# sthagen/foundationdb

Hardware: AMD Instinct MI355X
Metric: resolved txns/sec (conflict ranges checked/sec) per batch; HBM GB/s vs peak (higher is better)
Workload: dtype u8/int64 (byte keys, int64 versions)

## Files before the change

foundationdb_amd/build.py:

```python
from __future__ import annotations

import os
import shutil
import subprocess
import sys

HERE = os.path.dirname(os.path.abspath(__file__))
CSRC = os.path.join(HERE, "csrc")
ROOT = os.path.dirname(HERE)
LIB = os.path.join(HERE, "libfdbcs.so")
SOURCES = ["engine.cpp", "kernels.hip"]
HEADERS = ["dkey.h", "engine.h", "scan.h", "launch.h", "lane_xor.h"]
ARCH = os.environ.get("FDBCS_OFFLOAD_ARCH", "gfx950")


def _hipcc() -> str:
    for c in (os.environ.get("HIPCC"), "/opt/rocm/bin/hipcc", shutil.which("hipcc")):
        if c and os.path.exists(c):
            return c
    raise RuntimeError("hipcc not found")


def _stale() -> bool:
    if not os.path.exists(LIB):
        return True
    t = os.path.getmtime(LIB)
    deps = [os.path.join(CSRC, f) for f in SOURCES + HEADERS] + [os.path.join(ROOT, "include", "fdb_conflict_set.h")]
    return any(os.path.getmtime(d) > t for d in deps)


def build(force: bool = False, verbose: bool = False) -> str:
    if not force and not _stale():
        return LIB
    objs = []
    hipcc = _hipcc()
    common = ["-O3", "-std=c++17", "-fPIC", f"--offload-arch={ARCH}", "-Wall", "-Wno-unused-function",
              "-mllvm", "-disable-promote-alloca-to-lds"]
    for src in SOURCES:
        obj = os.path.join(CSRC, src.rsplit(".", 1)[0] + ".o")
        cmd = [hipcc, *common, "-c", os.path.join(CSRC, src), "-o", obj]
        if src.endswith(".cpp"):
            cmd = [hipcc, "-O3", "-std=c++17", "-fPIC", "-Wall", "-c", os.path.join(CSRC, src), "-o", obj]
        if verbose:
            print(" ".join(cmd), file=sys.stderr)
        subprocess.check_call(cmd)
        objs.append(obj)
    tmp = LIB + ".tmp"
    cmd = [hipcc, f"--offload-arch={ARCH}", "-shared", "-fPIC", "-o", tmp, *objs]
    if verbose:
        print(" ".join(cmd), file=sys.stderr)
    subprocess.check_call(cmd)
    os.replace(tmp, LIB)
    return LIB


if __name__ == "__main__":
    build(force="--force" in sys.argv, verbose=True)
    print(LIB)
```

foundationdb_amd/csrc/engine.cpp:

```cpp
#include <hip/hip_runtime.h>
#include <stdio.h>
#include <stdlib.h>
#include <string.h>
#include <unistd.h>

#include <cxxabi.h>

#include <algorithm>
#include <array>
#include <atomic>
#include <chrono>
#include <condition_variable>
#include <functional>
#include <mutex>
#include <new>
#include <string>
#include <thread>
#include <unordered_set>
#include <vector>

#include "../../include/fdb_conflict_set.h"
#include "engine.h"

using namespace fdbcs;
// ... 107 lines not shown
            shutdown();
            throw;
        }
    }
    ~AddPool() { shutdown(); }
    void shutdown() {
        {
            std::lock_guard<std::mutex> lk(m);
            stop = true;
            gen.fetch_add(1);
        }
        cv.notify_all();
        for (auto& t : th)
            if (t.joinable()) t.join();
    }
    void run(uint32_t g, int nn, const std::function<void(int)>* fn) {
        uint64_t cur = ticket.load(std::memory_order_acquire);
        for (;;) {
            if ((uint32_t)(cur >> 32) != g || (int)(cur & 0xffffffffu) >= nn) return;
            if (ticket.compare_exchange_weak(cur, cur + 1, std::memory_order_acq_rel)) {
                (*fn)((int)(cur & 0xffffffffu));
                done.fetch_add(1, std::memory_order_acq_rel);
                cur = ticket.load(std::memory_order_acquire);
            }
        }
    }
    void worker() {
        uint32_t seen = 0;
        for (;;) {
            uint32_t g;
            int nn;
            const std::function<void(int)>* fn;
            {
                std::unique_lock<std::mutex> lk(m);
                if (gen.load(std::memory_order_relaxed) == seen && !stop) {
                    sleepers.fetch_add(1);
                    cv.wait(lk, [&] { return stop || gen.load(std::memory_order_relaxed) != seen; });
                    sleepers.fetch_sub(1);
                }
                if (stop) return;
                seen = g = gen.load(std::memory_order_relaxed);
                nn = n;
                fn = job;
            }
            run(g, nn, fn);
        }
    }
    void parallel_for(int tickets, const std::function<void(int)>& fn) {
        uint32_t g;
        {
            std::lock_guard<std::mutex> lk(m);
            g = gen.load(std::memory_order_relaxed) + 1;
            n = tickets;
            job = &fn;
            done.store(0, std::memory_order_relaxed);
            ticket.store((uint64_t)g << 32, std::memory_order_release);
            gen.store(g, std::memory_order_release);
        }
        if (sleepers.load(std::memory_order_acquire) > 0) cv.notify_all();
        run(g, tickets, &fn);
        while (done.load(std::memory_order_acquire) < tickets) __builtin_ia32_pause();
    }
};

struct fdbcs_conflict_set {
    int device = 0;
    hipStream_t stream = nullptr;
    hipStream_t astream = nullptr;
    hipStream_t cstream = nullptr;
    hipEvent_t ev_c[kNumWork] = {};
    hipEvent_t ev_cmp = nullptr;
    bool cmp_recorded = false;
    int split_check = 2;
    hipStream_t ustream = nullptr;
    hipEvent_t ev_a[kNumWork] = {};
    hipEvent_t ev_b[kNumWork] = {};
    hipStream_t ystream = nullptr;
    hipEvent_t ev_res[kNumWork] = {};
    hipEvent_t xfree_ev[kNumWork] = {};
    bool prev_segs = false;
    int prev_wp = 0;
    int64_t prev_now = 0;
    int last_wp = -1, prev2_wp = -1;
    bool xfree_rec[kNumWork] = {};
    fdbcs_batch* ws_user[kNumWork] = {};
    fdbcs_batch* xfree_user[kNumWork] = {};
    bool y_async[kNumWork] = {};
    bool wused[kNumWork] = {};
    int wpar = 0;
    int timing = 0;
    uint32_t seq = 0;
    int64_t oldest = 0;
    int64_t header_version = 0;
    int64_t max_written = 0;
    int gc_interval = 0;
    int batches_since_compact = 0;
    int compactions_since_gc = 0;
    int64_t gc_applied = 0;
    int64_t delta_limit = 0;

    DBuf hkey[2], hlt[2], hver[2];
    DBuf lvl[kMaxLevels];
    DBuf dir;
    DBuf edir[2];
    uint32_t ddir_epoch[2] = {0, 0};
    uint32_t ddir_counter = 0;
    int cur = 0;
    int64_t hist_cap = 0;
    int64_t n_ub = 0;
    int64_t lvl3_n = 0;
    int64_t lvl2_n = 0;
    DBuf dkey[2], dlt[2], dver[2];
    DBuf dlvl[2][kMaxLevels];
    int dcur = 0;
    int64_t delta_cap = 0;
    int64_t nd_ub = 0;
    int64_t dlvl3_n = 0;
    int64_t dlvl2_n = 0;
    DBuf cws[6];
    DBuf htail[2];
    int tcur = 0;
    int64_t tail_ub = 0;
    int64_t tail_cap = 0;
    DBuf scal;
    int64_t route_timeout_ms = 60000;
    DBuf route_btail;
    std::vector<uint8_t> route_bounds;
    DBuf ws[kNumWork][56];
    DBuf wbtail[kNumWork];
    int64_t ws_T = -1, ws_R = -1, ws_W = -1;
    Work work[kNumWork]{};
    int64_t edge_cap = 0;

    int inflight = 0;
    bool validate = false;
    int bucket_target = 0;
    bool sort_cold = false;
    DBuf quant;
    int qcur = 0;
    bool quant_valid = false;
    hipStream_t quant_sa = nullptr;
    hipEvent_t ev_quant = nullptr;
    int64_t sort_big_buckets = 0;
    bool trace = false;
    bool serial = false;
    bool no_prepass = false;
    int64_t tail_reclaim = kTailReclaimDefault;
    bool write_groups = true;
    bool directory = true;
    uint32_t dir_p = 0;
    uint64_t dir_phi = 0, dir_plo = 0;
    uint32_t dir_e = 0, dir_top = 0;
    uint32_t dir_pos[kDirPos] = {}, dir_w[kDirPos] = {};
    int dir_bits = 0;
    DBuf trace_buf;
    struct KProf {
        const void* func;
        int64_t launches;
        double ms;
    };
    std::vector<KProf> kprof;
    const void* timed_func = nullptr;
    HBuf hold;
    HBuf hedge;
    bool skip_edges = true;
    fdbcs_stats stats{};
    std::vector<BatchSlot*> pool;
    bool submit_thread = true;
    int add_threads = 5;
    AddPool* add_pool = nullptr;
    int wait_query_ms = 2;
    bool htrace = false;
    std::vector<HSpan> htr[2];
    uint32_t work_a_seq = 0, work_y_seq = 0;
    double add_prof[4] = {0, 0, 0, 0};
    int64_t add_prof_n = 0;
    std::thread worker;
    std::mutex wmu;
    std::condition_variable wcv;
    std::atomic<int> wjob{0};
    std::atomic<uint32_t> b_issued{0};
    uint32_t b_recorded = 0;
    std::atomic<int> werr{0};
    LaunchList work_a, work_c;
    hipStream_t work_sa = nullptr;
    uint32_t work_need_b = 0;
    LaunchList work_y;
    hipStream_t work_ys = nullptr;
    uint32_t work_need_x = 0;
    std::atomic<uint32_t> x_issued{0};
    fdbcs_batch* work_y_batch = nullptr;
    LaunchList rec_a, rec_b, rec_c, rec_y, pending_b, pending_y;
    hipStream_t pending_ys = nullptr;
    fdbcs_batch* pending_batch = nullptr;
    std::unordered_set<fdbcs_batch*> live;
    DBuf x_pos, x_val, x_btail, x_state, x_ver, x_off, x_bytes;
    bool x_valid = false;
    int64_t x_n = 0, x_nbytes = 0;
    hipEvent_t x_ev0 = nullptr, x_ev1 = nullptr;
    double x_ms_kernels = 0, x_ms_d2h = 0;
    int64_t x_hdr = 0;
    DBuf i_bytes, i_off, i_ver, i_bnd, i_okey, i_olt, i_over, i_otail, i_mval, i_mkey, i_mlt, i_dblt, i_vblt, i_state;
    hipEvent_t i_ev[6] = {};
    double i_ms_kernels = 0, i_ms_host = 0;
};

struct BatchSlot {
    DBuf dev;
    HBuf pin_in;
    HBuf pin_out;
    DBuf dverdict;
    hipEvent_t ev[kPhCount] = {};
    bool events_made = false;
    hipEvent_t ev_up = nullptr;
    HBuf pin_inv;
    DBuf rt_scan, rt_inv, rt_rids, rt_dres, rt_info, rt_txpre;
    HBuf rt_res;
    hipEvent_t ev_rt0 = nullptr, ev_rt1 = nullptr;
    bool rt_timed = false;
    std::vector<hipEvent_t> prof_pool;
    size_t prof_next = 0;
    std::vector<std::pair<const void*, std::pair<hipEvent_t, hipEvent_t>>> prof_spans;
    LaunchList::Profile prof{&prof_pool, &prof_next, &prof_spans};
};

struct fdbcs_batch {
    fdbcs_conflict_set* cs = nullptr;
    BatchSlot* slot = nullptr;
    int report_enabled = 0;
    int state = 0;
    std::vector<int64_t> snap;
    std::vector<uint8_t> flags;
    std::vector<int32_t> roff{0}, woff{0};
    std::vector<int32_t> rowner, wowner;
    std::vector<DKey> rkeys, wkeys;
    std::vector<uint8_t> tail;
    bool direct = false;
    size_t d_keys = 0, d_rown = 0, d_wown = 0, d_tail = 0, d_small = 0;
    size_t d_tail_bytes = 0;
    BatchDev bd{};
    size_t tail_bytes = 0;
    uint8_t* h_verdict = nullptr;
    Scalars* h_scal = nullptr;
    uint8_t* h_rconf = nullptr;
    uint8_t* h_hist = nullptr;
    int32_t* h_first = nullptr;
    bool gc_ran = false;
    bool compacted = false;
    uint32_t seq = 0;
    volatile uint32_t* h_flag = nullptr;
    int64_t n_report = 0;
    uint32_t recorded = 0;
    bool any_report = false;
    int64_t check_hist = 0;
    std::vector<int32_t> out_ids;
    int64_t out_n = 0;
    uint8_t* out_dev = nullptr;
    int wp = 0;
    int32_t max_len = 0;
    int64_t wtail = 0;
    std::vector<int32_t> conf_off, conf_idx;
    int32_t n_committed = 0, n_too_old = 0;

    bool routed = false, route_pending = false;
    int32_t rT = 0, rR = 0, rW = 0;
    size_t r_tail = 0;

    int32_t T() const { return routed ? rT : (int32_t)snap.size(); }
    int32_t R() const { return routed ? rR : roff.back(); }
    int32_t W() const { return routed ? rW : woff.back(); }
    size_t tail_size() const { return routed ? r_tail : direct ? d_tail_bytes : tail.size(); }
};

namespace {

void add_key(fdbcs_batch* b, std::vector<DKey>& out, const uint8_t* p, int32_t len) {
    DKey k;
    dkey_prefix(p, (uint32_t)len, &k.hi, &k.lo);
    k.len = (uint32_t)len;
    k.tail = 0;
    if (len > b->max_len) b->max_len = len;
    if (len > 16) {
        k.tail = (uint32_t)b->tail.size();
        b->tail.insert(b->tail.end(), p + 16, p + len);
    }
    out.push_back(k);
}

int cmp_bytes(const uint8_t* a, int32_t al, const uint8_t* b, int32_t bl) {
    int c = memcmp(a, b, (size_t)std::min(al, bl));
    if (c) return c;
    return (al > bl) - (al < bl);
}

int ensure_scan_arena(fdbcs_conflict_set* cs) {
    if (cs->ws_T < 0 || cs->hist_cap <= 0) return FDBCS_OK;
    if (cs->delta_cap <= 0) return FDBCS_OK;
    const int64_t words = scan_arena_words(cs->ws_T, cs->ws_R, cs->ws_W, cs->hist_cap, cs->delta_cap);
    for (int k = 0; k < kNumWork; k++) {
        Work& w = cs->work[k];
        int rc = cs->ws[k][kWsArenaSlot].ensure(8 * words + 64);
        if (rc) return rc;
        w.scan_arena = (uint64_t*)cs->ws[k][kWsArenaSlot].p;
        if ((rc = cs->ws[k][kWsTileSlot].ensure(4 * (std::max(cs->hist_cap, cs->delta_cap) / 256 + 8)))) return rc;
        w.tile_first = (int32_t*)cs->ws[k][kWsTileSlot].p;
        carve_scans(w, cs->ws_T, cs->ws_R, cs->ws_W, cs->hist_cap, cs->delta_cap);
        HIPOK(hipMemsetAsync(w.scan_arena, 0, 8 * w.scan_words, cs->stream));
        for (int q = 0; q < kNumScans; q++) w.scan[q].error = &w.bsc->debug_error;
    }
    HIPOK(hipStreamSynchronize(cs->stream));
    return FDBCS_OK;
}

int flush_pending(fdbcs_conflict_set* cs);

int sync_all(fdbcs_conflict_set* cs) {
    if (int rc = flush_pending(cs)) return rc;
    HIPOK(hipStreamSynchronize(cs->ustream));
    HIPOK(hipStreamSynchronize(cs->cstream));
    HIPOK(hipStreamSynchronize(cs->astream));
    HIPOK(hipStreamSynchronize(cs->stream));
    HIPOK(hipStreamSynchronize(cs->ystream));
    cs->prev_segs = false;
    return FDBCS_OK;
}

int ensure_btail(fdbcs_conflict_set* cs, int64_t bytes) {
    const size_t need = (size_t)bytes + 64;
    if (cs->wbtail[0].p && need <= cs->wbtail[0].cap) return FDBCS_OK;
    if (int rc = sync_all(cs)) return rc;
    for (int k = 0; k < kNumWork; k++) {
        if (int rc = cs->wbtail[k].ensure(std::max<size_t>(need, 1 << 16))) return rc;
        cs->work[k].btail = (uint8_t*)cs->wbtail[k].p;
    }
    return FDBCS_OK;
}

int ensure_workspace(fdbcs_conflict_set* cs, int64_t T, int64_t R, int64_t W) {
    if (T <= cs->ws_T && R <= cs->ws_R && W <= cs->ws_W) return FDBCS_OK;
    T = std::max<int64_t>(T, std::max<int64_t>(cs->ws_T, 1024));
    R = std::max<int64_t>(R, std::max<int64_t>(cs->ws_R, 4096));
    W = std::max<int64_t>(W, std::max<int64_t>(cs->ws_W, 4096));
    if (int rc = sync_all(cs)) return rc;
    const int64_t E = 2 * (R + W);
    int64_t edge_cap = std::max<int64_t>(16 * R, 1 << 22);
    if (const char* env = getenv("FDBCS_EDGE_CAP")) edge_cap = std::max<int64_t>(1, atoll(env));
    for (int k = 0; k < kNumWork; k++) {
    Work& w = cs->work[k];
    size_t off = 0;
    char* arena = nullptr;
    auto take = [&](size_t bytes, void** ptr) -> int {
        off = align_up(off, 256);
        if (arena) *ptr = arena + off;
        off += bytes + 64;
        return FDBCS_OK;
    };
    for (int pass = 0; pass < 2; pass++) {
    if (pass == 1) {
        if (int rc = cs->ws[k][0].ensure(align_up(off, (size_t)2 << 20))) return rc;
        arena = (char*)cs->ws[k][0].p;
        off = 0;
    }
#define TAKE(field, bytes) \
    if (int rc = take((bytes), (void**)&w.field)) return rc
    TAKE(hist_conf, T);
    TAKE(rconf, R);
    TAKE(status, T);
    TAKE(first_conf, 4 * T);
    const int64_t slab_buckets = std::min<int64_t>(kSortMaxBuckets, (E + kSortTarget - 1) / kSortTarget + 1);
    TAKE(items, sizeof(SortItem) * E);
    TAKE(scnt, 8 * kCntStride * (size_t)kSortMaxBuckets);
    TAKE(slab, sizeof(SortItem) * kSlab * slab_buckets);
    TAKE(ovf, sizeof(SortItem) * E);
    TAKE(ovf_b, 4 * E);
    TAKE(big, sizeof(SortItem) * E);
    TAKE(big_p, 4 * E);
    TAKE(samples, sizeof(SortItem) * kMaxSample);
    TAKE(srank, 4 * (kMaxSample + 64));
    w.slab_buckets = (int32_t)slab_buckets;
    TAKE(pos, 4 * E);
    TAKE(pmeta, 4 * E);
    TAKE(cwb, 4 * (E + 1));
    TAKE(crb, 4 * (E + 1));
    TAKE(cwe, 4 * (E + 1));
    TAKE(wends, 8 * (2 * W + 1));
    TAKE(wkeys, sizeof(DKey) * (2 * W + 1));
    TAKE(segk, sizeof(DKey) * (2 * W + 2));
    TAKE(cflag, 2 * W + 2);
    TAKE(wbrange, 4 * W);
    TAKE(wlead, 4 * (W + 1));
    TAKE(wtxn, 4 * (W + 1));
    TAKE(gminc, 4 * (W + 1));
    TAKE(rbrange, 4 * R);
    TAKE(eoff, 4 * (R + 1));
    TAKE(poff, 4 * (R + W + 1));
    TAKE(pcg, 4 * (R + W + 1));
    TAKE(pcoff, 4 * (R + W + 1));
    TAKE(pcbase, 4 * (R + W + 1));
    TAKE(pca, 4 * (R + W + 1));
    TAKE(ecur, 4 * R);
    TAKE(edges, 4 * edge_cap);
    TAKE(eptr, 4 * T);
    TAKE(pre_st, T);
    TAKE(pre_ep, 4 * T);
    TAKE(pre_end, 4 * T);
    TAKE(ulist, 32 * T);
    TAKE(wpk, 4 * (W + 1));
    TAKE(tedges, 4 * edge_cap);
    TAKE(mcs_bits, 8 * (E / 64 + 2));
    TAKE(seg_b, 4 * (W + 1));
    TAKE(seg_e, 4 * (W + 1));
    TAKE(seg_lo, 8 * (W + 1));
    TAKE(seg_hi, 8 * (W + 1));
    TAKE(seg_rem, 8 * (W + 1));
    TAKE(seg_ins, 8 * (W + 1));
    TAKE(seg_tlen, 8 * (W + 1));
    TAKE(seg_endins, W + 1);
    TAKE(seg_vend, 8 * (W + 1));
    TAKE(verdict, T);
    TAKE(bsc, sizeof(BatchScalars));
    }
#undef TAKE
    w.edge_cap = edge_cap;
    w.cap_T = T;
    w.cap_R = R;
    HIPOK(hipMemsetAsync(w.hist_conf, 0, T, cs->stream));
    HIPOK(hipMemsetAsync(w.rconf, 0, R, cs->stream));
    HIPOK(hipMemsetAsync(w.ecur, 0, 4 * R, cs->stream));
    HIPOK(hipMemsetAsync(w.scnt, 0, 8 * kCntStride * (size_t)kSortMaxBuckets, cs->stream));
    HIPOK(hipMemsetAsync(w.srank, 0, 4 * (kMaxSample + 64), cs->stream));
    HIPOK(hipMemsetAsync(w.bsc, 0, sizeof(BatchScalars), cs->stream));
    if (k >= 1) {
        Work& w0 = cs->work[0];
        w.c_lo = w0.c_lo, w.c_hi = w0.c_hi, w.c_rem = w0.c_rem, w.c_ins = w0.c_ins, w.c_val = w0.c_val;
        w.c_exact = w0.c_exact;
    }
    }
    cs->edge_cap = edge_cap;
    cs->prev_segs = false;
    cs->ws_T = T;
    cs->ws_R = R;
    cs->ws_W = W;
    return ensure_scan_arena(cs);
}

constexpr int64_t kDeltaFloor = 1250000;
constexpr int kTimingEvery = 4;
int64_t delta_limit_for(const fdbcs_conflict_set* cs, int64_t n_base) {
    if (cs->delta_limit > 0) return cs->delta_limit;
    return std::max<int64_t>({(int64_t)1 << 16, n_base / 16, std::min<int64_t>(n_base / 4, kDeltaFloor)});
}


Hist hist_of(fdbcs_conflict_set* cs, int k) {
    Hist h;
    h.key = (ulonglong2*)cs->hkey[k].p;
    h.lt = (uint2*)cs->hlt[k].p;
    h.ver = (int64_t*)cs->hver[k].p;
    return h;
}

void carve_index(MaxLevels& m, ulonglong2* base, int64_t cap) {
    for (int L = 0; L < kIdxLevels; L++) {
        m.skey[L] = base;
        base += idx_level_cap(cap, L);
    }
    m.skey8 = base;
    m.idx_cap = cap;
}

int64_t index_bytes(int64_t cap) {
    int64_t n = 0;
    for (int L = 0; L < kIdxLevels; L++) n += idx_level_cap(cap, L);
    return 16 * (n + cap / 8 + 2);
}

static void set_dir_fields(const fdbcs_conflict_set* cs, MaxLevels& m) {
    m.dir_p = cs->dir_p;
    m.dir_phi = cs->dir_phi;
    m.dir_plo = cs->dir_plo;
    m.dir_e = cs->dir_e;
    m.dir_top = cs->dir_top;
    for (int i = 0; i < kDirPos; i++) m.dir_pos[i] = cs->dir_pos[i], m.dir_w[i] = cs->dir_w[i];
}

static int set_dir_map(fdbcs_conflict_set* cs, const ulonglong2* k, int64_t n) {
    auto byte_at = [](const ulonglong2& x, int i) -> uint32_t {
        return i < 8 ? (uint32_t)(x.x >> (56 - 8 * i)) & 255u : (uint32_t)(x.y >> (56 - 8 * (i - 8))) & 255u;
    };
    const bool rank = n >= 2;
    uint32_t p = 0;
    if (rank) {
        const uint64_t xh = k[0].x ^ k[n - 1].x, xl = k[0].y ^ k[n - 1].y;
        const uint32_t lcp = xh ? (uint32_t)__builtin_clzll(xh) / 8 : (xl ? 8 + (uint32_t)__builtin_clzll(xl) / 8 : 16);
        p = std::min<uint32_t>(lcp, 15);
    }
    const uint64_t mh = p >= 8 ? ~0ull : (p ? ~0ull << (64 - 8 * p) : 0ull);
    const uint64_t ml = p <= 8 ? 0ull : ~0ull << (128 - 8 * p);
    cs->dir_p = p;
    cs->dir_phi = n ? k[0].x & mh : 0;
    cs->dir_plo = n ? k[0].y & ml : 0;
    const int npos = std::min<int>(kDirPos, 16 - (int)p);
    uint32_t lo[kDirPos], hi[kDirPos];
    for (int i = 0; i < kDirPos; i++) lo[i] = rank ? 255 : 0, hi[i] = 255;
    if (rank) {
        for (int i = 0; i < kDirPos; i++) hi[i] = 0;
        const int64_t stride = std::max<int64_t>(1, n / (1 << 21));
        auto mark = [&](const ulonglong2& x) {
            for (int i = 0; i < npos; i++) {
                const uint32_t b = byte_at(x, (int)p + i);
                lo[i] = std::min(lo[i], b);
                hi[i] = std::max(hi[i], b);
            }
        };
        for (int64_t j = 0; j < n; j += stride) mark(k[j]);
        mark(k[n - 1]);
    }
    const int64_t samples = (n + kFan - 1) / kFan;
    uint64_t budget = 1ull << 16;
    if (cs->dir_bits)
        budget = 1ull << cs->dir_bits;
    else
        while (budget < (1ull << kDirMaxBits) && 8 * budget < (uint64_t)samples) budget <<= 1;
    uint32_t radix[kDirPos], shift[kDirPos];
    uint64_t prod = 1;
    int e = 0;
    for (int i = 0; i < npos; i++) {
        const uint32_t d = hi[i] - lo[i] + 1;
        shift[i] = 0;
        if (prod * d <= budget) {
            radix[i] = d;
            prod *= d;
            if (d > 1) e = i + 1;
            continue;
        }
        uint32_t s = 0;
        while (prod * (((d - 1) >> s) + 1) > budget) s++;
        if (((d - 1) >> s) + 1 > 1) {
            radix[i] = ((d - 1) >> s) + 1;
            shift[i] = s;
            e = i + 1;
        }
        break;
    }
    prod = 1;
    for (int i = 0; i < e; i++) prod *= radix[i];
    uint64_t w = 1;
    for (int i = kDirPos - 1; i >= 0; i--) {
        if (i >= e) {
            cs->dir_pos[i] = cs->dir_w[i] = 0;
            continue;
        }
        cs->dir_pos[i] = lo[i] | (hi[i] - lo[i] + 1) << 8 | shift[i] << 17;
        cs->dir_w[i] = (uint32_t)w;
        w *= radix[i];
    }
    cs->dir_e = (uint32_t)e;
    cs->dir_top = (uint32_t)prod + 2;
    return FDBCS_OK;
}

MaxLevels levels_of(fdbcs_conflict_set* cs, int k) {
    MaxLevels m;
    m.lvl[0] = (int64_t*)cs->hver[k].p;
    for (int L = 1; L < kMaxLevels; L++) m.lvl[L] = (int64_t*)cs->lvl[L].p;
    m.keys = (const ulonglong2*)cs->hkey[k].p;
    carve_index(m, (ulonglong2*)cs->lvl[0].p, cs->hist_cap);
    m.dir = cs->directory ? (const int32_t*)cs->dir.p : nullptr;
    set_dir_fields(cs, m);
    return m;
}

Hist delta_of(fdbcs_conflict_set* cs, int k) {
    Hist h;
    h.key = (ulonglong2*)cs->dkey[k].p;
    h.lt = (uint2*)cs->dlt[k].p;
    h.ver = (int64_t*)cs->dver[k].p;
    return h;
}

MaxLevels dlevels_of(fdbcs_conflict_set* cs, int k) {
    MaxLevels m;
    m.lvl[0] = (int64_t*)cs->dver[k].p;
    for (int L = 1; L < kMaxLevels; L++) m.lvl[L] = (int64_t*)cs->dlvl[k][L].p;
    m.keys = (const ulonglong2*)cs->dkey[k].p;
    carve_index(m, (ulonglong2*)cs->dlvl[k][0].p, cs->delta_cap);
    m.edir = (uint64_t*)cs->edir[k].p;
    m.edir_epoch = cs->edir[k].p ? cs->ddir_epoch[k] : 0;
    set_dir_fields(cs, m);
    return m;
}

int sync_sizes(fdbcs_conflict_set* cs) {
    if (int rc = sync_all(cs)) return rc;
    Scalars s;
    HIPOK(hipMemcpyAsync(&s, cs->scal.p, sizeof(s), hipMemcpyDeviceToHost, cs->stream));
    HIPOK(hipStreamSynchronize(cs->stream));
    cs->n_ub = s.n;
    cs->nd_ub = s.nd;
    cs->tail_ub = s.tail_used;
    return FDBCS_OK;
}

int alloc_levels(DBuf* lv, int64_t cap, int64_t* top_n, int64_t* l2_n) {
    lv[0].release();
    if (int rc = lv[0].ensure(index_bytes(cap))) return rc;
    int64_t m = cap;
    for (int L = 1; L < kMaxLevels; L++) {
// ... 1598 lines not shown
    b->bd.rowner = a.rown;
    b->bd.wowner = a.wown;
    b->bd.snap = a.snap;
    b->bd.roff = a.roff;
    b->bd.woff = a.woff;
    b->bd.flags = a.flags;
    b->bd.tail = a.tail;
    b->routed = true;
    b->route_pending = true;
    b->rT = b->rR = b->rW = 0;
    b->out_dev = conflict_out;
    b->out_n = n_global;
    b->out_ids.clear();
    b->state = 1;
    return FDBCS_OK;
}

static int finish_route(fdbcs_batch* b) {
    if (!b->route_pending) return FDBCS_OK;
    BatchSlot* sl = b->slot;
    HIPOK(hipEventSynchronize(sl->ev_up));
    std::atomic_thread_fence(std::memory_order_acquire);
    RouteResult r;
    memcpy(&r, (const void*)sl->rt_res.p, sizeof(r));
    if (r.error != 0) {
        if (r.error == 2) fprintf(stderr, "fdbcs: routed batch: the shares' ready flag was never set\n");
        b->routed = b->route_pending = false;
        b->out_dev = nullptr;
        b->out_n = 0;
        b->state = 0;
        return r.error == 2 ? FDBCS_E_TIMEOUT
                            : r.error == 1 ? FDBCS_E_NOMEM : r.error == 3 ? FDBCS_E_INVALID : FDBCS_E_DEVICE;
    }
    b->rT = r.T;
    b->rR = r.R;
    b->rW = r.W;
    b->r_tail = (size_t)r.tail_bytes;
    b->tail_bytes = b->r_tail;
    b->bd.tail_n = r.tail_bytes;
    b->bd.T = r.T;
    b->bd.R = r.R;
    b->bd.W = r.W;
    b->wtail = r.tail_bytes + 14 * (int64_t)r.W;
    b->max_len = r.n_gt24 ? 25 : (r.n_gt19 ? 20 : 16);
    b->any_report = r.reports > 0;
    b->route_pending = false;
    return FDBCS_OK;
}

int fdbcs_batch_routed_info(fdbcs_batch* b, int32_t* T, int32_t* R, int32_t* W, void** inv_dev, void** read_ids_dev) {
    if (!b) return FDBCS_E_INVALID;
    if (!b->routed) return FDBCS_E_STATE;
    if (int rc = finish_route(b)) return rc;
    if (T) *T = b->rT;
    if (R) *R = b->rR;
    if (W) *W = b->rW;
    if (inv_dev) *inv_dev = b->slot->rt_inv.p;
    if (read_ids_dev) *read_ids_dev = b->slot->rt_rids.p;
    return FDBCS_OK;
}

int fdbcs_sync(fdbcs_conflict_set* cs) {
    if (!cs) return FDBCS_E_INVALID;
    HIPOK(hipSetDevice(cs->device));
    return sync_all(cs);
}

int fdbcs_batch_upload(fdbcs_batch* b) {
    if (!b) return FDBCS_E_INVALID;
    if (!b->cs) return FDBCS_E_STATE;
    if (b->state != 0) return b->state == 1 ? FDBCS_OK : FDBCS_E_STATE;
    HIPOK(hipSetDevice(b->cs->device));
    return do_upload(b, b->cs->ustream);
}


int fdbcs_batch_detect_async(fdbcs_batch* b, int64_t now, int64_t new_oldest_version) {
    if (!b) return FDBCS_E_INVALID;
    if (!b->cs) return FDBCS_E_STATE;
    if (b->state > 1) return FDBCS_E_STATE;
    fdbcs_conflict_set* cs = b->cs;
    const auto t_begin = std::chrono::steady_clock::now();
    HIPOK(hipSetDevice(cs->device));
    if (now < cs->max_written) return FDBCS_E_VERSION;
    if (int rc0 = finish_route(b)) return rc0;
    if (b->T() > kMaxTxnLds) return FDBCS_E_INVALID;
    const int64_t tail_add = b->wtail;
    if (cs->tail_ub + tail_add + 1 >= kTailLimit) return FDBCS_E_NOMEM;
    const int64_t T = b->T(), R = b->R(), W = b->W();
    int rc;
    if ((rc = ensure_workspace(cs, T, R, W))) return rc;
    if ((rc = ensure_btail(cs, (int64_t)b->tail_size()))) return rc;
    if ((rc = ensure_delta(cs, cs->nd_ub + 2 * W + 1))) return rc;
    if ((rc = ensure_history(cs, cs->n_ub + cs->nd_ub + 2 * W + 1, cs->tail_ub + tail_add + 1)))
        return rc;
    if ((rc = ensure_events(b))) return rc;
    if (cs->ddir_counter == UINT32_MAX && cs->edir[0].p) {
        if ((rc = sync_all(cs))) return rc;
        for (int k = 0; k < 2; k++) HIPOK(hipMemsetAsync(cs->edir[k].p, 0, 8 * (size_t)kDirAlloc, cs->stream));
        HIPOK(hipStreamSynchronize(cs->stream));
        cs->ddir_counter = 0;
    }
    const ResultLayout RL = result_layout(T, R);
    const size_t o_sc = RL.sc, o_fl = RL.fl, o_rc = RL.rc, o_hc = RL.hc, o_fc = RL.fc, out_bytes = RL.total;
    BatchSlot* sl = b->slot;
    if ((rc = sl->pin_out.ensure(out_bytes, true))) return rc;
    char* ho = (char*)sl->pin_out.p;
    b->h_verdict = (uint8_t*)ho;
    b->h_scal = (Scalars*)(ho + o_sc);
    b->h_flag = (volatile uint32_t*)(ho + o_fl);
    b->h_rconf = (uint8_t*)(ho + o_rc);
    b->h_hist = (uint8_t*)(ho + o_hc);
    b->h_first = (int32_t*)(ho + o_fc);
    if ((rc = sl->dverdict.ensure(T + 64))) return rc;
    if (b->out_dev && b->out_n > 0 && !b->routed) {
        if ((int64_t)b->out_ids.size() != T) return FDBCS_E_STATE;
        if ((rc = sl->pin_inv.ensure(4 * (size_t)b->out_n + 64, true))) return rc;
        int32_t* inv = (int32_t*)sl->pin_inv.p;
        std::fill(inv, inv + b->out_n, -1);
        for (int32_t t = 0; t < (int32_t)T; t++) inv[b->out_ids[t]] = t;
    }
    if (!b->routed) {
        b->any_report = b->n_report > 0;
    }
    b->seq = ++cs->seq;
    if (b->seq == 0) b->seq = ++cs->seq;
    *b->h_flag = 0;
    b->recorded = 0;

    hipStream_t s = cs->stream;
    const int timing = cs->timing;
    hipStream_t sa = (timing == 2 || cs->serial) ? s : cs->astream;
    const int wp = cs->wpar;
    cs->wpar = (wp + 1) % kNumWork;
    b->wp = wp;
    Work& w = cs->work[wp];
    w.groups = cs->write_groups && W > 0 && W <= kMaxGroupWrites && T <= kMaxTxnLds ? 1 : 0;
    const bool sampled = timing >= 2 || b->seq % (uint32_t)kTimingEvery == 0;
    auto rec = [&](int ph, int level) -> hipEvent_t {
        if (timing == 3 || timing < level || (level == 1 && (!sampled || cs->timed_func))) return nullptr;
        b->recorded |= 1u << ph;
        return sl->ev[ph];
    };
    auto mark = [&](int ph) -> int {
        if (hipEvent_t e = rec(ph, 2)) fdb_event(LaunchList::kTimingRecord, e, s);
        return FDBCS_OK;
    };
    const bool was_uploaded = b->state == 1;
    LaunchList& la = cs->rec_a;
    LaunchList& lb = cs->rec_b;
    LaunchList& lc = cs->rec_c;
    LaunchList& ly = cs->rec_y;
    la.clear();
    lb.clear();
    lc.clear();
    ly.clear();
    sl->prof_next = 0;
    sl->prof_spans.clear();
    const bool kprof = timing == 3 || (timing == 1 && sampled && cs->timed_func);
    for (LaunchList* L : {&la, &lb, &lc, &ly}) {
        L->prof = kprof ? &sl->prof : nullptr;
        L->timed_func = timing == 3 ? nullptr : cs->timed_func;
    }
    const bool split = (cs->split_check == 1 || (cs->split_check == 2 && cs->n_ub >= kSplitCheckMinBase)) &&
                       !cs->serial && timing != 2;
    const bool threaded = cs->submit_thread && timing < 2 && !cs->trace && sa != s;
    cs->stats.host_ms_prepare += host_ms_since(t_begin);
    const auto t_rec = std::chrono::steady_clock::now();
    const bool own_upload = timing != 2 && !cs->serial;
    if (hipEvent_t e = rec(kPhStart, 2)) HIPOK(hipEventRecord(e, sa));
    if (b->state == 0 && (rc = do_upload(b, own_upload ? cs->ustream : sa))) return rc;
    if (hipEvent_t e = rec(kPhUpload, 2)) HIPOK(hipEventRecord(e, sa));
    t_record = &la;
    const bool ws_busy = cs->wused[wp] && (threaded || !stage_b_done(cs, wp));
    if (ws_busy && (sa != s || cs->y_async[wp])) fdb_event(LaunchList::kSyncWait, cs->ev_b[wp], sa);
    if (cs->xfree_rec[wp] && sa != s && (threaded || !batch_done(cs->xfree_user[wp])))
        fdb_event(LaunchList::kSyncWait, cs->xfree_ev[wp], sa);
    cs->xfree_rec[wp] = false;
    cs->wused[wp] = true;
    cs->ws_user[wp] = b;
    if (own_upload || (was_uploaded && hipEventQuery(sl->ev_up) != hipSuccess))
        fdb_event(LaunchList::kSyncWait, sl->ev_up, sa);
    const BatchDev& bd = b->bd;
    if (b->routed) launch_route_too_old(sa, bd, cs->oldest);
    const bool long_keys = b->max_len > 24;
    Scalars* sc = (Scalars*)cs->scal.p;
    const int bsrc = cs->cur, dsrc = cs->dcur;
    const bool pipe = !(timing == 2 || cs->serial);
    hipStream_t ys = pipe ? cs->ystream : s;
    const bool use_prev = pipe && cs->prev_segs;
    const int dchk = use_prev ? dsrc ^ 1 : dsrc;
    const Tier base{hist_of(cs, bsrc), levels_of(cs, bsrc), &sc->n, cs->header_version};
    const Tier delta{delta_of(cs, dsrc), dlevels_of(cs, dsrc), &sc->ndb[dsrc], kHole};
    const Tier cdelta{delta_of(cs, dchk), dlevels_of(cs, dchk), &sc->ndb[dchk], kHole};
    PrevSegs ps{};
    if (use_prev) {
        const Work& pw = cs->work[cs->prev_wp];
        ps = PrevSegs{pw.segk, pw.btail, &pw.bsc->n_segments, cs->prev_now};
    }
    uint8_t* htail = (uint8_t*)cs->htail[cs->tcur].p;

    w.trace = cs->trace ? (unsigned long long*)cs->trace_buf.p : nullptr;
    w.no_prepass = cs->no_prepass ? 1 : 0;
    if (w.trace) {
        HIPOK(hipStreamSynchronize(cs->astream));
        HIPOK(hipStreamSynchronize(s));
        unsigned long long init[kTrSlots];
        for (int i = 0; i < kTrSlots; i++)
            init[i] = (i == kTrSampleBegin || i == kTrCheckBegin || i == kTrEpiBegin || i == kTrResBegin || i == kTrResW0min ||
                       i == kTrPartBegin || i == kTrBktBegin)
                          ? ~0ull
                          : 0ull;
        HIPOK(hipMemcpy(w.trace, init, sizeof(init), hipMemcpyHostToDevice));
    }
    int sort_nb = 0, sort_samples = 0;
    {
        const int64_t E = 2 * (R + W);
        const int nbk = sort_bucket_count(E, cs->bucket_target, w.slab_buckets);
        const bool cold = nbk > 1 && (cs->sort_cold || !cs->quant_valid);
        sort_nb = E > 0 ? nbk : 0;
        sort_samples = E > 0 && cold ? sort_cold_samples(E, nbk) : 0;
        const bool write_quant = E >= kQuantMinE;
        SplitKey* qt = (SplitKey*)cs->quant.p;
        if (cs->quant_sa && cs->quant_sa != sa) {
            if ((rc = flush_pending(cs))) return rc;
            HIPOK(hipEventRecord(cs->ev_quant, cs->quant_sa));
            fdb_event(LaunchList::kSyncWait, cs->ev_quant, sa);
        }
        cs->quant_sa = sa;
        launch_sort(sa, bd, w, qt + cs->qcur * kQuant, write_quant ? qt + (cs->qcur ^ 1) * kQuant : nullptr, cold,
                    cs->bucket_target, b->max_len > (int32_t)kSortNxLen, cs->validate, rec(kPhSortBegin, 1),
                    rec(kPhSortEnd, 1));
        if (write_quant) {
            cs->qcur ^= 1;
            cs->quant_valid = true;
        }
    }
    mark(kPhSort);
    if (cs->validate) launch_validate_sort(sa, bd, w);
    w.hseq = b->seq;
    launch_edges(sa, bd, w);
    if (sa != s) fdb_event(LaunchList::kSyncRecord, cs->ev_a[wp], sa);
    mark(kPhEdges);
    if (split) {
        t_record = &lc;
        hipStream_t sc_ = cs->cstream;
        fdb_event(LaunchList::kSyncWait, sl->ev_up, sc_);
        if (ws_busy) fdb_event(LaunchList::kSyncWait, cs->ev_b[wp], sc_);
        if (cs->cmp_recorded && (threaded || hipEventQuery(cs->ev_cmp) != hipSuccess))
            fdb_event(LaunchList::kSyncWait, cs->ev_cmp, sc_);
        fdb_event(LaunchList::kTimingRecord, rec(kPhCheckBegin, 1), sc_);
        launch_check_tier(sc_, bd, w, base, true, htail, long_keys, PrevSegs{});
        fdb_event(LaunchList::kTimingRecord, rec(kPhCheckEnd, 1), sc_);
        fdb_event(LaunchList::kSyncRecord, cs->ev_c[wp], sc_);
    }
    t_record = &lb;
    if (sa == s || !was_uploaded || hipEventQuery(sl->ev_up) != hipSuccess) fdb_event(LaunchList::kSyncWait, sl->ev_up, s);
    {
        const int wy = use_prev ? cs->prev2_wp : cs->last_wp;
        if (wy >= 0 && cs->y_async[wy] && (threaded || !stage_b_done(cs, wy)))
            fdb_event(LaunchList::kSyncWait, cs->ev_b[wy], s);
    }
    if (split) {
        b->check_hist = cs->n_ub;
        launch_check_tier(s, bd, w, cdelta, false, htail, long_keys, ps);
    } else {
        b->check_hist = cs->n_ub + cs->nd_ub;
        fdb_event(LaunchList::kTimingRecord, rec(kPhCheckBegin, 1), s);
        launch_check(s, bd, w, base, cdelta, htail, long_keys, ps);
        fdb_event(LaunchList::kTimingRecord, rec(kPhCheckEnd, 1), s);
    }
    if (use_prev) {
        cs->xfree_ev[cs->prev_wp] = cs->ev_res[wp];
        cs->xfree_user[cs->prev_wp] = b;
        cs->xfree_rec[cs->prev_wp] = true;
    }
    mark(kPhCheck);
    if (sa != s) fdb_event(LaunchList::kSyncWait, cs->ev_a[wp], s);
    if (split) fdb_event(LaunchList::kSyncWait, cs->ev_c[wp], s);
    w.vdev = (uint8_t*)sl->dverdict.p;
    launch_resolve(s, bd, w, b->any_report, (uint8_t*)sl->pin_out.dp, sc);
    w.vdev = nullptr;
    if (b->out_dev && b->out_n > 0)
        launch_conflict_output(s, bd, w, b->routed ? (const int32_t*)sl->rt_inv.p : (const int32_t*)sl->pin_inv.dp,
                               b->out_n, b->out_dev);
    if (b->any_report) {
        char* hdv = (char*)sl->pin_out.dp;
        if (R) launch_copy_bytes(s, hdv + o_rc, w.rconf, R);
        launch_copy_bytes(s, hdv + o_hc, w.hist_conf, T);
        launch_copy_bytes(s, hdv + o_fc, w.first_conf, 4 * T);
    }
    mark(kPhIntra);
    mark(kPhCombine);
    fdb_event(LaunchList::kSyncRecord, cs->ev_res[wp], s);
    t_record = &ly;
    if (ys != s) fdb_event(LaunchList::kSyncWait, cs->ev_res[wp], ys);
    const int dnew = dsrc ^ 1;
    const int64_t nd_after = cs->nd_ub + 2 * W;
    const int64_t new_oldest = std::max(cs->oldest, new_oldest_version);
    bool compact = nd_after > delta_limit_for(cs, cs->n_ub);
    if (cs->gc_interval > 0 && ++cs->batches_since_compact >= cs->gc_interval) compact = true;
    if (cs->tail_ub > cs->tail_reclaim) compact = true;
    char* hd = (char*)sl->pin_out.dp;
    launch_merge(ys, bd, w, delta.h, delta.m, delta_of(cs, dnew), dlevels_of(cs, dnew), &sc->ndb[dsrc], htail, sc, now,
                 cs->dlvl3_n, cs->dlvl2_n, cs->nd_ub + 1, rec(kPhCopyBegin, 1), rec(kPhCopyEnd, 1), long_keys);
    mark(kPhMerge);
    bool gc = false;
    int final_base = bsrc;
    const int64_t base_hint = cs->n_ub + nd_after + 1;
    if (compact) {
        launch_compact(ys, w, base.h, base.m, delta_of(cs, dnew), hist_of(cs, bsrc ^ 1), htail, sc,
                       cs->header_version, cs->lvl3_n, cs->lvl2_n, nd_after + 1, cs->n_ub + 1, rec(kPhCompBegin, 1),
                       rec(kPhCompEnd, 1), long_keys ? 2 : 1, cs->n_ub <= (16 << 20) ? 1024 : 4096,
                       cs->n_ub > (16 << 20));
        final_base = bsrc ^ 1;
        cs->batches_since_compact = 0;
        const bool gc_turn = cs->gc_interval > 0 || ++cs->compactions_since_gc >= kGcEveryCompactions;
        gc = (new_oldest > cs->gc_applied && gc_turn) || cs->tail_ub > cs->tail_reclaim;
        if (gc) cs->compactions_since_gc = 0;
    }
    mark(kPhCompact);
    if (gc) {
        launch_gc(ys, w, hist_of(cs, final_base), hist_of(cs, final_base ^ 1), htail,
                  (uint8_t*)cs->htail[cs->tcur ^ 1].p, sc, std::max(new_oldest, cs->gc_applied), cs->header_version,
                  base_hint);
        cs->tcur ^= 1;
        final_base ^= 1;
        cs->gc_applied = new_oldest;
    }
    mark(kPhGc);
    b->gc_ran = gc;
    b->compacted = compact;
    if (compact || !cs->edir[dnew].p) {
        cs->ddir_epoch[dnew] = 0;
    } else {
        cs->ddir_epoch[dnew] = ++cs->ddir_counter;
    }
    launch_epilogue(ys, bd, w, compact ? levels_of(cs, final_base) : dlevels_of(cs, dnew), sc, compact ? 1 : 0,
                    gc ? 1 : 0, (uint8_t*)hd, (uint32_t*)(hd + o_fl), b->seq,
                    compact ? base_hint : nd_after + 1, &sc->ndb[dnew], sort_nb, sort_samples);
    fdb_event(LaunchList::kSyncRecord, cs->ev_b[wp], ys);
    if (compact || gc) {
        fdb_event(LaunchList::kSyncRecord, cs->ev_cmp, ys);
        cs->cmp_recorded = true;
    }
    mark(kPhEpilogue);
    mark(kPhEnd);
    t_record = nullptr;
    cs->stats.host_ms_record += host_ms_since(t_rec);
    const auto t_sub = std::chrono::steady_clock::now();
    if (threaded) {
        if ((rc = worker_wait(cs))) return rc;
        std::swap(cs->work_a, la);
        std::swap(cs->work_c, lc);
        cs->work_sa = sa;
        cs->work_a_seq = b->seq;
        const bool prev = cs->pending_batch != nullptr;
        if (prev) {
            cs->work_y_seq = cs->pending_batch->seq;
            std::swap(cs->work_y, cs->pending_y);
            cs->work_ys = cs->pending_ys;
            cs->work_need_x = cs->x_issued.load(std::memory_order_relaxed) + 1;
            cs->work_y_batch = cs->pending_batch;
        }
        cs->work_need_b = cs->b_recorded;
        worker_start_job(cs);
        if (prev) {
            fdbcs_batch* pb_ = cs->pending_batch;
            cs->pending_batch = nullptr;
            const int64_t tx = cs->htrace ? mono_ns() : 0;
            const uint32_t pseq = pb_->seq;
            hipError_t e = cs->pending_b.replay(s, x_skip(cs, pb_), &cs->stats.x_launches_skipped);
            if (cs->htrace) cs->htr[0].push_back({pseq, 'X', tx, mono_ns()});
            cs->x_issued.fetch_add(1, std::memory_order_release);
            if (e != hipSuccess) return FDBCS_E_DEVICE;
        }
        std::swap(cs->pending_b, lb);
        std::swap(cs->pending_y, ly);
        cs->pending_ys = ys;
        cs->b_recorded++;
        cs->pending_batch = b;
    } else if (flush_pending(cs)) {
        return FDBCS_E_DEVICE;
    } else {
        HIPOK(la.replay(sa));
        if (split) HIPOK(lc.replay(cs->cstream));
        HIPOK(lb.replay(s));
        HIPOK(ly.replay(ys));
    }
    HIPOK(take_launch_error());
    cs->stats.host_ms_submit += host_ms_since(t_sub);
    cs->cur = final_base;
    cs->dcur = dnew;
    cs->prev_segs = pipe && !compact;
    cs->prev2_wp = cs->last_wp;
    cs->last_wp = wp;
    cs->y_async[wp] = ys != s;
    cs->prev_wp = wp;
    cs->prev_now = now;
    cs->oldest = new_oldest;
    if (W) cs->max_written = std::max(cs->max_written, now);
    if (compact) {
        cs->n_ub += nd_after;
        cs->nd_ub = 0;
    } else {
        cs->nd_ub = nd_after;
    }
    cs->tail_ub += tail_add;
    cs->inflight++;
    cs->x_valid = false;
    b->state = 2;
    if (cs->htrace)
        cs->htr[0].push_back({b->seq, 'D',
                              (int64_t)std::chrono::duration_cast<std::chrono::nanoseconds>(t_begin.time_since_epoch()).count(),
                              mono_ns()});
    return FDBCS_OK;
}

int fdbcs_batch_wait(fdbcs_batch* b, uint8_t* verdicts, int32_t* n_committed, int32_t* n_too_old) {
    if (!b) return FDBCS_E_INVALID;
    if (b->state == 2 && !b->cs) return FDBCS_E_STATE;
    fdbcs_conflict_set* cs = b->cs;
    if (b->state == 2) {
        const int64_t tw0 = cs->htrace ? mono_ns() : 0;
        HIPOK(hipSetDevice(cs->device));
        if (cs->pending_batch == b)
            if (int rc = flush_pending(cs)) return rc;
        if (cs->work_y_batch == b)
            if (int rc = worker_wait(cs)) return rc;
        auto t_q = std::chrono::steady_clock::now();
        for (uint64_t spin = 0; *b->h_flag != b->seq; spin++) {
            __builtin_ia32_pause();
            if ((spin & 4095) != 4095) continue;
            if (std::chrono::steady_clock::now() - t_q < std::chrono::milliseconds(cs->wait_query_ms)) continue;
            t_q = std::chrono::steady_clock::now();
            {
                hipError_t e = hipStreamQuery(cs->astream);
                if (e == hipSuccess || e == hipErrorNotReady) e = hipStreamQuery(cs->stream);
                if (e == hipSuccess) e = hipStreamQuery(cs->ystream);
                if (e != hipSuccess && e != hipErrorNotReady) {
                    fprintf(stderr, "fdbcs: stream error while waiting: %s\n", hipGetErrorString(e));
                    return FDBCS_E_DEVICE;
                }
                if (e == hipSuccess && *b->h_flag != b->seq) {
                    fprintf(stderr, "fdbcs: stream idle but batch %u not completed\n", b->seq);
                    return FDBCS_E_DEVICE;
                }
            }
        }
        std::atomic_thread_fence(std::memory_order_acquire);
        if (cs->htrace) cs->htr[0].push_back({b->seq, 'W', tw0, mono_ns()});
        if (cs->trace && cs->inflight == 1) {
            if (int rc = sync_all(cs)) return rc;
            unsigned long long tr[kTrSlots];
            HIPOK(hipMemcpy(tr, cs->trace_buf.p, sizeof(tr), hipMemcpyDeviceToHost));
            auto us = [&](int a, int z) { return (double)((long long)(tr[z] - tr[a])) / 100.0; };
            fprintf(stderr,
                    "fdbcs trace: sample %.2f us, check %.2f us (check starts %+.2f us after sample); epilogue "
                    "levels %.2f, zero %.2f, host %.2f, fence %.2f us\n",
                    us(kTrSampleBegin, kTrSampleEnd), us(kTrCheckBegin, kTrCheckEnd), us(kTrSampleBegin, kTrCheckBegin),
                    us(kTrEpiBegin, kTrEpiLevels), us(kTrEpiLevels, kTrEpiZero), us(kTrEpiZero, kTrEpiHost),
                    us(kTrEpiHost, kTrEpiFence));
            fprintf(stderr,
                    "fdbcs trace: sort partition fill %.2f, search %.2f, end %.2f us; bucket prologue %.2f, "
                    "sorted %.2f, ties %.2f, end %.2f us (partition start to bucket start %.2f us)\n",
                    us(kTrPartBegin, kTrPartFill), us(kTrPartBegin, kTrPartSearch), us(kTrPartBegin, kTrPartEnd),
                    us(kTrBktBegin, kTrBktPrologue), us(kTrBktBegin, kTrBktSorted), us(kTrBktBegin, kTrBktTies),
                    us(kTrBktBegin, kTrBktEnd),
                    us(kTrPartBegin, kTrBktBegin));
            {
                const double nw = tr[kTrBktWaves] ? (double)tr[kTrBktWaves] : 1.0;
                fprintf(stderr, "fdbcs trace: bucket tie runs: %llu lanes in runs, %llu ranked in registers, %llu serially, "
                        "longest run %llu\n", tr[kTrBktRuns], tr[kTrBktSimple], tr[kTrBktSlow], tr[kTrBktMaxRun]);
                fprintf(stderr,
                        "fdbcs trace: bucket per wave (%llu waves): load %.2f, sort %.2f, ties %.2f, put %.2f us\n",
                        tr[kTrBktWaves], tr[kTrBktSumLoad] / nw / 100.0, tr[kTrBktSumSort] / nw / 100.0,
                        tr[kTrBktSumTies] / nw / 100.0, tr[kTrBktSumPut] / nw / 100.0);
                const double np = tr[kTrPartWaves] ? (double)tr[kTrPartWaves] : 1.0;
                fprintf(stderr,
                        "fdbcs trace: partition per wave (%llu waves): fill %.2f, tail copy %.2f, search %.2f, "
                        "place %.2f us\n",
                        tr[kTrPartWaves], tr[kTrPartSumFill] / np / 100.0, tr[kTrPartSumCopy] / np / 100.0,
                        tr[kTrPartSumSearch] / np / 100.0, tr[kTrPartSumPlace] / np / 100.0);
            }
            fprintf(stderr, "fdbcs trace: resolve pre-pass %.2f us, wait %.2f us, rounds %.2f us (setup %.2f, first round "
                    "%.2f of which minima %.2f, %d rounds), finish %.2f us; waves start %.2f..%.2f us before the first kernarg use\n",
                    us(kTrResBegin, kTrResPre), us(kTrResPre, kTrResWait), us(kTrResWait, kTrResRounds),
                    us(kTrResWait, kTrResSetup), us(kTrResSetup, kTrResRound1), us(kTrResSetup, kTrResMin1),
                    (int)b->h_scal->intra_rounds,
                    us(kTrResRounds, kTrResEnd), us(kTrResW0min, kTrResWait), us(kTrResW0max, kTrResWait));
            fprintf(stderr, "fdbcs trace: combine chunk 0: loads %.2f, scan1 %.2f, scan2 %.2f, stores %.2f us\n",
                    us(kTrResRounds, kTrCmbLoad), us(kTrCmbLoad, kTrCmbScan1), us(kTrCmbScan1, kTrCmbScan2),
                    us(kTrCmbScan2, kTrCmbStore));


        }
        if (b->h_scal->debug_error) {
            fprintf(stderr, "fdbcs: device invariant check failed (debug_error=%d)\n", b->h_scal->debug_error);
            cs->inflight--;
            b->state = 3;
            return FDBCS_E_DEVICE;
        }
        const int32_t T = b->T();
        int32_t nc = 0, nt = 0;
        for (int32_t t = 0; t < T; t++) {
            nc += b->h_verdict[t] == FDBCS_TRANSACTION_COMMITTED;
            nt += b->h_verdict[t] == FDBCS_TRANSACTION_TOO_OLD;
        }
        b->n_committed = nc;
        b->n_too_old = nt;
        b->conf_off.assign(T + 1, 0);
        b->conf_idx.clear();
        if (b->any_report) {
            for (int32_t t = 0; t < T; t++) {
                if ((b->flags[t] & kFlagReport) && b->h_verdict[t] == FDBCS_TRANSACTION_CONFLICT) {
                    if (b->h_hist[t]) {
                        for (int32_t r = b->roff[t]; r < b->roff[t + 1]; r++)
                            if (b->h_rconf[r]) b->conf_idx.push_back(r - b->roff[t]);
                    } else if (b->h_first[t] != INT_MAX) {
                        b->conf_idx.push_back(b->h_first[t]);
                    }
                }
                b->conf_off[t + 1] = (int32_t)b->conf_idx.size();
            }
        }
        fdbcs_stats& st = cs->stats;
        st.batches++;
        st.transactions += T;
        st.read_ranges += b->R();
        st.write_ranges += b->W();
        for (int e : {(int)kPhEnd, (int)kPhCompEnd, (int)kPhCopyEnd, (int)kPhCheckEnd})
            if ((b->recorded >> e) & 1u) {
                HIPOK(hipEventSynchronize(b->slot->ev[e]));
                break;
            }
        for (const auto& sp : b->slot->prof_spans) {
            HIPOK(hipEventSynchronize(sp.second.second));
            const double ms = ev_ms(sp.second.first, sp.second.second);
            auto it = std::find_if(cs->kprof.begin(), cs->kprof.end(), [&](const auto& k) { return k.func == sp.first; });
            if (it == cs->kprof.end()) {
                cs->kprof.push_back({sp.first, 0, 0.0});
                it = cs->kprof.end() - 1;
            }
            it->launches += 1;
            it->ms += ms;
        }
        b->slot->prof_spans.clear();
        auto ph = [&](int a, int z) {
            return ((b->recorded >> a) & (b->recorded >> z) & 1u) ? ev_ms(b->slot->ev[a], b->slot->ev[z]) : 0.0;
        };
        st.ms_upload += ph(kPhStart, kPhUpload);
        st.ms_sort += ph(kPhUpload, kPhSort);
        st.ms_intra += ph(kPhSort, kPhEdges) + ph(kPhCheck, kPhIntra);
        st.ms_check_read += ph(kPhEdges, kPhCheck);
        st.ms_combine += ph(kPhIntra, kPhCombine);
        st.ms_merge += ph(kPhCombine, kPhMerge);
        st.ms_compact += ph(kPhMerge, kPhCompact);
        st.ms_gc += ph(kPhCompact, kPhGc);
        st.ms_epilogue += ph(kPhGc, kPhEpilogue);
        st.ms_total += ph(kPhUpload, kPhEnd);
        if (b->h_scal->intra_edges < 0) {
            st.intra_fallbacks += 1;
        } else {
            st.intra_edges += b->h_scal->intra_edges;
            st.intra_rounds += b->h_scal->intra_rounds;
        }
        {
            const int64_t kept = b->h_scal->d_before - b->h_scal->d_rem, out = b->h_scal->nd_next;
            const int64_t bytes = 32 * (kept + (out - kept) + out);
            st.merge_bytes_all += bytes;
            st.delta_sum += b->h_scal->d_before;
            st.base_sum += b->h_scal->n;
            st.segments_sum += b->h_scal->n_segments;
            if ((b->recorded >> kPhCopyEnd) & 1u) {
                st.ms_merge_kernel += ph(kPhCopyBegin, kPhCopyEnd);
                st.merge_launches += 1;
                st.merge_bytes += bytes;
            }
        }
        if ((b->recorded >> kPhCheckEnd) & 1u) {
            st.ms_check_kernel += ph(kPhCheckBegin, kPhCheckEnd);
            st.check_launches += b->R() > 0;
            st.check_reads += b->R();
            st.check_history += b->R() > 0 ? b->check_hist : 0;
        }
        if ((b->recorded >> kPhSortEnd) & 1u) {
            st.ms_sort_kernel += ph(kPhSortBegin, kPhSortEnd);
            st.sort_launches += 1;
            st.sort_items += 2 * (int64_t)(b->R() + b->W());
        }
        st.gc_runs += b->gc_ran ? 1 : 0;
        st.sort_big_buckets += b->h_scal->sort_big;
        if (b->routed && b->slot->rt_timed) {
            float ms = 0.f;
            if (hipEventElapsedTime(&ms, b->slot->ev_rt0, b->slot->ev_rt1) == hipSuccess) st.ms_route_kernels += ms;
            st.routed_batches += 1;
            b->slot->rt_timed = false;
        }
        if (b->compacted) {
            st.compactions += 1;
            const int64_t kept = b->h_scal->c_before - b->h_scal->c_rem;
            const int64_t bytes = 32 * (kept + (b->h_scal->n_next - kept) + b->h_scal->n_next);
            st.compact_bytes_all += bytes;
            if ((b->recorded >> kPhCompEnd) & 1u) {
                st.ms_compact_kernel += ph(kPhCompBegin, kPhCompEnd);
                st.compact_launches += 1;
                st.compact_bytes += bytes;
            }
        }
        cs->inflight--;
        if (cs->inflight == 0) {
            cs->n_ub = b->h_scal->n;
            cs->nd_ub = b->h_scal->nd;
            cs->tail_ub = b->h_scal->tail_used;
        }
        b->state = 3;
    }
    if (b->state != 3) return FDBCS_E_STATE;
    if (verdicts && b->T()) memcpy(verdicts, b->h_verdict, b->T());
    if (n_committed) *n_committed = b->n_committed;
    if (n_too_old) *n_too_old = b->n_too_old;
    return FDBCS_OK;
}

int fdbcs_batch_detect_conflicts(fdbcs_batch* b, int64_t now, int64_t new_oldest_version, uint8_t* verdicts,
                                 int32_t* n_committed, int32_t* n_too_old) {
    int rc = fdbcs_batch_detect_async(b, now, new_oldest_version);
    if (rc) return rc;
    return fdbcs_batch_wait(b, verdicts, n_committed, n_too_old);
}

int fdbcs_batch_conflicting_reads(fdbcs_batch* b, int32_t txn, int32_t* idx_out, int32_t cap, int32_t* n_out) {
    if (!b || !n_out) return FDBCS_E_INVALID;
    if (b->state != 3) return FDBCS_E_STATE;
    if (txn < 0 || txn >= b->T()) return FDBCS_E_INVALID;
    const int32_t a = b->conf_off[txn], e = b->conf_off[txn + 1];
    *n_out = e - a;
    if (idx_out)
        for (int32_t i = a; i < e && i - a < cap; i++) idx_out[i - a] = b->conf_idx[i];
    return FDBCS_OK;
}

int fdbcs_batch_too_old(fdbcs_batch* b, int32_t* idx_out, int32_t cap, int32_t* n_out) {
// ... 84 lines not shown
```

foundationdb_amd/csrc/engine.h:

```cpp
#pragma once
#include <hip/hip_runtime.h>
#include <stdint.h>
#include <limits.h>

#include "dkey.h"
#include "scan.h"

namespace fdbcs {

constexpr int kBlock = 256;
constexpr int kWG = 1024;
constexpr int kSortTile = 4096;
constexpr int kFan = 64;
constexpr int kMaxLevels = 4;
constexpr int kL3Rep = 8;
constexpr int kL3Pad = 16;
__host__ __device__ constexpr int64_t l3_words(int64_t n) { return n * kL3Rep * kL3Pad; }
constexpr int kGcTile = 4096;
constexpr int kMaxGroupWrites = 12288;
constexpr int kMaxTxnLds = 49152;

enum : uint8_t { kUndecided = 0, kAborted = 1, kCommitted = 2 };
enum : uint8_t { kFlagTooOld = 1, kFlagReport = 2 };

struct Hist {
    ulonglong2* key;
    uint2* lt;
    int64_t* ver;
};

constexpr int kArity = 8;
constexpr int kDirMaxBits = 20;
constexpr int kDirAlloc = (1 << kDirMaxBits) + 4;
constexpr int kDirPos = 8;
constexpr int kDirRun = 128;
constexpr int kIdxLevels = 12;
struct MaxLevels {
    int64_t* lvl[kMaxLevels];
    const ulonglong2* keys;
    ulonglong2* skey[kIdxLevels];
    ulonglong2* skey8;
    int64_t idx_cap;
    const int32_t* dir = nullptr;
    uint32_t dir_p = 0;
    uint64_t dir_phi = 0, dir_plo = 0;
    uint32_t dir_e = 0;
    uint32_t dir_top = 0;
    uint32_t dir_pos[kDirPos] = {};
    uint32_t dir_w[kDirPos] = {};
    uint64_t* edir = nullptr;
    uint32_t edir_epoch = 0;
};
__host__ __device__ inline int64_t idx_level_cap(int64_t cap, int L) {
    int64_t d = 64;
    for (int i = 0; i < L && d <= cap; i++) d *= kArity;
    return cap / d + 2;
}

struct Scalars {
    int64_t n;
    int64_t nd;
    int64_t n_next;
    int64_t nd_next;
    int64_t n_gc;
    int64_t tail_used;
    int64_t tail_next;
    int64_t tail_gc;
    int64_t n_segments;
    int64_t d_before;
    int64_t d_rem;
    int64_t c_before;
    int64_t c_rem;
    int32_t debug_error;
    int32_t intra_rounds;
    int64_t intra_edges;
    int32_t sort_big;
    int32_t sort_pad;
    int64_t ndb[2];
};

struct BatchScalars {
    int64_t n_edges;
    int32_t edge_overflow;
    int32_t rounds;
    int32_t debug_error;
    int32_t ovf_n;
    int32_t sort_big;
    int64_t n_segments;
    int64_t n_pranges;
    int32_t n_undec;
    int32_t pad2;
};

constexpr int64_t kHole = INT64_MIN;

struct TierIO {
    const int64_t* n_in;
    int64_t* n_out;
    int64_t* before;
    int64_t* removed;
};

struct Segs {
    int64_t *lo, *hi, *rem, *ins;
    int32_t* tile_first;
};

enum ScanKind { kScanEdges, kScanSegSum, kScanCompact, kScanGc, kScanCover, kScanSegNum, kScanFold, kNumScans };

struct BatchDev {
    int32_t T, R, W;
    int64_t* snap;
    uint8_t* flags;
    int32_t* roff;
    int32_t* woff;
    int32_t* rowner;
    int32_t* wowner;
    DKey* keys;
    uint8_t* tail;
    int64_t tail_n;
};

#ifndef FDBCS_SORT_TARGET
#define FDBCS_SORT_TARGET 64
#endif
constexpr int kSortTarget = FDBCS_SORT_TARGET;
constexpr int kSlab = 256;
constexpr int kSortMaxBuckets = 4096;
constexpr int kQuant = 4096;
constexpr int kQuantMinE = 2048;
constexpr int kMaxSample = 8192;
#ifndef FDBCS_CNT_STRIDE
#define FDBCS_CNT_STRIDE 16
#endif
constexpr int kCntStride = FDBCS_CNT_STRIDE;
constexpr int kSplitWords = 8;
constexpr int kSplitBytes = 8 * kSplitWords;
struct SplitKey {
    uint64_t w[kSplitWords];
    uint32_t len, meta;
};

struct Work {
    uint8_t* hist_conf;
    uint8_t* rconf;
    uint8_t* status;
    int32_t* first_conf;
    SortItem* items;
    uint64_t* scnt;
    SortItem* slab;
    int32_t slab_buckets;
    SortItem* ovf;
    int32_t* ovf_b;
    SortItem* big;
    int32_t* big_p;
    SortItem* samples;
    int32_t* srank;
    int32_t* pos;
    uint32_t* pmeta;
    int32_t* cwb;
    int32_t* crb;
    int32_t* cwe;
    int2* wends;
    DKey* wkeys;
    DKey* segk;
    uint8_t* cflag;
    uint8_t* btail;
    int32_t* wbrange;
    int32_t* rbrange;
    int32_t* eoff;
    int32_t* poff;
    int32_t* pcg;
    int32_t* pcoff;
    int32_t* pcbase;
    int32_t* pca;
    int32_t* ecur;
    int32_t* wlead;
    int32_t* wtxn;
    int32_t* gminc;
    int32_t groups = 0;
    int32_t* edges;
    int64_t edge_cap;
    int32_t* eptr;
    uint8_t* pre_st;
    int32_t* pre_ep;
    int32_t* pre_end;
    int4* ulist;
    uint32_t* wpk;
    int32_t report = 0;
    int32_t* tedges;
    uint64_t* mcs_bits;
    int32_t* seg_b;
    int32_t* seg_e;
    int64_t* seg_lo;
    int64_t* seg_hi;
    int64_t* seg_rem;
    int64_t* seg_ins;
    int64_t* seg_tlen;
    uint8_t* seg_endins;
    int64_t* seg_vend;
    uint8_t* verdict;
    BatchScalars* bsc;
    ScanState scan[kNumScans];
    int64_t scan_gran[kNumScans];
    uint64_t* scan_arena;
    int64_t scan_words;
    int64_t cap_T, cap_R;
    int32_t* tile_first;
    int64_t *c_lo, *c_hi, *c_rem, *c_ins, *c_val;
    uint8_t* c_exact;
    unsigned long long* trace;
    int32_t no_prepass;
    uint32_t* hedge;
    uint32_t hseq;
    uint8_t* vdev;
};

enum TraceSlot {
    kTrSampleBegin, kTrSampleEnd, kTrCheckBegin, kTrCheckEnd,
    kTrEpiBegin, kTrEpiLevels, kTrEpiZero, kTrEpiHost, kTrEpiFence, kTrEpiEnd,
    kTrResBegin, kTrResPre, kTrResWait, kTrResRounds, kTrResEnd,
    kTrPartBegin, kTrPartFill, kTrPartSearch, kTrPartEnd,
    kTrBktBegin, kTrBktPrologue, kTrBktSorted, kTrBktTies, kTrBktEnd,
    kTrBktWaves, kTrBktSumLoad, kTrBktSumSort, kTrBktSumTies, kTrBktSumPut,
    kTrPartWaves, kTrPartSumFill, kTrPartSumCopy, kTrPartSumSearch, kTrPartSumPlace,
    kTrCmbLoad, kTrCmbScan1, kTrCmbScan2, kTrCmbStore,
    kTrResSetup, kTrResRound1,
    kTrResMin1,
    kTrResW0min, kTrResW0max,
    kTrBktRuns, kTrBktSimple, kTrBktSlow, kTrBktMaxRun,
    kTrSlots
};
__device__ __forceinline__ void trace_min(unsigned long long* tr, int slot) {
    if (tr) atomicMin(&tr[slot], (unsigned long long)wall_clock64());
}
__device__ __forceinline__ void trace_max(unsigned long long* tr, int slot) {
    if (tr) atomicMax(&tr[slot], (unsigned long long)wall_clock64());
}

__host__ __device__ inline int64_t verdict_scalars_offset(int64_t T) { return (T + 64) / 64 * 64; }

struct ShareHeader {
    int32_t T, R, W, pad0;
    int64_t bytes;
    int64_t off_keys, off_snap, off_roff, off_woff, off_report, off_tail;
    int64_t tail_bytes;
    int64_t off_owner;
    int64_t pad[5];
};
static_assert(sizeof(ShareHeader) == 128, "ShareHeader is 128 bytes");
struct RouteResult {
    int32_t T, R, W, reports;
    int32_t n_gt19, n_gt24;
    int64_t tail_bytes;
    int32_t error;
    int32_t pad;
    int64_t global_T;
};
struct RouteArgs {
    const uint8_t* shares;
    int64_t stride;
    int32_t n_shares, tcap;
    int32_t has_lo, has_hi;
    DKey lo, hi;
    const uint8_t* btail;
    int32_t report_enabled;
    int32_t cap_T, cap_R, cap_W;
    int64_t cap_tail;
    DKey* keys;
    uint32_t* info;
    int64_t rstride;
    int4* txpre;
    int32_t *rown, *wown, *roff, *woff;
    int64_t* snap;
    uint8_t* flags;
    uint8_t* tail;
    int32_t* inv;
    int64_t inv_n;
    int32_t* read_ids;
    uint8_t* out_zero;
    int64_t out_n;
    RouteResult* res;
    RouteResult* dres;
    const uint32_t* ready;
    uint32_t ready_value;
    uint32_t* wait_err;
    uint64_t wait_ticks;
};
void launch_route(hipStream_t s, const RouteArgs& a, ScanState st);
int64_t route_scan_words(int64_t n_elems);
void launch_route_too_old(hipStream_t s, const BatchDev& b, int64_t oldest);

struct Tier {
    Hist h;
    MaxLevels m;
    const int64_t* n;
    int64_t hdr;
};
struct PrevSegs {
    const DKey* segk;
    const uint8_t* tail;
    const int64_t* n;
    int64_t version;
};
void launch_sort(hipStream_t s, const BatchDev& b, const Work& w, SplitKey* quant, SplitKey* quant_out, bool cold,
                 int bucket_target, bool long_keys, bool validate, hipEvent_t sort_begin, hipEvent_t sort_end);
int sort_bucket_count(int64_t E, int target, int slab_buckets);
void launch_check(hipStream_t s, const BatchDev& b, const Work& w, const Tier& base, const Tier& delta,
                  const uint8_t* htail, bool long_keys = false, const PrevSegs& ps = PrevSegs{});
void launch_check_tier(hipStream_t s, const BatchDev& b, const Work& w, const Tier& t, bool is_base,
                       const uint8_t* htail, bool long_keys = false, const PrevSegs& ps = PrevSegs{});
hipError_t debug_time_sort(hipStream_t s, const BatchDev& b, const Work& w, SplitKey* quant, int bucket_target,
                           bool long_keys, int which, int reps, double* us);
void launch_validate_sort(hipStream_t s, const BatchDev& b, const Work& w);
void launch_edges(hipStream_t s, const BatchDev& b, const Work& w);
void launch_resolve(hipStream_t s, const BatchDev& b, const Work& w, bool report, uint8_t* verdict_out, Scalars* sc);
void launch_merge(hipStream_t s, const BatchDev& b, const Work& w, const Hist& src, const MaxLevels& srcm,
                  const Hist& dst, const MaxLevels& dstm, const int64_t* nd_src, uint8_t* htail, Scalars* sc,
                  int64_t now, int64_t lvl3_n, int64_t lvl2_n, int64_t grid_hint_n, hipEvent_t copy_begin,
                  hipEvent_t copy_end, bool long_keys = false);
void launch_compact(hipStream_t s, const Work& w, const Hist& base, const MaxLevels& basem, const Hist& delta,
                    const Hist& dst, const uint8_t* htail, Scalars* sc, int64_t header_version, int64_t lvl3_n,
                    int64_t lvl2_n, int64_t delta_hint_n, int64_t grid_hint_n, hipEvent_t copy_begin,
                    hipEvent_t copy_end, int mode, int base_tile, bool nt);
void launch_gc(hipStream_t s, const Work& w, const Hist& src, const Hist& dst, const uint8_t* tsrc, uint8_t* tdst,
               Scalars* sc, int64_t oldest, int64_t header_version, int64_t grid_hint_n);
void launch_hold(hipStream_t s, const uint32_t* release);
void init_kernel_attributes();
void launch_copy_bytes(hipStream_t s, void* dst, const void* src, int64_t n);
void launch_conflict_output(hipStream_t s, const BatchDev& b, const Work& w, const int32_t* inv, int64_t n,
                            uint8_t* out);
int64_t scan_arena_words(int64_t T, int64_t R, int64_t W, int64_t hist_cap, int64_t delta_cap);
void carve_scans(Work& w, int64_t T, int64_t R, int64_t W, int64_t hist_cap, int64_t delta_cap);
void launch_rangemax(hipStream_t s, const MaxLevels& m, Scalars* sc, const int64_t* n, int64_t lvl3_n,
                     int64_t lvl2_n, int64_t grid_hint_n);
void launch_epilogue(hipStream_t s, const BatchDev& b, const Work& w, const MaxLevels& m, Scalars* sc,
                     int compacted, int gc_ran, uint8_t* verdict_out, uint32_t* flag,
                     uint32_t seq, int64_t grid_hint_n, int64_t* nd_out, int sort_nb, int sort_samples);
int sort_cold_samples(int64_t E, int nb);

enum ExportWord { kXwLo, kXwHi, kXwHeader, kXwN, kXwBytes, kXwScan , kXwWords = 8 };
struct ExportArgs {
    Hist base, delta;
    const uint8_t* htail;
    int64_t nb, nd;
    int64_t hdr;
    int64_t floor;
    int32_t has_lo, has_hi;
    DKey lo, hi;
    const uint8_t* btail;
    int64_t* d_pos;
    int64_t* d_val;
    int64_t* words;
    int64_t* tile_tb;
    int64_t* versions;
    int64_t* offsets;
    uint8_t* bytes;
    int64_t bytes_cap;
};
int64_t export_tiles(int64_t n);
void launch_export(hipStream_t s, const ExportArgs& a, const MaxLevels& basem, uint64_t* granules, int mode);

enum ImportWord {
    kIwError,
    kIwJlo,
    kIwM,
    kIwKept,
    kIwTailUnits,
    kIwMaxVer,
    kIwScan,
    kIwWords = 8
};
struct ImportArgs {
    Hist base, delta;
    const uint8_t* htail;
    int64_t nb, nd;
    int64_t hdr;
    int64_t n;
    const uint8_t* bytes;
    int64_t nbytes;
    const int64_t* offsets;
    const int64_t* versions;
    int64_t ihdr;
    int32_t has_lo, has_hi;
    int32_t lo_len, hi_len;
    const uint8_t* bnd;
    int64_t bnd_hi;
    Hist ov;
    uint8_t* otail;
    int64_t otail_lo, otail_hi;
    int64_t ovhdr;
    int64_t* words;
    int64_t* m_val;
    ulonglong2* m_key;
    uint2* m_lt;
    int64_t* d_blt;
    int64_t* v_blt;
    Hist dst;
    uint8_t* tdst;
    int64_t dst_cap, tdst_units;
    int64_t new_hdr;
};
void launch_import_overlay(hipStream_t s, const ImportArgs& a);
void launch_import_fold(hipStream_t s, const ImportArgs& a, int64_t m, uint64_t* granules);
void launch_import_max(hipStream_t s, const MaxLevels& m, int64_t lvl3_n, int64_t* out);

}
```

foundationdb_amd/csrc/kernels.hip:

```cpp
#include <hip/hip_runtime.h>
#include <stdio.h>
#include <stdlib.h>
#include <algorithm>
#include <vector>
#include <limits.h>

#include "engine.h"
#include "lane_xor.h"

namespace fdbcs {

thread_local LaunchList* t_record = nullptr;
thread_local uint8_t t_group = 0;
thread_local hipError_t t_launch_error = hipSuccess;


__device__ __forceinline__ const uint8_t* hist_tail(const uint8_t* htail, uint32_t unit) {
    return htail + 8 * (size_t)unit;
}
__device__ __forceinline__ uint32_t tail_units(uint32_t len) { return len > 16u ? (len - 16u + 7u) / 8u : 0u; }

__device__ __forceinline__ void copy_tail_words(uint8_t* dst, const uint8_t* src, uint32_t n) {
    const uintptr_t a = (uintptr_t)src;
    const uint64_t* w = (const uint64_t*)(a & ~(uintptr_t)7);
    const uint32_t sh = (uint32_t)(a & 7u) * 8u;
    uint64_t* d = (uint64_t*)dst;
    for (uint32_t i = 0; i < (n + 7u) / 8u; i++) d[i] = sh ? (w[i] >> sh) | (w[i + 1] << (64u - sh)) : w[i];
}

__device__ __forceinline__ int hist_cmp(const Hist& h, int64_t i, const uint8_t* htail, const DKey& q,
                                        const uint8_t* qtail) {
    ulonglong2 k = h.key[i];
    if (k.x != q.hi) return k.x < q.hi ? -1 : 1;
    if (k.y != q.lo) return k.y < q.lo ? -1 : 1;
    uint2 lt = h.lt[i];
    if (lt.x > 16u && q.len > 16u) return tail_cmp(hist_tail(htail, lt.y), lt.x, qtail + q.tail, q.len);
    return (lt.x > q.len) - (lt.x < q.len);
}

__device__ __forceinline__ bool prefix_less(const ulonglong2& k, const DKey& q) {
    return k.x < q.hi || (k.x == q.hi && k.y < q.lo);
}

__device__ __forceinline__ int probe_cmp(const Hist& h, int64_t i, const ulonglong2& k, const uint8_t* htail,
                                         const DKey& q, const uint8_t* qtail) {
    if (k.x != q.hi) return k.x < q.hi ? -1 : 1;
    if (k.y != q.lo) return k.y < q.lo ? -1 : 1;
    return hist_cmp(h, i, htail, q, qtail);
}
__device__ __forceinline__ int probe_cmp_lean(const Hist& h, int64_t i, const ulonglong2& k, const uint8_t* htail,
                                              const DKey& q, const uint8_t* qtail) {
    if (k.x != q.hi) return k.x < q.hi ? -1 : 1;
    if (k.y != q.lo) return k.y < q.lo ? -1 : 1;
    const uint2 lt = h.lt[i];
#if defined(__HIP_DEVICE_COMPILE__)
    if (lt.x > 16u && q.len > 16u) {
        const uint8_t* ta = hist_tail(htail, lt.y);
        const uint8_t* tb = qtail + q.tail;
        const uint32_t nb = (lt.x < q.len ? lt.x : q.len) - 16u;
        for (uint32_t o = 0; o < nb; o += 8) {
            const int vb = (int)(nb - o);
            const uint64_t msk = vb >= 8 ? ~0ull : ~0ull << (64 - 8 * vb);
            const uint64_t x = tail_word(ta + o) & msk, y = tail_word(tb + o) & msk;
            if (x != y) return x < y ? -1 : 1;
        }
    }
#endif
    return (lt.x > q.len) - (lt.x < q.len);
}

constexpr int kQW = 12;
[[maybe_unused]] constexpr int kHW = 6;
struct QTail {
    uint64_t w[kQW];
};

__device__ __forceinline__ void load_qtail(QTail& qt, const DKey& q, const uint8_t* qtail) {
#if defined(__HIP_DEVICE_COMPILE__)
    const uint32_t n = q.len > 16u ? q.len - 16u : 0u;
    const uintptr_t a = (uintptr_t)(qtail + q.tail);
    const uint64_t* w = (const uint64_t*)(a & ~(uintptr_t)7);
    const uint32_t sh = (uint32_t)(a & 7u) * 8u;
    const uint32_t cnt = ((uint32_t)(a & 7u) + n + 7u) / 8u;
    uint64_t raw[kQW + 1];
#pragma unroll
    for (int j = 0; j <= kQW; j++) raw[j] = (uint32_t)j < cnt ? w[j] : 0ull;
#pragma unroll
    for (int j = 0; j < kQW; j++) qt.w[j] = __builtin_bswap64(sh ? (raw[j] >> sh) | (raw[j + 1] << (64u - sh)) : raw[j]);
#endif
}

__device__ __forceinline__ int probe_cmp_long(const ulonglong2& k, const uint2& lt, const uint8_t* htail, const DKey& q,
                                              const QTail& qt, const uint8_t* qtail) {
    if (k.x != q.hi) return k.x < q.hi ? -1 : 1;
    if (k.y != q.lo) return k.y < q.lo ? -1 : 1;
#if defined(__HIP_DEVICE_COMPILE__)
    if (lt.x > 16u && q.len > 16u) {
        const uint64_t* ha = (const uint64_t*)hist_tail(htail, lt.y);
        const uint32_t n = (lt.x < q.len ? lt.x : q.len) - 16u;
        const int nw = (int)((n + 7u) / 8u);
#pragma unroll
        for (int j0 = 0; j0 < kQW; j0 += kHW) {
            if (j0 >= nw) break;
            uint64_t x[kHW];
#pragma unroll
            for (int u = 0; u < kHW; u++) x[u] = j0 + u < nw ? ha[j0 + u] : 0ull;
#pragma unroll
            for (int u = 0; u < kHW; u++) {
                const int j = j0 + u;
                const int vb = (int)n - 8 * j;
                if (vb <= 0) break;
                const uint64_t msk = vb >= 8 ? ~0ull : ~0ull << (64 - 8 * vb);
                const uint64_t hx = __builtin_bswap64(x[u]) & msk, qy = qt.w[j] & msk;
                if (hx != qy) return hx < qy ? -1 : 1;
            }
        }
        if (nw > kQW)
            return tail_cmp(hist_tail(htail, lt.y) + 8 * kQW, lt.x - 8 * kQW, qtail + q.tail + 8 * kQW,
                            q.len - 8 * kQW);
    }
#endif
    return (lt.x > q.len) - (lt.x < q.len);
}

__device__ __forceinline__ uint32_t gmask(bool pred) {
    const uint64_t m = __ballot(pred);
    return (uint32_t)(m >> (threadIdx.x & 63 & ~(kArity - 1))) & ((1u << kArity) - 1u);
}

__device__ __forceinline__ uint32_t dir_slot(const MaxLevels& m, uint64_t hi, uint64_t lo) {
    const uint32_t p = m.dir_p;
    if (p) {
        const uint64_t mh = p >= 8 ? ~0ull : ~0ull << (64 - 8 * p);
        const uint64_t ml = p <= 8 ? 0ull : ~0ull << (128 - 8 * p);
        const uint64_t xh = hi & mh, xl = lo & ml;
        if (xh != m.dir_phi || xl != m.dir_plo)
            return (xh < m.dir_phi || (xh == m.dir_phi && xl < m.dir_plo)) ? 0u : m.dir_top;
    }
    const uint64_t h = p == 0 ? hi : (p < 8 ? (hi << (8 * p)) | (lo >> (64 - 8 * p)) : lo << (8 * (p - 8)));
    uint32_t code = 1;
    bool live = true;
#pragma unroll
    for (int i = 0; i < kDirPos; i++) {
        const uint32_t b = (uint32_t)(h >> (56 - 8 * i)) & 255u;
        const uint32_t pos = m.dir_pos[i];
        const uint32_t l = pos & 255u, d = (pos >> 8) & 511u, s = pos >> 17;
        const uint32_t r = b < l ? 0u : (b - l < d ? b - l : d);
        if (live && (uint32_t)i < m.dir_e) code += (r >> s) * m.dir_w[i];
        live = live && b >= l && b - l < d;
    }
    return code;
}

__device__ __forceinline__ bool dir_range8(const MaxLevels& m, const DKey& q, int64_t& d8a, int64_t& d8b) {
    if (!m.dir && !m.edir_epoch) return false;
    const uint32_t dv = dir_slot(m, q.hi, q.lo);
    if (m.dir) {
        d8a = m.dir[dv];
        d8b = m.dir[dv + 1];
        return true;
    }
    const uint64_t x0 = m.edir[dv], x1 = m.edir[dv + 1];
    d8a = (uint32_t)x0;
    d8b = (uint32_t)x1;
    return (uint32_t)(x0 >> 32) == m.edir_epoch && (uint32_t)(x1 >> 32) == m.edir_epoch;
}

template <bool LONG = false>
__device__ __forceinline__ int64_t group_lower_bound(const Hist& h, const MaxLevels& m, int64_t n, const DKey& q,
                                                     const uint8_t* htail, const uint8_t* qtail, bool& eq) {
    const int gl = threadIdx.x & (kArity - 1);
    const int g0 = threadIdx.x & 63 & ~(kArity - 1);
    eq = false;
    if (n <= 0) return 0;
    QTail qt;
    if constexpr (LONG) load_qtail(qt, q, qtail);
    auto probe = [&](int64_t p, const ulonglong2* kp) -> int {
        if constexpr (LONG) {
            const ulonglong2 k = *kp;
            const uint2 lt = h.lt[p];
            return probe_cmp_long(k, lt, htail, q, qt, qtail);
        } else {
            return probe_cmp(h, p, *kp, htail, q, qtail);
        }
    };
    int64_t sz[kIdxLevels];
    sz[0] = (n + kFan - 1) / kFan;
#pragma unroll
    for (int L = 1; L < kIdxLevels; L++) sz[L] = (sz[L - 1] + kArity - 1) / kArity;
    int top = 0;
    while (top + 1 < kIdxLevels && sz[top] > kArity) top++;
    auto prefix_eq = [&](const ulonglong2& k) { return k.x == q.hi && k.y == q.lo; };
    int64_t c = 0;
    bool bknown = false;
    const bool v_top = gl < sz[top];
    const ulonglong2 e_top = m.skey[top][v_top ? gl : 0];
    bool direct = false;
    int64_t d8a, d8b;
    if (dir_range8(m, q, d8a, d8b)) {
        const int64_t d0 = (d8a + 7) >> 3, d1 = (d8b + 7) >> 3;
        if (d1 - d0 <= 2 * kArity && d1 <= sz[0]) {
            direct = true;
            c = d0;
            bknown = true;
            for (int64_t j0 = d0; j0 < d1; j0 += kArity) {
                const bool v = j0 + gl < d1;
                const ulonglong2 e = m.skey[0][v ? j0 + gl : 0];
                const int k = __popc(gmask(v && prefix_less(e, q)));
                c += k;
                if (k < __popc(gmask(v))) {
                    bknown = !((gmask(v && prefix_eq(e)) >> k) & 1u);
                    break;
                }
            }
        }
    }
    if (!direct) {
        for (int64_t j0 = 0; j0 < sz[top]; j0 += kArity) {
            const bool v = j0 == 0 ? v_top : j0 + gl < sz[top];
            const ulonglong2 e = j0 == 0 ? e_top : m.skey[top][v ? j0 + gl : 0];
            const int k = __popc(gmask(v && prefix_less(e, q)));
            if (top == 0 && k < __popc(gmask(v))) bknown = !((gmask(v && prefix_eq(e)) >> k) & 1u);
            c += k;
            if (k < kArity) break;
        }
        for (int L = top; L > 0; L--) {
            if (c == 0) continue;
            const int64_t base = (int64_t)kArity * (c - 1) + 1;
            const int64_t end = min((int64_t)kArity * c, sz[L - 1]);
            const bool v = base + gl < end;
            const ulonglong2 e = m.skey[L - 1][v ? base + gl : 0];
            const int k = __popc(gmask(v && prefix_less(e, q)));
            if (L == 1 && k < __popc(gmask(v))) bknown = !((gmask(v && prefix_eq(e)) >> k) & 1u);
            c = base + k;
        }
    }
    int64_t b = c;
    for (; !bknown;) {
        const bool v = b + gl < sz[0];
        const ulonglong2 k = m.skey[0][v ? b + gl : 0];
        const uint32_t same = gmask(v && k.x == q.hi && k.y == q.lo);
        const int run = __ffs(~same) - 1;
        b += run;
        if (run < kArity) break;
    }
    int64_t lo = c > 0 ? kFan * (c - 1) + 1 : 0;
    const int64_t hi = min(n, kFan * b);
    if (b == c && m.skey8) {
        const int64_t B = c > 0 ? kFan * (c - 1) : 0;
        const int64_t p8 = B + 8 * gl;
        const bool v8 = p8 < hi;
        int r8 = 1;
        if (v8) r8 = probe(p8, &m.skey8[p8 / 8]);
        const int k8 = __popc(gmask(v8 && r8 < 0));
        const int r_first = __shfl(r8, g0, 64);
        if (k8 == 0) {
            eq = hi > 0 && r_first == 0;
            return 0;
        }
        const int64_t g = B + 8 * (k8 - 1);
        const int64_t gend = min(g + 8, hi);
        const int64_t pk = g + 1 + gl;
        const bool vk = gl < 7 && pk < gend;
        int rk = 1;
        if (vk) rk = probe(pk, &h.key[pk]);
        const int k1 = __popc(gmask(vk && rk < 0));
        const int64_t lb = g + 1 + k1;
        const int r_stop = __shfl(rk, g0 + (k1 < 7 ? k1 : 6), 64);
        const int r_next = __shfl(r8, g0 + (k8 < kArity ? k8 : kArity - 1), 64);
        if (lb < gend)
            eq = r_stop == 0;
        else if (lb < hi)
            eq = r_next == 0;
        return lb;
    }
    int64_t span = hi - lo;
    int64_t stride0 = kFan / kArity;
    while (stride0 * kArity < span) stride0 *= kArity;
    bool eq_cand = false;
    for (int64_t stride = stride0; span > 0; stride = stride > kArity ? stride / kArity : 1) {
        const int64_t p = lo + stride * (gl + 1) - 1;
        const bool v = stride * (gl + 1) <= span && p < hi;
        int r = 1;
        if (v) r = probe(p, &h.key[p]);
        const uint32_t valid = gmask(v);
        const int cnt = __popc(gmask(v && r < 0));
        const int stop = __shfl(r, g0 + (cnt < kArity ? cnt : kArity - 1), 64);
        if (cnt < __popc(valid)) eq_cand = stop == 0;
        lo += stride * cnt;
        span = cnt < __popc(valid) ? stride - 1 : span - stride * cnt;
        if (stride == 1) break;
    }
    if (lo < hi) eq = eq_cand;
    return lo;
}

__device__ __forceinline__ int64_t l3_at(const int64_t* a, int64_t i) {
    int64_t v[kL3Rep];
#pragma unroll
    for (int r = 0; r < kL3Rep; r++) v[r] = a[(i * kL3Rep + r) * kL3Pad];
    int64_t best = v[0];
#pragma unroll
    for (int r = 1; r < kL3Rep; r++) best = v[r] > best ? v[r] : best;
    return best;
}

__device__ __forceinline__ int64_t range_max(const MaxLevels& m, int64_t lo, int64_t hi, int64_t snap) {
    int64_t best = LLONG_MIN;
    for (int L = 0; L < kMaxLevels; L++) {
        const int64_t* a = m.lvl[L];
        if (hi - lo <= 2 * kFan || L == kMaxLevels - 1) {
// ... 2085 lines not shown
    };
    __syncthreads();
    if (threadIdx.x == 0) trace_max(w.trace, kTrResSetup);
    if (in_regs) {
        volatile uint8_t* vst = st;
        __shared__ int s_more2[2];
        if (threadIdx.x == 0) s_more2[0] = s_more2[1] = 0;
        __syncthreads();
        for (;;) {
            if (NW)
                group_minima(vst);
            else
                __syncthreads();
            if (rounds == 0 && threadIdx.x == 0) trace_max(w.trace, kTrResMin1);
            if (threadIdx.x == 0) s_more2[(rounds + 1) & 1] = 0;
            int more = 0;
#pragma unroll
            for (int k = 0; k < kTPer; k++) {
                const int t = tt[k];
                if (t < 0 || vst[t] != kUndecided) continue;
                int p = ep[k];
                const int end = en[k];
                uint8_t res = kUndecided;
                int e = cur[k];
                while (p < end) {
                    const uint8_t sp = e >= T ? group_status(e, t) : vst[e];
                    if (sp != kAborted) {
                        if (sp == kCommitted) res = kAborted;
                        break;
                    }
                    int nx[4];
#pragma unroll
                    for (int u = 0; u < 4; u++) {
                        const int q = p + 1 + u, d = q - ep0[k];
                        nx[u] = q >= end ? 0
                                : d < 4  ? (d == 0 ? f4[k].x : d == 1 ? f4[k].y : d == 2 ? f4[k].z : f4[k].w)
                                         : w.tedges[q];
                    }
                    int adv = 0, ne = 0;
                    bool stop = false;
#pragma unroll
                    for (int u = 0; u < 4; u++) {
                        if (!stop && p + 1 + u < end) {
                            const int x = nx[u];
                            if ((x >= T ? group_status(x, t) : vst[x]) != kAborted) {
                                stop = true;
                                ne = x;
                            } else {
                                adv++;
                            }
                        }
                    }
                    p += 1 + adv;
                    if (p < end) e = stop ? ne : (p - ep0[k] < 4 ? f4[k].w : w.tedges[p]);
                }
                if (p == end) res = kCommitted;
                ep[k] = p;
                cur[k] = e;
                if (res != kUndecided)
                    vst[t] = res;
                else
                    more = 1;
            }
            if (more) s_more2[rounds & 1] = 1;
            __syncthreads();
            if (rounds == 0 && threadIdx.x == 0) trace_max(w.trace, kTrResRound1);
            const int again = s_more2[rounds & 1];
            rounds++;
            if (!again) break;
        }
    } else if (!overflow) {
        for (int t = threadIdx.x; t < T; t += blockDim.x)
            w.eptr[t] = use_pre ? w.pre_ep[t] : (b.roff[t] < b.roff[t + 1] ? w.eoff[b.roff[t]] : 0);
        volatile uint8_t* vst = st;
        for (;;) {
            if (threadIdx.x == 0) s_more = 0;
            if (NW) group_minima(vst);
            __syncthreads();
            int more = 0;
            for (int t = threadIdx.x; t < T; t += blockDim.x) {
                if (vst[t] != kUndecided) continue;
                int p = w.eptr[t];
                uint8_t res = kUndecided;
                if (use_pre) {
                    const int end = w.pre_end[t];
                    while (p < end) {
                        const int e = w.tedges[p];
                        const uint8_t sp = e >= T ? group_status(e, t) : vst[e];
                        if (sp == kAborted) {
                            p++;
                            continue;
                        }
                        if (sp == kCommitted) res = kAborted;
                        break;
                    }
                    if (p == end) res = kCommitted;
                    w.eptr[t] = p;
                    if (res != kUndecided)
                        vst[t] = res;
                    else
                        more = 1;
                    continue;
                }
                int r = b.roff[t];
                const int rend = b.roff[t + 1];
                for (; r < rend; r++) {
                    const int s0 = w.eoff[r], s1 = s0 + w.ecur[r];
                    if (p < s0) p = s0;
                    while (p < s1) {
                        int e[4];
#pragma unroll
                        for (int u = 0; u < 4; u++) e[u] = p + u < s1 ? w.edges[p + u] : -1;
                        int u = 0;
                        uint8_t sp = kAborted;
                        for (; u < 4 && p + u < s1; u++) {
                            sp = (unsigned)e[u] < (unsigned)T ? vst[e[u]] : (e[u] >= T && NW ? group_status(e[u], t) : kAborted);
                            if (sp != kAborted) break;
                        }
                        p += u;
                        if (sp != kAborted) {
                            if (sp == kCommitted) res = kAborted;
                            break;
                        }
                    }
                    if (p < s1) break;
                }
                if (r == rend) res = kCommitted;
                w.eptr[t] = p;
                if (res != kUndecided)
                    vst[t] = res;
                else
                    more = 1;
            }
            if (more) s_more = 1;
            __syncthreads();
            rounds++;
            if (!s_more) break;
            __syncthreads();
        }
    } else {
        const int E = 2 * (b.R + b.W);
        for (int i = threadIdx.x; i <= E / 64; i += blockDim.x) w.mcs_bits[i] = 0;
        __syncthreads();
        for (int t = 0; t < T; t++) {
            if (st[t] != kUndecided) continue;
            int conflict_at = INT_MAX;
            for (int r = b.roff[t]; r < b.roff[t + 1]; r++) {
                const int a = w.pos[2 * r], e = w.pos[2 * r + 1];
                int hit = 0;
                if (a < e) {
                    for (int word = (a >> 6) + threadIdx.x; word <= ((e - 1) >> 6); word += blockDim.x) {
                        uint64_t m = ((volatile uint64_t*)w.mcs_bits)[word];
                        const int lo = word << 6;
                        if (a > lo) m &= ~0ull << (a - lo);
                        if (e < lo + 64) m &= (e - lo >= 64) ? ~0ull : ((1ull << (e - lo)) - 1);
                        if (m) hit = 1;
                    }
                }
                if (__syncthreads_or(hit)) {
                    conflict_at = r - b.roff[t];
                    break;
                }
            }
            if (conflict_at == INT_MAX) {
                for (int x = b.woff[t]; x < b.woff[t + 1]; x++) {
                    const int g = b.R + x;
                    const int a = w.pos[2 * g], e = w.pos[2 * g + 1];
                    if (a < e) {
                        for (int word = (a >> 6) + threadIdx.x; word <= ((e - 1) >> 6); word += blockDim.x) {
                            uint64_t m = ~0ull;
                            const int lo = word << 6;
                            if (a > lo) m &= ~0ull << (a - lo);
                            if (e < lo + 64) m &= (e - lo >= 64) ? ~0ull : ((1ull << (e - lo)) - 1);
                            atomicOr((unsigned long long*)&w.mcs_bits[word], (unsigned long long)m);
                        }
                    }
                    __syncthreads();
                }
            }
            if (threadIdx.x == 0) {
                st[t] = conflict_at == INT_MAX ? kCommitted : kAborted;
                if (conflict_at != INT_MAX) w.first_conf[t] = conflict_at;
            }
            __syncthreads();
        }
        rounds = -1;
    }
    __syncthreads();
    if (threadIdx.x == 0) trace_max(w.trace, kTrResRounds);
    if (NW && !overflow && w.report) {
        group_minima(st);
        for (int j = threadIdx.x; j < NW; j += blockDim.x) w.gminc[j] = minComm[j];
    }
    if (in_regs) {
#pragma unroll
        for (int k = 0; k < kTPer; k++) {
            const int t = tt[k];
            if (t >= 0) {
                const uint8_t x = st[t];
                w.status[t] = x;
                vout[t] = x == kCommitted ? 2 : 0;
                if (w.vdev) w.vdev[t] = x == kCommitted ? 2 : 0;
            }
        }
    } else {
        for (int t = threadIdx.x; t < T; t += blockDim.x) {
            w.status[t] = st[t];
            vout[t] = verdict_byte(b, t, st[t]);
            if (w.vdev) w.vdev[t] = verdict_byte(b, t, st[t]);
        }
    }
    if (threadIdx.x == 0) sc->rounds = rounds;
    (void)hs;
    if (threadIdx.x == 0) trace_max(w.trace, kTrResEnd);
}

__global__ __launch_bounds__(kScanThreads) void k_combine(BatchDev b, Work w) {
    __shared__ uint32_t sv[1][scan_pad(kCombineP)];
    __shared__ uint32_t swave[1][kScanThreads / 64];
    __shared__ uint32_t sbase[1];
    __shared__ int s_tile;
    if (w.bsc->n_edges == 0 && !w.bsc->edge_overflow) return;
    if (threadIdx.x == 0) s_tile = atomicAdd(w.scan[kScanCover].counter, 1);
    __syncthreads();
    const int64_t n = 2 * (int64_t)b.W;
    const int64_t ntiles = n > 0 ? (n + kCombineTile - 1) / kCombineTile : 1;
    if (s_tile >= ntiles) return;
    scan_tile<1, CoverScan, kCombineP>(CoverScan{w, b, 1}, n, s_tile, ntiles, w.scan[kScanCover], sv, swave, sbase);
    scan_tile<1, SegNumScan, kCombineP>(SegNumScan{w}, n, s_tile, ntiles, w.scan[kScanSegNum], sv, swave, sbase);
}

__global__ __launch_bounds__(kBlock) void k_intra_report(BatchDev b, Work w) {
    const BatchScalars* sc = w.bsc;
    const int r = blockIdx.x * blockDim.x + threadIdx.x;
    if (r >= b.R || sc->edge_overflow) return;
    const int t = b.rowner[r];
    if (!(b.flags[t] & kFlagReport) || w.hist_conf[t] || w.status[t] != kAborted) return;
    for (int p = w.eoff[r]; p < w.eoff[r] + w.ecur[r]; p++) {
        const int e = w.edges[p];
        if (((unsigned)e < (unsigned)b.T && w.status[e] == kCommitted) ||
            (w.groups && e >= b.T && w.gminc[e - b.T] < t)) {
            atomicMin(&w.first_conf[t], r - b.roff[t]);
            return;
        }
    }
}

constexpr size_t kResolveLdsMax = 160 * 1024 - 1024;

void init_kernel_attributes() {
    (void)hipFuncSetAttribute((const void*)k_resolve<5>, hipFuncAttributeMaxDynamicSharedMemorySize, (int)kResolveLdsMax);
    (void)hipFuncSetAttribute((const void*)k_resolve<8>, hipFuncAttributeMaxDynamicSharedMemorySize, (int)kResolveLdsMax);
}

void launch_resolve(hipStream_t s, const BatchDev& b, const Work& w, bool report, uint8_t* verdict_out, Scalars* sc) {
    if (b.T == 0) {
        fdb_launch(k_set_i64, dim3(1), dim3(64), 0, s, &w.bsc->n_segments, (int64_t)0);
        return;
    }
    const int64_t pre_grid = std::max<int64_t>(((int64_t)b.T * 64 + kBlock - 1) / kBlock,
                                               (2 * (int64_t)b.W + kCombineTile - 1) / kCombineTile);
    fdb_launch(k_resolve_pre, dim3((unsigned)pre_grid), dim3(kBlock), 0, s, b, w, verdict_out);
    const size_t lds = ((size_t)b.T + 15) / 16 * 16 + (w.groups ? 8 * (size_t)b.W : 0);
    Work wr = w;
    wr.report = report ? 1 : 0;
    t_group = kGroupEdges;
    fdb_launch(b.T <= 5 * kWG ? k_resolve<5> : k_resolve<8>, dim3(1), dim3(kWG), (uint32_t)lds, s, b, wr, verdict_out,
               sc);
    fdb_launch(k_combine, dim3((unsigned)std::max<int64_t>(1, (2 * (int64_t)b.W + kCombineTile - 1) / kCombineTile)),
               dim3(kScanThreads), 0, s, b, w);
    if (b.R && report) fdb_launch(k_intra_report, dim3((b.R + kBlock - 1) / kBlock), dim3(kBlock), 0, s, b, w);
    t_group = 0;
}

struct Epilogue {
    uint8_t* verdict_out;
    uint32_t* flag;
    uint32_t seq;
    unsigned long long* trace;
    int32_t T;
    int compacted, gc_ran;
    uint8_t* zero8;
    int64_t zero8_n;
    uint8_t* zero8r;
    int64_t zero8r_n;
    int32_t* zero32b;
    int64_t zero32_n;
    uint64_t* zero64[kNumScans + 1];
    int64_t zero64_n[kNumScans + 1];
    uint64_t* zero_bc;
    int64_t zero_bc_n;
    int32_t* zero_rank;
    int64_t zero_rank_n;
    BatchScalars* bsc;
    int64_t* nd_out;
};


__device__ __forceinline__ const DKey& seg_key(const BatchDev& b, const Work& w, int pos, int end) {
    const int g = (int)item_range(w.pmeta[pos]);
    return b.keys[2 * g + end];
}

constexpr int kDeltaTile = 256;
constexpr int kBaseTile = 4096;

__device__ __forceinline__ void fill_tile_first(int32_t* tile_first, const int64_t* lo, int64_t j, int tile) {
    const int64_t t0 = j > 0 ? lo[j - 1] / tile + 1 : 0;
    for (int64_t t = t0; t <= lo[j] / tile; t++) tile_first[t] = (int32_t)j;
}
__device__ __forceinline__ void fill_tile_first_tail(int32_t* tile_first, const int64_t* lo, int64_t U, int64_t n,
                                                     int tile) {
    const int64_t t0 = U > 0 ? lo[U - 1] / tile + 1 : 0;
    for (int64_t t = t0; t <= n / tile + 1; t++) tile_first[t] = (int32_t)U;
}

constexpr int kSegWideMinW = 24576;
constexpr int seg_per(bool long_keys, bool wide) { return long_keys || !wide ? 63 : 127; }
constexpr int seg_lanes(bool, bool wide) { return wide ? 1 : kArity; }
constexpr int seg_threads(bool long_keys, bool wide) {
    return 2 * seg_lanes(long_keys, wide) * (seg_per(long_keys, wide) + 1);
}
inline bool seg_wide(int64_t W, bool long_keys) { return long_keys || W >= kSegWideMinW; }
inline int64_t seg_tiles(int64_t W, bool long_keys, bool wide) { return (W > 0 ? W : 1) / seg_per(long_keys, wide) + 1; }
inline int64_t seg_prep_tiles(int64_t W) { return (W > 0 ? W : 1) / 63 + 1; }

template <bool LONG, bool WIDE>
__global__ __launch_bounds__(seg_threads(LONG, WIDE)) void k_seg_prep(BatchDev b, Work w, Hist h, MaxLevels hm,
                                                                      const uint8_t* htail, Scalars* sc, TierIO io,
                                                                      int64_t* lvl3, int64_t lvl3_n, int64_t* lvl2,
                                                                      int64_t lvl2_n) {
    constexpr int SP = seg_per(LONG, WIDE);
    constexpr int LL = seg_lanes(LONG, WIDE);
    constexpr int NSW = (SP + 1 + 63) / 64;
    __shared__ int64_t s_lo[SP + 1];
    __shared__ uint32_t s_val[3][SP + 1];
    __shared__ uint32_t s_wsum[3][NSW];
    __shared__ uint32_t s_base[3];
    __shared__ int s_tile;
    const int64_t gt = (int64_t)blockIdx.x * blockDim.x + threadIdx.x;
    for (int64_t i = gt; i < lvl3_n * kL3Rep; i += (int64_t)gridDim.x * blockDim.x) lvl3[i * kL3Pad] = LLONG_MIN;
    for (int64_t i = gt; i < lvl2_n; i += (int64_t)gridDim.x * blockDim.x) lvl2[i] = LLONG_MIN;
    if (threadIdx.x == 0) s_tile = atomicAdd(w.scan[kScanSegSum].counter, 1);
    __syncthreads();
    const int tile = s_tile;
    const int U = (int)w.bsc->n_segments;
    const int ntiles = U > 0 ? (U + SP - 1) / SP : 1;
    if (tile >= ntiles) return;
    const int64_t n = *io.n_in;
    const int q = threadIdx.x / (2 * LL), role = (threadIdx.x / LL) & 1;
    const int sg = tile * SP + (q < SP ? q : -1);
    const bool live = sg >= 0 && sg < U && (q < SP || role == 0);
    int64_t pos = 0;
    bool eq = false;
    DKey kb{}, ke{};
    if (live) {
        kb = seg_key(b, w, w.seg_b[sg], 0);
        ke = seg_key(b, w, w.seg_e[sg], 1);
        const DKey& key = role ? ke : kb;
        if constexpr (LONG) {
            static_assert(WIDE, "long-key batches take the one-lane layout");
            QTail qt;
            load_qtail(qt, key, b.tail);
            pos = lane_lower_bound_long(h, hm, n, key, qt, htail, b.tail, eq);
        } else if constexpr (WIDE) {
            pos = lane_lower_bound(h, hm, n, key, htail, b.tail, eq);
        } else {
            pos = group_lower_bound<false>(h, hm, n, key, htail, b.tail, eq);
        }
    }
    const int lane = threadIdx.x & 63, wid = threadIdx.x >> 6;
    const int64_t hi = __shfl(pos, (lane + LL) & 63, 64);
    const int exact = __shfl((int)eq, (lane + LL) & 63, 64);
    if (threadIdx.x % (2 * LL) == 0) {
        if (q == SP) {
            s_lo[0] = live ? pos : 0;
        } else if (live) {
            const int64_t lo = pos;
            const bool glue = sg + 1 < U && dkey_cmp(seg_key(b, w, w.seg_b[sg + 1], 0), b.tail, ke, b.tail) == 0;
            const bool endins = !exact && !glue;
            w.seg_lo[sg] = lo;
            w.seg_hi[sg] = hi;
            w.seg_endins[sg] = endins ? 1 : 0;
            w.seg_vend[sg] = hi > 0 ? h.ver[hi - 1] : kHole;
            s_lo[q + 1] = lo;
            s_val[0][q] = (uint32_t)(hi - lo);
            s_val[1][q] = endins ? 2 : 1;
            s_val[2][q] = tail_units(kb.len) + (endins ? tail_units(ke.len) : 0u);
        } else {
            s_val[0][q] = s_val[1][q] = s_val[2][q] = 0;
        }
    }
    __syncthreads();
    uint32_t ex[3] = {0, 0, 0};
    if (wid < NSW) {
#pragma unroll
        for (int c = 0; c < 3; c++) {
            const uint32_t v = threadIdx.x < SP ? s_val[c][threadIdx.x] : 0u;
            uint32_t x = v;
#pragma unroll
            for (int o = 1; o < 64; o <<= 1) {
                const uint32_t y = __shfl_up(x, o, 64);
                if (lane >= o) x += y;
            }
            ex[c] = x - v;
            if (lane == 63) s_wsum[c][wid] = x;
        }
    }
    __syncthreads();
    if (threadIdx.x < 64) {
        uint32_t btot[3];
#pragma unroll
        for (int c = 0; c < 3; c++) {
            uint32_t t = 0;
#pragma unroll
            for (int k = 0; k < NSW; k++) t += s_wsum[c][k];
            btot[c] = t;
        }
        tile_lookback<3>(w.scan[kScanSegSum], tile, btot, s_base);
    }
    __syncthreads();
    if (wid < NSW) {
        const int k = threadIdx.x;
#pragma unroll
        for (int c = 0; c < 3; c++) {
            uint32_t before = s_base[c];
            for (int v = 0; v < wid; v++) before += s_wsum[c][v];
            ex[c] += before;
        }
        const int j = tile * SP + k;
        if (k < SP && j < U) {
            w.seg_rem[j] = ex[0];
            w.seg_ins[j] = ex[1];
            w.seg_tlen[j] = ex[2];
            const int64_t t0 = j > 0 ? s_lo[k] / kDeltaTile + 1 : 0;
            for (int64_t t = t0; t <= s_lo[k + 1] / kDeltaTile; t++) w.tile_first[t] = j;
        }
        if (tile == ntiles - 1 && j == U && k <= SP) {
            const uint32_t r = ex[0], in = ex[1], tl = ex[2];
            w.seg_rem[U] = r;
            w.seg_ins[U] = in;
            w.seg_tlen[U] = tl;
            const int64_t t0 = U > 0 ? s_lo[k] / kDeltaTile + 1 : 0;
            for (int64_t t = t0; t <= n / kDeltaTile + 1; t++) w.tile_first[t] = U;
            *io.before = n;
            *io.removed = r;
            *io.n_out = n - (int64_t)r + (int64_t)in;
            sc->tail_next = sc->tail_used + 8 * (int64_t)tl;
        }
    }
}

constexpr int kSegLds = 1024;

typedef uint64_t u64x2 __attribute__((ext_vector_type(2)));
template <bool NT, class T>
__device__ __forceinline__ T stream_load(const T* p) {
    if constexpr (NT) return __builtin_nontemporal_load(p);
    else return *p;
}
template <bool NT, class T>
__device__ __forceinline__ void stream_store(T* p, const T& v) {
    if constexpr (NT) __builtin_nontemporal_store(v, p);
    else *p = v;
}

template <class Ins, int TILE, bool NT = false>
__global__ __launch_bounds__(kBlock) void k_merge_copy(Segs g, Hist src, Hist dst, const int64_t* n_in,
                                                       const int64_t* U_ptr, Ins ins) {
    __shared__ int64_t s_lo[kSegLds + 1], s_hi[kSegLds + 1], s_shift[kSegLds + 1];
    __shared__ int s_j0, s_cnt;
    const int64_t n = *n_in;
    const int64_t U = *U_ptr;
    __shared__ int s_ins0, s_ins1;
    for (int64_t i0 = (int64_t)blockIdx.x * TILE; i0 <= n; i0 += (int64_t)gridDim.x * TILE) {
        const int64_t i1 = min(n, i0 + TILE);
        if (threadIdx.x == 0) {
            const int64_t t = i0 / TILE;
            s_ins0 = g.tile_first[t];
            s_ins1 = g.tile_first[t + 1];
            s_j0 = s_ins0;
            s_cnt = s_ins1 - s_ins0;
        }
        __syncthreads();
        const int ja = s_j0, cnt = s_cnt;
        int top = 0;
        if (cnt > 0 && cnt <= kSegLds)
            for (top = 1; 2 * top <= cnt;) top *= 2;
        if (cnt <= kSegLds) {
            for (int k = threadIdx.x; k <= cnt; k += blockDim.x) {
                const int j = ja - 1 + k;
                s_lo[k] = j >= 0 ? g.lo[j] : LLONG_MIN;
                s_hi[k] = j >= 0 ? g.hi[j] : LLONG_MIN;
                s_shift[k] = g.ins[j + 1] - g.rem[j + 1];
            }
        }
        __syncthreads();
        if (cnt <= kSegLds) {
            constexpr int kPer = TILE / kBlock < 8 ? TILE / kBlock : 8;
            for (int64_t c0 = i0; c0 < i1; c0 += kPer * kBlock) {
                int64_t dsto[kPer];
#pragma unroll
                for (int k = 0; k < kPer; k++) {
                    const int64_t i = c0 + k * kBlock + threadIdx.x;
                    int sl = 0;
#pragma unroll
                    for (int step = kSegLds; step > 0; step >>= 1) {
                        if (step > top) continue;
                        const int mid = sl + step;
                        if (mid <= cnt && s_lo[mid] <= i) sl = mid;
                    }
                    const bool keep = i < i1 && !(i >= s_lo[sl] && i < s_hi[sl]);
                    dsto[k] = keep ? i + s_shift[sl] : -1;
                }
                u64x2 kk[kPer];
                uint64_t lt[kPer], vv[kPer];
#pragma unroll
                for (int k = 0; k < kPer; k++) {
                    const int64_t i = c0 + k * kBlock + threadIdx.x;
                    const int64_t j = dsto[k] >= 0 ? i : i0;
                    kk[k] = stream_load<NT>(reinterpret_cast<const u64x2*>(src.key) + j);
                    lt[k] = stream_load<NT>(reinterpret_cast<const uint64_t*>(src.lt) + j);
                    vv[k] = stream_load<NT>(reinterpret_cast<const uint64_t*>(src.ver) + j);
                }
#pragma unroll
                for (int k = 0; k < kPer; k++) {
                    if (dsto[k] >= 0) {
                        stream_store<NT>(reinterpret_cast<u64x2*>(dst.key) + dsto[k], kk[k]);
                        stream_store<NT>(reinterpret_cast<uint64_t*>(dst.lt) + dsto[k], lt[k]);
                        stream_store<NT>(reinterpret_cast<uint64_t*>(dst.ver) + dsto[k], vv[k]);
                    }
                }
            }
        } else {
            for (int64_t i = i0 + threadIdx.x; i < i1; i += blockDim.x) {
                int64_t lo = 0, hi = U;
                while (lo < hi) {
                    int64_t mid = (lo + hi) >> 1;
                    if (g.lo[mid] <= i) lo = mid + 1; else hi = mid;
                }
                const int64_t j = lo - 1;
                if (j >= 0 && i >= g.lo[j] && i < g.hi[j]) continue;
                const int64_t o = i + g.ins[j + 1] - g.rem[j + 1];
                dst.key[o] = src.key[i];
                dst.lt[o] = src.lt[i];
                dst.ver[o] = src.ver[i];
            }
        }
        __syncthreads();
    }
    for (int64_t sg = (int64_t)blockIdx.x * blockDim.x + threadIdx.x; sg < U; sg += (int64_t)gridDim.x * blockDim.x)
        ins((int)sg, dst, g.lo[sg] - g.rem[sg] + g.ins[sg]);
}

struct BatchIns {
    BatchDev b;
    const uint32_t* pmeta;
    const int32_t *seg_b, *seg_e;
    const int64_t *tlen, *vend;
    const uint8_t* endins;
    uint8_t* htail;
    const Scalars* sc;
    int64_t now;
    __device__ const DKey& key(int pos, int end) const {
        return b.keys[2 * (int)item_range(pmeta[pos]) + end];
    }
    __device__ void operator()(int s, Hist dst, int64_t o) const {
        int64_t tu = sc->tail_used / 8 + tlen[s];
        const DKey kb = key(seg_b[s], 0);
        uint32_t tb = 0;
        if (kb.len > 16) {
            tb = (uint32_t)tu;
            copy_tail_words(htail + 8 * tu, b.tail + kb.tail, kb.len - 16);
            tu += tail_units(kb.len);
        }
        dst.key[o] = make_ulonglong2(kb.hi, kb.lo);
        dst.lt[o] = make_uint2(kb.len, tb);
        dst.ver[o] = now;
        if (endins[s]) {
            const DKey ke = key(seg_e[s], 1);
            uint32_t te = 0;
            if (ke.len > 16) {
                te = (uint32_t)tu;
                copy_tail_words(htail + 8 * tu, b.tail + ke.tail, ke.len - 16);
            }
            dst.key[o + 1] = make_ulonglong2(ke.hi, ke.lo);
            dst.lt[o + 1] = make_uint2(ke.len, te);
            dst.ver[o + 1] = vend[s];
        }
    }
};

static Segs batch_segs(const Work& w) { return Segs{w.seg_lo, w.seg_hi, w.seg_rem, w.seg_ins, w.tile_first}; }

static unsigned copy_tiles(int64_t grid_hint_n, int tile, int64_t max_inserts = 0) {
    int64_t tiles = (grid_hint_n + 1 + tile - 1) / tile;
    tiles = std::max<int64_t>(tiles, (max_inserts + kBlock - 1) / kBlock);
    if (tiles < 1) tiles = 1;
    if (tiles > 8192) tiles = 8192;
    return (unsigned)tiles;
}

static Epilogue make_epilogue(const BatchDev& b, const Work& w, int compacted, int gc_ran, uint8_t* verdict_out,
                              uint32_t* flag, uint32_t seq, int sort_nb, int sort_samples) {
    Epilogue ep{};
    ep.flag = flag;
    ep.seq = seq;
    ep.trace = w.trace;
    ep.verdict_out = verdict_out;
    ep.T = b.T;
    ep.compacted = compacted;
    ep.gc_ran = gc_ran;
    ep.zero8 = w.hist_conf;
    ep.zero8_n = b.T;
    ep.zero8r = w.rconf;
    ep.zero8r_n = b.R;
    ep.zero32b = w.ecur;
    ep.zero32_n = b.R;
    const int64_t G = (int64_t)b.R + b.W;
    const int64_t used[kNumScans] = {scan_granules(G, 3, kEdgeScanP), 3 * seg_prep_tiles(b.W),
                                     compacted ? w.scan_gran[kScanCompact] : 0, gc_ran ? w.scan_gran[kScanGc] : 0,
                                     scan_granules(2 * (int64_t)b.W, 1, kCombineP),
                                     scan_granules(2 * (int64_t)b.W, 1, kCombineP)};
    ep.zero64[0] = w.scan_arena;
    ep.zero64_n[0] = kNumScans;
    for (int k = 0; k < kNumScans; k++) {
        ep.zero64[k + 1] = w.scan[k].granules;
        ep.zero64_n[k + 1] = std::min<int64_t>(used[k], w.scan_gran[k]);
    }
    ep.zero_bc = w.scnt;
    ep.zero_bc_n = sort_nb;
    ep.zero_rank = w.srank;
    ep.zero_rank_n = sort_samples;
    ep.bsc = w.bsc;
    return ep;
}

void launch_merge(hipStream_t s, const BatchDev& b, const Work& w, const Hist& src, const MaxLevels& srcm,
                  const Hist& dst, const MaxLevels& dstm, const int64_t* nd_src, uint8_t* htail, Scalars* sc,
                  int64_t now, int64_t lvl3_n, int64_t lvl2_n, int64_t grid_hint_n, hipEvent_t copy_begin,
                  hipEvent_t copy_end, bool long_keys) {
    const TierIO io{nd_src, &sc->nd_next, &sc->d_before, &sc->d_rem};
    const bool wide = seg_wide(b.W, long_keys);
    fdb_launch(long_keys ? k_seg_prep<true, true> : (wide ? k_seg_prep<false, true> : k_seg_prep<false, false>),
               dim3((unsigned)seg_tiles(b.W, long_keys, wide)), dim3(seg_threads(long_keys, wide)), 0, s, b, w, src, srcm, htail, sc, io, dstm.lvl[3], lvl3_n,
               dstm.lvl[2], lvl2_n);
    fdb_event(LaunchList::kTimingRecord, copy_begin, s);
    BatchIns ins{};
    ins.b = b;
    ins.pmeta = w.pmeta;
    ins.seg_b = w.seg_b;
    ins.seg_e = w.seg_e;
    ins.tlen = w.seg_tlen;
    ins.vend = w.seg_vend;
    ins.endins = w.seg_endins;
    ins.htail = htail;
    ins.sc = sc;
    ins.now = now;
    fdb_launch((k_merge_copy<BatchIns, kDeltaTile>), dim3(copy_tiles(grid_hint_n, kDeltaTile, b.W)), dim3(kBlock), 0,
               s, batch_segs(w), src, dst, nd_src, &w.bsc->n_segments, ins);
    fdb_event(LaunchList::kTimingRecord, copy_end, s);
}


template <int MODE>
__global__ __launch_bounds__(kBlock) void k_compact_search(Hist base, MaxLevels basem, Hist delta,
                                                           const uint8_t* htail, const int64_t* nb_ptr,
                                                           const int64_t* nd_ptr, int64_t hdr, Work w, int64_t* lvl3,
                                                           int64_t lvl3_n, int64_t* lvl2, int64_t lvl2_n) {
    const int64_t gt = (int64_t)blockIdx.x * blockDim.x + threadIdx.x;
    for (int64_t i = gt; i < lvl3_n * kL3Rep; i += (int64_t)gridDim.x * blockDim.x) lvl3[i * kL3Pad] = LLONG_MIN;
    for (int64_t i = gt; i < lvl2_n; i += (int64_t)gridDim.x * blockDim.x) lvl2[i] = LLONG_MIN;
    const int64_t j = gt;
    const int64_t nd = *nd_ptr;
    if (j >= nd) return;
    const int64_t nb = *nb_ptr;
    const ulonglong2 k = delta.key[j];
    const uint2 lt = delta.lt[j];
    DKey q;
    q.hi = k.x;
    q.lo = k.y;
    q.len = lt.x;
    q.tail = 0;
    bool exact;
    const uint8_t* qtail = hist_tail(htail, lt.y);
    int64_t lo;
    if constexpr (MODE == 1) {
        lo = lane_lower_bound(base, basem, nb, q, htail, qtail, exact);
    } else {
        QTail qt;
        load_qtail(qt, q, qtail);
        lo = lane_lower_bound_long(base, basem, nb, q, qt, htail, qtail, exact);
    }
    const int64_t dv = delta.ver[j];
    w.c_lo[j] = lo;
    w.c_exact[j] = exact ? 1 : 0;
    w.c_val[j] = dv != kHole ? dv : (lo > 0 ? base.ver[lo - 1] : hdr);
}

struct CompactSumScan {
    Segs g;
    const int64_t* dver;
    const uint8_t* exact;
    TierIO io;
    const int64_t* nd_ptr;
    int tile;
    __device__ int64_t hi_of(int64_t j) const {
        if (dver[j] == kHole) return g.lo[j];
        return j + 1 < *nd_ptr ? g.lo[j + 1] : *io.n_in;
    }
    __device__ void load(int64_t j, uint32_t (&v)[2]) const {
        v[0] = (uint32_t)(hi_of(j) - g.lo[j]);
        v[1] = (dver[j] != kHole || !exact[j]) ? 1u : 0u;
    }
    __device__ void store(int64_t j, const uint32_t (&ex)[2]) const {
        g.hi[j] = hi_of(j);
        g.rem[j] = ex[0];
        g.ins[j] = ex[1];
        fill_tile_first(g.tile_first, g.lo, j, tile);
    }
    __device__ void finish(const uint32_t (&tot)[2]) const {
        const int64_t U = *nd_ptr, n = *io.n_in;
        g.rem[U] = tot[0];
        g.ins[U] = tot[1];
        fill_tile_first_tail(g.tile_first, g.lo, U, n, tile);
        *io.before = n;
        *io.removed = tot[0];
        *io.n_out = n - (int64_t)tot[0] + (int64_t)tot[1];
    }
};

struct CompactIns {
    Hist delta;
    const int64_t *val, *ins;
    __device__ void operator()(int s, Hist dst, int64_t o) const {
        if (ins[s + 1] == ins[s]) return;
        dst.key[o] = delta.key[s];
        dst.lt[o] = delta.lt[s];
        dst.ver[o] = val[s];
    }
};

void launch_compact(hipStream_t s, const Work& w, const Hist& base, const MaxLevels& basem, const Hist& delta,
                    const Hist& dst, const uint8_t* htail, Scalars* sc, int64_t header_version, int64_t lvl3_n,
                    int64_t lvl2_n, int64_t delta_hint_n, int64_t grid_hint_n, hipEvent_t copy_begin,
                    hipEvent_t copy_end, int mode, int base_tile, bool nt) {
    int64_t blocks = (delta_hint_n + kBlock - 1) / kBlock;
    if (blocks < 1) blocks = 1;
    if (mode == 1)
        fdb_launch(k_compact_search<1>, dim3((unsigned)blocks), dim3(kBlock), 0, s, base, basem, delta, htail,
                   &sc->n, &sc->nd_next, header_version, w, basem.lvl[3], lvl3_n, basem.lvl[2], lvl2_n);
    else
        fdb_launch(k_compact_search<2>, dim3((unsigned)blocks), dim3(kBlock), 0, s, base, basem, delta, htail,
                   &sc->n, &sc->nd_next, header_version, w, basem.lvl[3], lvl3_n, basem.lvl[2], lvl2_n);
    const Segs g{w.c_lo, w.c_hi, w.c_rem, w.c_ins, w.tile_first};
    const TierIO io{&sc->n, &sc->n_next, &sc->c_before, &sc->c_rem};
    const int tile = base_tile == 1024 || base_tile == 2048 ? base_tile : kBaseTile;
    launch_scan<2>(s, CompactSumScan{g, delta.ver, w.c_exact, io, &sc->nd_next, tile}, &sc->nd_next,
                   delta_hint_n + 1, w.scan[kScanCompact]);
    fdb_event(LaunchList::kTimingRecord, copy_begin, s);
    const dim3 grid(copy_tiles(grid_hint_n, tile, delta_hint_n + 1));
    const CompactIns ins{delta, w.c_val, w.c_ins};
    auto k = tile == 1024 ? (nt ? k_merge_copy<CompactIns, 1024, true> : k_merge_copy<CompactIns, 1024>)
             : tile == 2048 ? (nt ? k_merge_copy<CompactIns, 2048, true> : k_merge_copy<CompactIns, 2048>)
                            : (nt ? k_merge_copy<CompactIns, kBaseTile, true> : k_merge_copy<CompactIns, kBaseTile>);
    fdb_launch(k, grid, dim3(kBlock), 0, s, g, base, dst, &sc->n, &sc->nd_next, ins);
    fdb_event(LaunchList::kTimingRecord, copy_end, s);
}


__device__ __forceinline__ bool gc_keep(const Hist& h, int64_t i, int64_t v, int64_t hdr) {
    const int64_t pv = i ? h.ver[i - 1] : hdr;
    return h.ver[i] >= v || pv >= v;
}

struct GcScan {
    Hist src, dst;
    const uint8_t* tsrc;
    uint8_t* tdst;
    int64_t v, hdr;
    Scalars* sc;
    __device__ void load(int64_t i, uint32_t (&x)[2]) const {
        const bool keep = gc_keep(src, i, v, hdr);
        x[0] = keep ? 1u : 0u;
        x[1] = keep ? tail_units(src.lt[i].x) : 0u;
    }
    __device__ void store(int64_t i, const uint32_t (&ex)[2]) const {
        if (!gc_keep(src, i, v, hdr)) return;
        const int64_t o = ex[0];
        uint2 lt = src.lt[i];
        if (lt.x > 16u) {
            const uint64_t* a = (const uint64_t*)hist_tail(tsrc, lt.y);
            uint64_t* d = (uint64_t*)hist_tail(tdst, ex[1]);
            for (uint32_t k = 0; k < tail_units(lt.x); k++) d[k] = a[k];
            lt.y = ex[1];
        }
        dst.key[o] = src.key[i];
        dst.lt[o] = lt;
        dst.ver[o] = src.ver[i];
    }
    __device__ void finish(const uint32_t (&tot)[2]) const {
        sc->n_gc = tot[0];
        sc->tail_gc = 8 * (int64_t)tot[1];
    }
};

void launch_gc(hipStream_t s, const Work& w, const Hist& src, const Hist& dst, const uint8_t* tsrc, uint8_t* tdst,
               Scalars* sc, int64_t oldest, int64_t header_version, int64_t grid_hint_n) {
    launch_scan<2>(s, GcScan{src, dst, tsrc, tdst, oldest, header_version, sc}, &sc->n_next, grid_hint_n,
                   w.scan[kScanGc]);
}

int64_t scan_arena_words(int64_t T, int64_t R, int64_t W, int64_t hist_cap, int64_t delta_cap) {
    (void)T;
    const int64_t E = 2 * (R + W);
    (void)E;
    return kNumScans + scan_granules(R + W, 3, kEdgeScanP) + 3 * seg_prep_tiles(W) + scan_granules(delta_cap + 1, 2) +
           scan_granules(hist_cap, 2) + 2 * scan_granules(2 * W, 1, kCombineP);
}

void carve_scans(Work& w, int64_t T, int64_t R, int64_t W, int64_t hist_cap, int64_t delta_cap) {
    (void)T;
    const int64_t E = 2 * (R + W);
    uint64_t* a = w.scan_arena;
    (void)E;
    const int64_t gran[kNumScans] = {scan_granules(R + W, 3, kEdgeScanP), 3 * seg_prep_tiles(W),
                                     scan_granules(delta_cap + 1, 2), scan_granules(hist_cap, 2),
                                     scan_granules(2 * W, 1, kCombineP), scan_granules(2 * W, 1, kCombineP)};
    uint64_t* g = a + kNumScans;
    for (int k = 0; k < kNumScans; k++) {
        w.scan[k].counter = (int*)(a + k);
        w.scan[k].granules = g;
        w.scan_gran[k] = gran[k];
        g += gran[k];
    }
    w.scan_words = g - a;
}


__device__ __forceinline__ const ShareHeader* share_at(const RouteArgs& a, int p) {
    return (const ShareHeader*)(a.shares + (int64_t)p * a.stride);
}

__global__ void k_route_wait(const uint32_t* ready, uint32_t value, uint32_t* err, uint64_t timeout_ticks) {
    if (threadIdx.x != 0) return;
    if (ready) {
        const uint64_t t0 = wall_clock64();
        for (;;) {
            if (__hip_atomic_load(ready, __ATOMIC_RELAXED, __HIP_MEMORY_SCOPE_AGENT) == value) {
                __builtin_amdgcn_fence(__ATOMIC_ACQUIRE, "agent");
                *err = 0;
                return;
            }
            if (wall_clock64() - t0 > timeout_ticks) break;
            __builtin_amdgcn_s_sleep(16);
        }
        *err = 1;
        return;
    }
    *err = 0;
}

__global__ __launch_bounds__(kBlock) void k_route_mark(RouteArgs a) {
    if (*a.wait_err) return;
    const int p = blockIdx.y;
    const ShareHeader* h = share_at(a, p);
    const int j = blockIdx.x * blockDim.x + threadIdx.x;
    if (j >= h->R + h->W || j >= a.rstride) return;
    const uint8_t* base = (const uint8_t*)h;
    const DKey* keys = (const DKey*)(base + h->off_keys);
    const uint8_t* tb = base + h->off_tail;
    const DKey kb = keys[2 * j], ke = keys[2 * j + 1];
    bool in = !a.has_hi || dkey_cmp(kb, tb, a.hi, a.btail) < 0;
    if (in && a.has_lo) in = dkey_cmp(ke, tb, a.lo, a.btail) > 0 || dkey_cmp(kb, tb, a.lo, a.btail) >= 0;
    const uint32_t tl = (kb.len > 16u ? kb.len - 16u : 0u) + (ke.len > 16u ? ke.len - 16u : 0u);
    a.info[(int64_t)p * a.rstride + j] =
        (in ? 1u : 0u) | ((kb.len > 19u || ke.len > 19u) ? 2u : 0u) | ((kb.len > 24u || ke.len > 24u) ? 4u : 0u) | (tl << 8);
}

struct RouteScan {
    RouteArgs a;
    __device__ const ShareHeader* at(int64_t i, int& p, int& t, int64_t& gid) const {
        p = (int)(i / a.tcap);
        t = (int)(i - (int64_t)p * a.tcap);
        if (*a.wait_err) return nullptr;
        const ShareHeader* h = share_at(a, p);
        if (t >= h->T) return nullptr;
        gid = t;
        for (int q = 0; q < p; q++) gid += share_at(a, q)->T;
        return h;
    }
    __device__ bool visit(int64_t i, uint32_t (&v)[6], bool& any, int& p, int& t, int64_t& gid,
                          const ShareHeader*& h) const {
        h = at(i, p, t, gid);
        if (!h) return false;
        const uint8_t* base = (const uint8_t*)h;
        const int32_t* roff = (const int32_t*)(base + h->off_roff);
        const int32_t* woff = (const int32_t*)(base + h->off_woff);
        const uint32_t* info = a.info + (int64_t)p * a.rstride;
        uint32_t nr = 0, nw = 0, tl = 0, g19 = 0, g24 = 0;
        const int r0 = roff[t], r1 = roff[t + 1], w0 = h->R + woff[t], w1 = h->R + woff[t + 1];
        for (int j = r0; j < r1; j++) {
            const uint32_t x = info[j];
            if (!(x & 1u)) continue;
            nr++;
            tl += x >> 8;
            g19 += (x >> 1) & 1u;
            g24 += (x >> 2) & 1u;
        }
        for (int j = w0; j < w1; j++) {
            const uint32_t x = info[j];
            if (!(x & 1u)) continue;
            nw++;
            tl += x >> 8;
            g19 += (x >> 1) & 1u;
            g24 += (x >> 2) & 1u;
        }
        any = nr + nw > 0;
        if (!any) return true;
        v[0] = 1;
        v[1] = nr;
        v[2] = nw;
        v[3] = tl;
        v[4] = g19;
        v[5] = g24;
        return true;
    }
    __device__ void load(int64_t i, uint32_t (&v)[6]) const {
        bool any;
        int p, t;
        int64_t gid;
        const ShareHeader* h;
        visit(i, v, any, p, t, gid, h);
    }
    __device__ void store(int64_t i, const uint32_t (&ex)[6]) const {
        uint32_t v[6] = {0, 0, 0, 0, 0, 0};
        bool any;
        int p, t;
        int64_t gid;
        const ShareHeader* h;
        if (!visit(i, v, any, p, t, gid, h)) return;
        if (a.out_zero && gid < a.out_n) a.out_zero[gid] = 0;
        const int lt = (int)ex[0];
        const bool fits = any && lt < a.cap_T;
        if (gid < a.inv_n) a.inv[gid] = fits ? lt : -1;
        a.txpre[i] = make_int4(fits ? lt : -1, (int)ex[1], (int)ex[2], (int)ex[3]);
        if (!fits) return;
        const uint8_t* base = (const uint8_t*)h;
        a.snap[lt] = ((const int64_t*)(base + h->off_snap))[t];
        a.flags[lt] = 0;
        a.roff[lt] = (int32_t)ex[1];
        a.woff[lt] = (int32_t)ex[2];
    }
    __device__ void finish(const uint32_t (&tot)[6]) const {
        RouteResult r{};
        if (!*a.wait_err)
            for (int q = 0; q < a.n_shares; q++) r.global_T += share_at(a, q)->T;
        r.T = (int32_t)tot[0];
        r.R = (int32_t)tot[1];
        r.W = (int32_t)tot[2];
        r.tail_bytes = tot[3];
        r.n_gt19 = (int32_t)tot[4];
        r.n_gt24 = (int32_t)tot[5];
        r.error = (r.T > a.cap_T || r.R > a.cap_R || r.W > a.cap_W || (int64_t)tot[3] > a.cap_tail) ? 1 : 0;
        if (*a.wait_err) r.error = 2;
        if (!r.error && a.out_zero && r.global_T != a.out_n) r.error = 3;
        if (!r.error) {
            a.roff[r.T] = r.R;
            a.woff[r.T] = r.W;
        }
        *a.dres = r;
        *a.res = r;
    }
};

__global__ __launch_bounds__(kBlock) void k_route_write(RouteArgs a) {
    const RouteResult res = *a.dres;
    if (res.error) return;
    const int p = blockIdx.y;
    const ShareHeader* h = share_at(a, p);
    const int j = blockIdx.x * blockDim.x + threadIdx.x;
    if (j >= h->R + h->W) return;
    const uint32_t* info = a.info + (int64_t)p * a.rstride;
    const uint32_t x = info[j];
    if (!(x & 1u)) return;
    const uint8_t* base = (const uint8_t*)h;
    const int t = ((const int32_t*)(base + h->off_owner))[j];
    const int4 pre = a.txpre[(int64_t)p * a.tcap + t];
    if (pre.x < 0) return;
    const int32_t* roff = (const int32_t*)(base + h->off_roff);
    const int32_t* woff = (const int32_t*)(base + h->off_woff);
    const bool is_read = j < h->R;
    const int first = is_read ? roff[t] : h->R + woff[t];
    uint32_t rank = 0, tail = (uint32_t)pre.w;
    if (!is_read)
        for (int q = roff[t]; q < roff[t + 1]; q++) tail += (info[q] & 1u) ? info[q] >> 8 : 0u;
    for (int q = first; q < j; q++) {
        const uint32_t y = info[q];
        if (!(y & 1u)) continue;
        rank++;
        tail += y >> 8;
    }
    const DKey* keys = (const DKey*)(base + h->off_keys);
    const uint8_t* tb = base + h->off_tail;
    const int64_t slot = is_read ? (int64_t)pre.y + rank : (int64_t)res.R + pre.z + rank;
    if (is_read) {
        a.rown[pre.y + rank] = pre.x;
        if (a.read_ids) a.read_ids[pre.y + rank] = j - roff[t];
    } else {
        a.wown[pre.z + rank] = pre.x;
    }
#pragma unroll
    for (int e = 0; e < 2; e++) {
        DKey k = keys[2 * j + e];
        const uint32_t n = k.len > 16u ? k.len - 16u : 0u;
        if (n) {
            const uint8_t* src = tb + k.tail;
            for (uint32_t q = 0; q < n; q++) a.tail[tail + q] = src[q];
            k.tail = tail;
            tail += n;
        } else {
            k.tail = 0;
        }
        a.keys[2 * slot + e] = k;
    }
}

__global__ __launch_bounds__(kBlock) void k_route_too_old(BatchDev b, int64_t oldest) {
    const int t = blockIdx.x * blockDim.x + threadIdx.x;
    if (t >= b.T) return;
    if (b.roff[t + 1] > b.roff[t] && b.snap[t] < oldest) b.flags[t] |= kFlagTooOld;
}

void launch_route_too_old(hipStream_t s, const BatchDev& b, int64_t oldest) {
    if (b.T <= 0) return;
    fdb_launch(k_route_too_old, dim3((unsigned)((b.T + kBlock - 1) / kBlock)), dim3(kBlock), 0, s, b, oldest);
}

int64_t route_scan_words(int64_t n_elems) { return 8 + scan_granules(n_elems, 6, kRouteScanP); }

void launch_route(hipStream_t s, const RouteArgs& a, ScanState st) {
    const dim3 grid((unsigned)std::max<int64_t>(1, (a.rstride + kBlock - 1) / kBlock), (unsigned)a.n_shares);
    fdb_launch(k_route_wait, dim3(1), dim3(64), 0, s, a.ready, a.ready_value, a.wait_err, a.wait_ticks);
    fdb_launch(k_route_mark, grid, dim3(kBlock), 0, s, a);
    launch_scan<6, kRouteScanP>(s, RouteScan{a}, nullptr, (int64_t)a.n_shares * a.tcap, st);
    fdb_launch(k_route_write, grid, dim3(kBlock), 0, s, a);
}


constexpr int kEpiWaves = 4;
constexpr int kEpiThreads = 64 * kEpiWaves;
constexpr int kEpiBlocks = 4;
constexpr int64_t kEpiSpan = (int64_t)kEpiWaves * kEpiBlocks * kFan;
static_assert(kFan % kEpiBlocks == 0, "a wave's blocks share one level-2 entry");

constexpr int kScWords = (int)(sizeof(Scalars) / 8);
constexpr int kBscWords = (int)(sizeof(BatchScalars) / 8);
static_assert(sizeof(Scalars) % 8 == 0 && sizeof(BatchScalars) % 8 == 0, "scalars move in 8-byte words");
static_assert(kScWords <= 32 && kBscWords <= 32, "one lane per word, Scalars in lanes 0-31, BatchScalars in 32-63");
constexpr int sc_word(size_t off) { return (int)(off / 8); }

template <bool BASE>
__global__ __launch_bounds__(kEpiThreads) void k_epilogue(MaxLevels m, Scalars* sc, const int64_t* n_levels, Epilogue ep) {
    if (threadIdx.x == 0) trace_min(ep.trace, kTrEpiBegin);
    const int lane = threadIdx.x & 63, wid = threadIdx.x >> 6;
    uint64_t pre = 0;
    if (ep.verdict_out && blockIdx.x == 0 && wid == 0) {
        if (lane < kScWords)
            pre = reinterpret_cast<const uint64_t*>(sc)[lane];
        else if (lane >= 32 && lane < 32 + kBscWords)
            pre = reinterpret_cast<const uint64_t*>(ep.bsc)[lane - 32];
    }
    int64_t n0;
    if (n_levels)
        n0 = *n_levels;
    else if (ep.compacted)
        n0 = ep.gc_ran ? sc->n_gc : sc->n_next;
    else
        n0 = sc->nd_next;
    const int64_t n1 = (n0 + kFan - 1) / kFan, nwv = (n1 + kEpiBlocks - 1) / kEpiBlocks;
    for (int64_t wv = (int64_t)blockIdx.x * kEpiWaves + wid; wv < nwv; wv += (int64_t)gridDim.x * kEpiWaves) {
        const int64_t b1_0 = wv * kEpiBlocks;
        int64_t v[kEpiBlocks];
#pragma unroll
        for (int q = 0; q < kEpiBlocks; q++) {
            const int64_t i = (b1_0 + q) * kFan + lane;
            v[q] = i < n0 ? m.lvl[0][i] : LLONG_MIN;
        }
        const int64_t b1l = b1_0 + lane;
        ulonglong2 sk = make_ulonglong2(0, 0);
        if (lane < kEpiBlocks && b1l < n1) sk = m.keys[b1l * kFan];
        constexpr int kE8 = kEpiBlocks * kFan / 8;
        static_assert(kE8 <= 64, "one skey8 entry per lane");
        const int64_t n8 = (n0 + 7) / 8, e8_0 = b1_0 * (kFan / 8);
        ulonglong2 k8 = make_ulonglong2(0, 0);
        ulonglong2 prev_k = make_ulonglong2(0, 0);
        if (lane < kE8 && e8_0 + lane < n8) {
            k8 = m.keys[(e8_0 + lane) * 8];
            m.skey8[e8_0 + lane] = k8;
        }
        if (m.edir_epoch && lane == 0 && e8_0 > 0 && e8_0 < n8) prev_k = m.keys[(e8_0 - 1) * 8];
        int64_t mine = LLONG_MIN;
#pragma unroll
        for (int q = 0; q < kEpiBlocks; q++) {
            int64_t x = v[q];
#pragma unroll
            for (int o = 32; o > 0; o >>= 1) {
                const int64_t y = __shfl_xor(x, o, 64);
                x = y > x ? y : x;
            }
            if (lane == q) mine = x;
        }
        if (lane < kEpiBlocks && b1l < n1) {
            m.lvl[1][b1l] = mine;
            m.skey[0][b1l] = sk;
            int64_t d = b1l, off = 0;
            for (int L = 1; L < kIdxLevels && d % kArity == 0; L++) {
                off += idx_level_cap(m.idx_cap, L - 1);
                d /= kArity;
                m.skey[0][off + d] = sk;
            }
        }
        if (m.edir_epoch) {
            const int64_t e = e8_0 + lane;
            const bool live = lane < kE8 && e < n8;
            const int64_t c_l = live ? (int64_t)dir_slot(m, k8.x, k8.y) : -1;
            int64_t a = __shfl_up(c_l, 1, 64);
            if (lane == 0) a = e8_0 > 0 && live ? (int64_t)dir_slot(m, prev_k.x, prev_k.y) : -1;
            const uint64_t tag = (uint64_t)m.edir_epoch << 32;
            const int64_t z = live ? (c_l < a + kDirRun ? c_l : a + kDirRun) : a;
            const bool wide = live && z - a > 4;
            if (live && !wide)
                for (int64_t v = a + 1; v <= z; v++) m.edir[v] = tag | (uint64_t)e;
            for (uint64_t wm = __ballot(wide); wm; wm &= wm - 1) {
                const int q = __builtin_ctzll(wm);
                const int64_t aq = __shfl(a, q, 64), zq = __shfl(z, q, 64);
                for (int64_t v = aq + 1 + lane; v <= zq; v += 64) m.edir[v] = tag | (uint64_t)(e8_0 + q);
            }
            const uint64_t lm = __ballot(live && e == n8 - 1);
            if (lm) {
                const int q = __builtin_ctzll(lm);
                const int64_t cq = __shfl(c_l, q, 64);
                const int64_t top = (int64_t)m.dir_top + 1, z2 = cq + kDirRun < top ? cq + kDirRun : top;
                for (int64_t v = cq + 1 + lane; v <= z2; v += 64) m.edir[v] = tag | (uint64_t)n8;
            }
        }
        int64_t x = lane < kEpiBlocks ? mine : LLONG_MIN;
#pragma unroll
        for (int o = 1; o < kEpiBlocks; o <<= 1) {
            const int64_t y = __shfl_xor(x, o, 64);
            x = y > x ? y : x;
        }
#ifndef FDBCS_EPI_EXP
#define FDBCS_EPI_EXP 0
#endif
        if (lane == 0 && b1_0 < n1) {
            if (!(FDBCS_EPI_EXP & 1)) atomicMax((long long*)&m.lvl[2][b1_0 / kFan], (long long)x);
            int64_t* l3 = &m.lvl[3][((b1_0 / ((int64_t)kFan * kFan)) * kL3Rep + (int64_t)(blockIdx.x % kL3Rep)) * kL3Pad];
            if (!(FDBCS_EPI_EXP & 2) && x > __hip_atomic_load(l3, __ATOMIC_RELAXED, __HIP_MEMORY_SCOPE_AGENT))
                atomicMax((long long*)l3, (long long)x);
        }
    }
    if (!ep.verdict_out) return;
    if (threadIdx.x == 0) trace_max(ep.trace, kTrEpiLevels);
    const int64_t tid = (int64_t)blockIdx.x * blockDim.x + threadIdx.x, stride = (int64_t)gridDim.x * blockDim.x;
    for (int64_t i = tid; i < ep.zero8_n; i += stride) ep.zero8[i] = 0;
    for (int64_t i = tid; i < ep.zero8r_n; i += stride) ep.zero8r[i] = 0;
    for (int64_t i = tid; i < ep.zero32_n; i += stride) ep.zero32b[i] = 0;
#pragma unroll
    for (int k = 0; k <= kNumScans; k++)
        for (int64_t i = tid; i < ep.zero64_n[k]; i += stride) ep.zero64[k][i] = 0;
    for (int64_t i = tid; i < ep.zero_bc_n; i += stride) {
        ep.zero_bc[(size_t)kCntStride * i] = 0;
        ep.zero_bc[(size_t)kCntStride * i + 1] = 0;
    }
    for (int64_t i = tid; i < ep.zero_rank_n; i += stride) ep.zero_rank[i] = 0;
    __syncthreads();
    if (threadIdx.x == 0) trace_max(ep.trace, kTrEpiZero);
    if (blockIdx.x != 0) return;
    if (wid == 0) {
        auto scw = [&](size_t off) -> int64_t { return (int64_t)__shfl(pre, sc_word(off), 64); };
        auto bsw = [&](size_t off) -> uint64_t { return __shfl(pre, 32 + sc_word(off), 64); };
        auto bs32 = [&](size_t off) -> uint32_t { return (uint32_t)(bsw(off) >> (8 * (off % 8))); };
        const int64_t n_new = !ep.compacted ? scw(offsetof(Scalars, n))
                                            : (ep.gc_ran ? scw(offsetof(Scalars, n_gc)) : scw(offsetof(Scalars, n_next)));
        const int64_t nd_new = ep.compacted ? 0 : scw(offsetof(Scalars, nd_next));
        const int64_t tail_new = ep.gc_ran ? scw(offsetof(Scalars, tail_gc)) : scw(offsetof(Scalars, tail_next));
        const int64_t edges = bs32(offsetof(BatchScalars, edge_overflow)) ? -1 : (int64_t)bsw(offsetof(BatchScalars, n_edges));
        const uint32_t dbg = bs32(offsetof(BatchScalars, debug_error)), rounds = bs32(offsetof(BatchScalars, rounds));
        const uint32_t big = bs32(offsetof(BatchScalars, sort_big));
        const int64_t nseg = (int64_t)bsw(offsetof(BatchScalars, n_segments));
        const int64_t nd_slot = ep.nd_out ? ep.nd_out - sc->ndb : -1;
        static_assert(offsetof(Scalars, debug_error) % 8 == 0 &&
                          offsetof(Scalars, intra_rounds) == offsetof(Scalars, debug_error) + 4 &&
                          offsetof(Scalars, sort_big) % 8 == 0 && offsetof(Scalars, intra_edges) % 8 == 0,
                      "Scalars word packing the host copy assumes");
        if (lane < kScWords) {
            uint64_t x = pre;
            if (lane == sc_word(offsetof(Scalars, n))) x = (uint64_t)n_new;
            if (lane == sc_word(offsetof(Scalars, nd))) x = (uint64_t)nd_new;
            if (lane == sc_word(offsetof(Scalars, tail_used))) x = (uint64_t)tail_new;
            if (nd_slot >= 0 && nd_slot < 2 && lane == sc_word(offsetof(Scalars, ndb)) + nd_slot) x = (uint64_t)nd_new;
            if (lane == sc_word(offsetof(Scalars, debug_error))) x = (uint64_t)dbg | (uint64_t)rounds << 32;
            if (lane == sc_word(offsetof(Scalars, intra_edges))) x = (uint64_t)edges;
            if (lane == sc_word(offsetof(Scalars, sort_big))) x = (x & ~0xffffffffull) | big;
            if (lane == sc_word(offsetof(Scalars, n_segments))) x = (uint64_t)nseg;
            reinterpret_cast<uint64_t*>(ep.verdict_out + verdict_scalars_offset(ep.T))[lane] = x;
        }
        if (lane == 0) {
            sc->n = n_new;
            sc->nd = nd_new;
            if (ep.nd_out) *ep.nd_out = nd_new;
            sc->tail_used = tail_new;
            ep.bsc->debug_error = 0;
            ep.bsc->ovf_n = 0;
            ep.bsc->n_undec = 0;
            ep.bsc->sort_big = 0;
        }
    }
    __syncthreads();
    if (threadIdx.x == 0) trace_max(ep.trace, kTrEpiHost);
    __threadfence_system();
    __syncthreads();
    if (threadIdx.x == 0) {
        trace_max(ep.trace, kTrEpiFence);
        __hip_atomic_store(ep.flag, ep.seq, __ATOMIC_RELEASE, __HIP_MEMORY_SCOPE_SYSTEM);
    }
}

__global__ __launch_bounds__(kBlock) void k_copy_bytes(uint8_t* __restrict__ dst, const uint8_t* __restrict__ src,
                                                       int64_t n) {
    for (int64_t i = (int64_t)blockIdx.x * blockDim.x + threadIdx.x; i < n; i += (int64_t)gridDim.x * blockDim.x)
        dst[i] = src[i];
}

void launch_copy_bytes(hipStream_t s, void* dst, const void* src, int64_t n) {
    if (n <= 0) return;
    int64_t blocks = (n + kBlock - 1) / kBlock;
    blocks = blocks > 256 ? 256 : blocks;
    fdb_launch(k_copy_bytes, dim3((unsigned)blocks), dim3(kBlock), 0, s, (uint8_t*)dst, (const uint8_t*)src, n);
}

__global__ __launch_bounds__(kBlock) void k_conflict_output(BatchDev b, const uint8_t* __restrict__ status,
                                                            const int32_t* __restrict__ inv, int64_t n,
                                                            uint8_t* __restrict__ out) {
    for (int64_t g = (int64_t)blockIdx.x * blockDim.x + threadIdx.x; g < n; g += (int64_t)gridDim.x * blockDim.x) {
        const int t = inv[g];
        uint8_t c = 0;
        if (t >= 0) c = (uint8_t)(2 - verdict_byte(b, t, status[t]));
        out[g] = c;
    }
}

void launch_conflict_output(hipStream_t s, const BatchDev& b, const Work& w, const int32_t* inv, int64_t n,
                            uint8_t* out) {
    if (n <= 0) return;
    int64_t blocks = (n + kBlock - 1) / kBlock;
    blocks = blocks > 1024 ? 1024 : blocks;
    fdb_launch(k_conflict_output, dim3((unsigned)blocks), dim3(kBlock), 0, s, b, (const uint8_t*)w.status, inv, n,
               out);
}

__global__ void k_hold(const volatile uint32_t* release) {
    if (threadIdx.x != 0) return;
    for (int64_t spin = 0; spin < ((int64_t)1 << 22) && *release == 0u; spin++) __builtin_amdgcn_s_sleep(64);
}

void launch_hold(hipStream_t s, const uint32_t* release) {
    fdb_launch(k_hold, dim3(1), dim3(64), 0, s, (const volatile uint32_t*)release);
}

__global__ void k_lvl3_reset(int64_t* lvl3, int64_t n, int64_t* lvl2, int64_t n2) {
    for (int64_t i = threadIdx.x; i < n * kL3Rep; i += blockDim.x) lvl3[i * kL3Pad] = LLONG_MIN;
    for (int64_t i = threadIdx.x; i < n2; i += blockDim.x) lvl2[i] = LLONG_MIN;
}

static int64_t epilogue_grid(int64_t hint_n, int64_t extra) {
    int64_t g = (hint_n + kEpiSpan - 1) / kEpiSpan;
    const int64_t ge = (extra + kEpiThreads - 1) / kEpiThreads;
    g = g > ge ? g : ge;
    g = g < 1 ? 1 : g;
    return g > 4096 ? 4096 : g;
}

__global__ __launch_bounds__(kBlock) void k_directory(MaxLevels m, const int64_t* np) {
    const int v = blockIdx.x * blockDim.x + threadIdx.x;
    if (v > (int)m.dir_top + 1) return;
    const ulonglong2* keys = m.keys;
    int32_t* dir = const_cast<int32_t*>(m.dir);
    const int64_t S = (*np + 7) / 8;
    int64_t lo = 0, hi = S;
    while (lo < hi) {
        const int64_t mid = (lo + hi) >> 1;
        const ulonglong2 k = keys[mid * 8];
        if ((int64_t)dir_slot(m, k.x, k.y) < v)
            lo = mid + 1;
        else
            hi = mid;
    }
    dir[v] = (int32_t)lo;
}

static void launch_directory(hipStream_t s, const MaxLevels& m, const int64_t* n) {
    if (!m.dir) return;
    fdb_launch(k_directory, dim3((m.dir_top + 1 + kBlock) / kBlock), dim3(kBlock), 0, s, m, n);
}

void launch_rangemax(hipStream_t s, const MaxLevels& m, Scalars* sc, const int64_t* n, int64_t lvl3_n,
                     int64_t lvl2_n, int64_t grid_hint_n) {
    launch_directory(s, m, n);
    fdb_launch(k_lvl3_reset, dim3(1), dim3(kBlock), 0, s, m.lvl[3], lvl3_n, m.lvl[2], lvl2_n);
    Epilogue ep{};
    ep.trace = nullptr;
    fdb_launch(k_epilogue<true>, dim3((unsigned)epilogue_grid(grid_hint_n, 0)), dim3(kEpiThreads), 0, s, m, sc, n, ep);
}

void launch_epilogue(hipStream_t s, const BatchDev& b, const Work& w, const MaxLevels& m, Scalars* sc,
                     int compacted, int gc_ran, uint8_t* verdict_out, uint32_t* flag,
                     uint32_t seq, int64_t grid_hint_n, int64_t* nd_out, int sort_nb, int sort_samples) {
    Epilogue ep = make_epilogue(b, w, compacted, gc_ran, verdict_out, flag, seq, sort_nb, sort_samples);
    ep.nd_out = nd_out;
    if (compacted) launch_directory(s, m, gc_ran ? &sc->n_gc : &sc->n_next);
    int64_t extra = std::max<int64_t>(b.R, b.T);
    for (int k = 0; k <= kNumScans; k++) extra = std::max(extra, ep.zero64_n[k]);
    if (compacted)
        fdb_launch(k_epilogue<true>, dim3((unsigned)epilogue_grid(grid_hint_n, extra)), dim3(kEpiThreads), 0, s, m, sc,
                   (const int64_t*)nullptr, ep);
    else
        fdb_launch(k_epilogue<false>, dim3((unsigned)epilogue_grid(grid_hint_n, extra)), dim3(kEpiThreads), 0, s, m, sc,
                   (const int64_t*)nullptr, ep);
}


__device__ __forceinline__ int64_t export_prefix64(uint32_t a, uint32_t b) {
    const uint64_t lower = 8ull * b;
    return (int64_t)(lower + (uint32_t)(a - (uint32_t)lower));
}

__device__ __forceinline__ int64_t export_clamp(int64_t v, int64_t floor) {
    return (floor == kHole || v >= floor) ? v : floor - 1;
}

template <int MODE>
__global__ __launch_bounds__(kBlock) void k_export_search(Hist base, MaxLevels basem, Hist delta,
                                                          const uint8_t* htail, int64_t nb, int64_t nd, int64_t hdr,
                                                          int64_t* d_pos, int64_t* d_val) {
    const int64_t j = (int64_t)blockIdx.x * blockDim.x + threadIdx.x;
    if (j >= nd) return;
    const ulonglong2 k = delta.key[j];
    const uint2 lt = delta.lt[j];
    DKey q;
    q.hi = k.x;
    q.lo = k.y;
    q.len = lt.x;
    q.tail = 0;
    bool exact = false;
    const uint8_t* qtail = hist_tail(htail, lt.y);
    int64_t lb;
    if constexpr (MODE == 1) {
        lb = lane_lower_bound(base, basem, nb, q, htail, qtail, exact);
    } else {
        QTail qt;
        load_qtail(qt, q, qtail);
        lb = lane_lower_bound_long(base, basem, nb, q, qt, htail, qtail, exact);
    }
    const int64_t dv = delta.ver[j];
    d_pos[j] = j + lb;
    d_val[j] = dv != kHole ? dv : exact ? base.ver[lb] : lb > 0 ? base.ver[lb - 1] : hdr;
}

__device__ __forceinline__ int64_t export_bound(const Hist& h, int64_t n, const uint8_t* htail, const DKey& q,
                                                const uint8_t* qtail, bool upper) {
    int64_t lo = 0, hi = n;
    while (lo < hi) {
        const int64_t mid = lo + (hi - lo) / 2;
        const int c = hist_cmp(h, mid, htail, q, qtail);
        if (c < 0 || (upper && c == 0))
            lo = mid + 1;
        else
            hi = mid;
    }
    return lo;
}

__global__ __launch_bounds__(64) void k_export_bounds(ExportArgs a) {
    __shared__ int64_t r[4];
    const int t = threadIdx.x;
    if (t < 4) {
        const bool is_hi = t >= 2, is_delta = t & 1;
        const int64_t n = is_delta ? a.nd : a.nb;
        if (is_hi ? a.has_hi : a.has_lo)
            r[t] = export_bound(is_delta ? a.delta : a.base, n, a.htail, is_hi ? a.hi : a.lo, a.btail, !is_hi);
        else
            r[t] = is_hi ? n : 0;
    }
    __syncthreads();
    if (t != 0) return;
    int64_t h = a.hdr;
    if (r[0] > 0) h = a.base.ver[r[0] - 1];
    if (r[1] > 0) {
        const int64_t dv = a.delta.ver[r[1] - 1];
        if (dv != kHole) h = dv;
    }
    const int64_t m_lo = r[0] + r[1], m_hi = r[2] + r[3];
    a.words[kXwLo] = m_lo;
    a.words[kXwHi] = m_hi > m_lo ? m_hi : m_lo;
    a.words[kXwHeader] = export_clamp(h, a.floor);
}

template <class G>
__device__ __forceinline__ void export_put_key(uint8_t* d, uint32_t n, uint32_t nw, const G& get) {
    uint32_t head = (uint32_t)((8u - ((uintptr_t)d & 7u)) & 7u);
    if (head > n) head = n;
    uint64_t cur = nw ? get(0u) : 0ull;
    for (uint32_t b = 0; b < head; b++) d[b] = (uint8_t)(cur >> (8u * b));
    const uint32_t sh = 8u * head, nfull = (n - head) >> 3;
    uint64_t* dw = (uint64_t*)(d + head);
    for (uint32_t q = 0; q < nfull; q++) {
        const uint64_t next = q + 1u < nw ? get(q + 1u) : 0ull;
        dw[q] = sh ? (cur >> sh) | (next << (64u - sh)) : cur;
        cur = next;
    }
    for (uint32_t b = head + 8u * nfull; b < n; b++) d[b] = (uint8_t)(get(b >> 3) >> (8u * (b & 7u)));
}

__global__ __launch_bounds__(kBlock) void k_export_tile_starts(ExportArgs a) {
    const int64_t tile = (int64_t)blockIdx.x * blockDim.x + threadIdx.x;
    const int64_t m_lo = a.words[kXwLo], n = a.words[kXwHi] - m_lo;
    const int64_t ntiles = n > 0 ? (n + kScanTile - 1) / kScanTile : 1;
    if (tile >= ntiles) return;
    const int64_t mfirst = m_lo + tile * kScanTile - (tile > 0 ? 1 : 0);
    int64_t tb = 0, th = a.nd;
    while (tb < th) {
        const int64_t mid = tb + (th - tb) / 2;
        if (a.d_pos[mid] < mfirst)
            tb = mid + 1;
        else
            th = mid;
    }
    a.tile_tb[tile] = tb;
}

constexpr int kExpWin = kScanTile + 2;

struct ExportScan {
    ExportArgs a;
    const int64_t* s_val;
    const int64_t* s_src;
    int64_t tile0;
    int* err;
    __device__ bool keep(int e) const { return s_val[e + 1] != s_val[e]; }
    __device__ void load(int64_t i, uint32_t (&v)[3]) const {
        const int e = (int)(i - tile0);
        uint32_t len = 0;
        const bool kp = keep(e);
        if (kp) {
            const int64_t src = s_src[e];
            len = src >= 0 ? a.base.lt[src].x : a.delta.lt[~src].x;
        }
        v[0] = kp ? 1u : 0u;
        v[1] = len;
        v[2] = len >> 3;
    }
    __device__ void store(int64_t i, const uint32_t (&ex)[3]) const {
        const int e = (int)(i - tile0);
        if (!keep(e)) return;
        const int64_t o = ex[0], P = export_prefix64(ex[1], ex[2]);
        const int64_t src = s_src[e];
        const Hist& h = src >= 0 ? a.base : a.delta;
        const int64_t p = src >= 0 ? src : ~src;
        const ulonglong2 k = h.key[p];
        const uint2 lt = h.lt[p];
        a.versions[o] = s_val[e + 1];
        a.offsets[o] = P;
        if (P + (int64_t)lt.x > a.bytes_cap) {
            atomicOr(err, 8);
            return;
        }
        const uint64_t w0 = __builtin_bswap64(k.x), w1 = __builtin_bswap64(k.y);
        const uint64_t* tw = (const uint64_t*)hist_tail(a.htail, lt.x > 16u ? lt.y : 0u);
        export_put_key(a.bytes + P, lt.x, (lt.x + 7u) >> 3,
                       [&](uint32_t q) { return q == 0u ? w0 : q == 1u ? w1 : tw[q - 2u]; });
    }
    __device__ void finish(const uint32_t (&tot)[3]) const {
        const int64_t P = export_prefix64(tot[1], tot[2]);
        a.words[kXwN] = tot[0];
        a.words[kXwBytes] = P;
        a.offsets[tot[0]] = P;
    }
};

__global__ __launch_bounds__(kScanThreads) void k_export_scan(ExportArgs a, ScanState st) {
    __shared__ uint32_t sv[3][kScanPad];
    __shared__ uint32_t swave[3][kScanThreads / 64];
    __shared__ uint32_t sbase[3];
    __shared__ int s_tile;
    __shared__ int64_t s_pos[kExpWin];
    __shared__ int64_t s_val[kScanTile + 1];
    __shared__ int64_t s_src[kScanTile];
    const int64_t m_lo = a.words[kXwLo], n = a.words[kXwHi] - m_lo;
    if (threadIdx.x == 0) s_tile = atomicAdd(st.counter, 1);
    __syncthreads();
    const int tile = s_tile;
    const int64_t ntiles = n > 0 ? (n + kScanTile - 1) / kScanTile : 1;
    if (tile >= ntiles) return;
    const int64_t tile0 = (int64_t)tile * kScanTile;
    const int pre = tile > 0 ? 1 : 0;
    const int64_t mfirst = m_lo + tile0 - pre;
    int64_t rest = n - tile0;
    const int cnt = (int)(rest < kScanTile ? rest : kScanTile) + pre;
    const int64_t tb = a.tile_tb[tile];
    for (int q = threadIdx.x; q < kExpWin; q += kScanThreads) s_pos[q] = tb + q < a.nd ? a.d_pos[tb + q] : LLONG_MAX;
    __syncthreads();
    for (int k = threadIdx.x; k < cnt; k += kScanThreads) {
        const int64_t m = mfirst + k;
        int l = 0, h = kExpWin;
        while (l < h) {
            const int mid = (l + h) >> 1;
            if (s_pos[mid] <= m)
                l = mid + 1;
            else
                h = mid;
        }
        const int64_t t = tb + l;
        int64_t v, src;
        if (l > 0 && s_pos[l - 1] == m) {
            src = ~(t - 1);
            v = a.d_val[t - 1];
        } else {
            src = m - t;
            if (src < 0 || src >= a.nb) {
                atomicOr(st.error, 4);
                src = a.nb > 0 ? 0 : ~(int64_t)0;
            }
            const int64_t dv = t > 0 ? a.delta.ver[t - 1] : kHole;
            v = dv != kHole ? dv : src >= 0 ? a.base.ver[src] : a.hdr;
        }
        const int slot = k + 1 - pre;
        s_val[slot] = export_clamp(v, a.floor);
        if (slot > 0) s_src[slot - 1] = src;
    }
    if (tile == 0 && threadIdx.x == 0) s_val[0] = a.words[kXwHeader];
    __syncthreads();
    const ExportScan f{a, s_val, s_src, tile0, st.error};
    scan_tile<3>(f, n, tile, ntiles, st, sv, swave, sbase);
}

int64_t export_tiles(int64_t n) { return n > 0 ? (n + kScanTile - 1) / kScanTile : 1; }

void launch_export(hipStream_t s, const ExportArgs& a, const MaxLevels& basem, uint64_t* granules, int mode) {
    if (a.nd > 0) {
        const dim3 grid((unsigned)((a.nd + kBlock - 1) / kBlock));
        if (mode == 1)
            fdb_launch(k_export_search<1>, grid, dim3(kBlock), 0, s, a.base, basem, a.delta, a.htail, a.nb, a.nd, a.hdr,
                       a.d_pos, a.d_val);
        else
            fdb_launch(k_export_search<2>, grid, dim3(kBlock), 0, s, a.base, basem, a.delta, a.htail, a.nb, a.nd, a.hdr,
                       a.d_pos, a.d_val);
    }
    fdb_launch(k_export_bounds, dim3(1), dim3(64), 0, s, a);
    const int64_t tiles = export_tiles(a.nb + a.nd);
    fdb_launch(k_export_tile_starts, dim3((unsigned)((tiles + kBlock - 1) / kBlock)), dim3(kBlock), 0, s, a);
    ScanState st;
    st.granules = granules;
    st.counter = (int*)&a.words[kXwScan];
    st.error = st.counter + 1;
    fdb_launch(k_export_scan, dim3((unsigned)tiles), dim3(kScanThreads), 0, s, a, st);
}


__device__ __forceinline__ uint64_t import_load8(const uint8_t* p) {
    const uintptr_t a = (uintptr_t)p;
    const uint64_t* w = (const uint64_t*)(a & ~(uintptr_t)7);
    const uint32_t sh = (uint32_t)(a & 7u) * 8u;
    const uint64_t x = w[0];
    return sh ? (x >> sh) | (w[1] << (64u - sh)) : x;
}

__device__ __forceinline__ int import_cmp(const uint8_t* a, uint32_t al, const uint8_t* b, uint32_t bl) {
    const uint32_t n = al < bl ? al : bl;
    uint32_t i = 0;
    for (; i + 8u <= n; i += 8u) {
        const uint64_t x = __builtin_bswap64(import_load8(a + i)), y = __builtin_bswap64(import_load8(b + i));
        if (x != y) return x < y ? -1 : 1;
    }
    if (i < n) {
        const uint64_t msk = ~0ull << (64u - 8u * (n - i));
        const uint64_t x = __builtin_bswap64(import_load8(a + i)) & msk, y = __builtin_bswap64(import_load8(b + i)) & msk;
        if (x != y) return x < y ? -1 : 1;
    }
    return (al > bl) - (al < bl);
}

__device__ __forceinline__ bool import_key(const ImportArgs& a, int64_t j, const uint8_t*& p, uint32_t& len) {
    const int64_t o0 = a.offsets[j], o1 = a.offsets[j + 1];
    p = a.bytes;
    len = 0;
    if (o0 < 0 || o1 < o0 || o1 > a.nbytes || o1 - o0 > (int64_t)INT32_MAX) return false;
    p = a.bytes + o0;
    len = (uint32_t)(o1 - o0);
    return true;
}

__global__ __launch_bounds__(kBlock) void k_import_check(ImportArgs a) {
    const int64_t j = (int64_t)blockIdx.x * blockDim.x + threadIdx.x;
    if (j >= a.n) return;
    const uint8_t *p, *q;
    uint32_t pl, ql;
    bool ok = import_key(a, j, p, pl);
    if (j == 0) {
        ok = ok && a.offsets[0] == 0;
    } else if (ok) {
        ok = import_key(a, j - 1, q, ql) && import_cmp(q, ql, p, pl) < 0;
    }
    if (!ok) atomicOr((int*)&a.words[kIwError], 1);
}

__global__ __launch_bounds__(64) void k_import_bounds(ImportArgs a) {
    __shared__ int64_t r[2];
    const int t = threadIdx.x;
    if (t < 2) {
        const bool is_hi = t == 1;
        int64_t lo = 0, hi = a.n;
        if (!(is_hi ? a.has_hi : a.has_lo)) {
            lo = is_hi ? a.n : 0;
        } else {
            const uint8_t* b = a.bnd + (is_hi ? a.bnd_hi : 0);
            const uint32_t bl = (uint32_t)(is_hi ? a.hi_len : a.lo_len);
            while (lo < hi) {
                const int64_t mid = lo + (hi - lo) / 2;
                const uint8_t* p;
                uint32_t pl;
                import_key(a, mid, p, pl);
// ... 206 lines not shown
```

Baseline: 54.59 million.

## Replace delta merge copy with output-indexed gather fused with epilogue index build

```diff
diff --git a/foundationdb_amd/build.py b/foundationdb_amd/build.py
--- a/foundationdb_amd/build.py
+++ b/foundationdb_amd/build.py
@@ -10,7 +10,7 @@
 ROOT = os.path.dirname(HERE)
 LIB = os.path.join(HERE, "libfdbcs.so")
 SOURCES = ["engine.cpp", "kernels.hip"]
-HEADERS = ["dkey.h", "engine.h", "scan.h", "launch.h", "lane_xor.h"]
+HEADERS = ["dkey.h", "engine.h", "scan.h", "launch.h", "lane_xor.h", "merge_map.h"]
 ARCH = os.environ.get("FDBCS_OFFLOAD_ARCH", "gfx950")
 
 
diff --git a/foundationdb_amd/csrc/engine.cpp b/foundationdb_amd/csrc/engine.cpp
--- a/foundationdb_amd/csrc/engine.cpp
+++ b/foundationdb_amd/csrc/engine.cpp
@@ -433,8 +433,10 @@
         int rc = cs->ws[k][kWsArenaSlot].ensure(8 * words + 64);
         if (rc) return rc;
         w.scan_arena = (uint64_t*)cs->ws[k][kWsArenaSlot].p;
-        if ((rc = cs->ws[k][kWsTileSlot].ensure(4 * (std::max(cs->hist_cap, cs->delta_cap) / 256 + 8)))) return rc;
+        const int64_t ctiles = std::max(cs->hist_cap, cs->delta_cap) / 256 + 8, otiles = cs->delta_cap / 256 + 8;
+        if ((rc = cs->ws[k][kWsTileSlot].ensure(4 * (ctiles + otiles)))) return rc;
         w.tile_first = (int32_t*)cs->ws[k][kWsTileSlot].p;
+        w.otile_first = w.tile_first + ctiles;
         carve_scans(w, cs->ws_T, cs->ws_R, cs->ws_W, cs->hist_cap, cs->delta_cap);
         HIPOK(hipMemsetAsync(w.scan_arena, 0, 8 * w.scan_words, cs->stream));
         for (int q = 0; q < kNumScans; q++) w.scan[q].error = &w.bsc->debug_error;
@@ -2639,8 +2641,15 @@
     if (cs->gc_interval > 0 && ++cs->batches_since_compact >= cs->gc_interval) compact = true;
     if (cs->tail_ub > cs->tail_reclaim) compact = true;
     char* hd = (char*)sl->pin_out.dp;
+    if (compact || !cs->edir[dnew].p) {
+        cs->ddir_epoch[dnew] = 0;
+    } else {
+        cs->ddir_epoch[dnew] = ++cs->ddir_counter;
+    }
+    const BatchFinish fin{(uint8_t*)hd, (uint32_t*)(hd + o_fl), b->seq, &sc->ndb[dnew], sort_nb, sort_samples};
     launch_merge(ys, bd, w, delta.h, delta.m, delta_of(cs, dnew), dlevels_of(cs, dnew), &sc->ndb[dsrc], htail, sc, now,
-                 cs->dlvl3_n, cs->dlvl2_n, cs->nd_ub + 1, rec(kPhCopyBegin, 1), rec(kPhCopyEnd, 1), long_keys);
+                 cs->dlvl3_n, cs->dlvl2_n, nd_after + 1, rec(kPhCopyBegin, 1), rec(kPhCopyEnd, 1), long_keys,
+                 compact ? nullptr : &fin);
     mark(kPhMerge);
     bool gc = false;
     int final_base = bsrc;
@@ -2668,14 +2677,7 @@
     mark(kPhGc);
     b->gc_ran = gc;
     b->compacted = compact;
-    if (compact || !cs->edir[dnew].p) {
-        cs->ddir_epoch[dnew] = 0;
-    } else {
-        cs->ddir_epoch[dnew] = ++cs->ddir_counter;
-    }
-    launch_epilogue(ys, bd, w, compact ? levels_of(cs, final_base) : dlevels_of(cs, dnew), sc, compact ? 1 : 0,
-                    gc ? 1 : 0, (uint8_t*)hd, (uint32_t*)(hd + o_fl), b->seq,
-                    compact ? base_hint : nd_after + 1, &sc->ndb[dnew], sort_nb, sort_samples);
+    if (compact) launch_epilogue(ys, bd, w, levels_of(cs, final_base), sc, gc ? 1 : 0, fin, base_hint);
     fdb_event(LaunchList::kSyncRecord, cs->ev_b[wp], ys);
     if (compact || gc) {
         fdb_event(LaunchList::kSyncRecord, cs->ev_cmp, ys);
diff --git a/foundationdb_amd/csrc/engine.h b/foundationdb_amd/csrc/engine.h
--- a/foundationdb_amd/csrc/engine.h
+++ b/foundationdb_amd/csrc/engine.h
@@ -106,7 +106,7 @@
     int32_t* tile_first;
 };
 
-enum ScanKind { kScanEdges, kScanSegSum, kScanCompact, kScanGc, kScanCover, kScanSegNum, kScanFold, kNumScans };
+enum ScanKind { kScanEdges, kScanSegSum, kScanCompact, kScanGc, kScanCover, kScanSegNum, kNumScans };
 
 struct BatchDev {
     int32_t T, R, W;
@@ -207,6 +207,7 @@
     int64_t scan_words;
     int64_t cap_T, cap_R;
     int32_t* tile_first;
+    int32_t* otile_first;
     int64_t *c_lo, *c_hi, *c_rem, *c_ins, *c_val;
     uint8_t* c_exact;
     unsigned long long* trace;
@@ -315,10 +316,17 @@
 void launch_validate_sort(hipStream_t s, const BatchDev& b, const Work& w);
 void launch_edges(hipStream_t s, const BatchDev& b, const Work& w);
 void launch_resolve(hipStream_t s, const BatchDev& b, const Work& w, bool report, uint8_t* verdict_out, Scalars* sc);
+struct BatchFinish {
+    uint8_t* verdict_out;
+    uint32_t* flag;
+    uint32_t seq;
+    int64_t* nd_out;
+    int sort_nb, sort_samples;
+};
 void launch_merge(hipStream_t s, const BatchDev& b, const Work& w, const Hist& src, const MaxLevels& srcm,
                   const Hist& dst, const MaxLevels& dstm, const int64_t* nd_src, uint8_t* htail, Scalars* sc,
-                  int64_t now, int64_t lvl3_n, int64_t lvl2_n, int64_t grid_hint_n, hipEvent_t copy_begin,
-                  hipEvent_t copy_end, bool long_keys = false);
+                  int64_t now, int64_t lvl3_n, int64_t lvl2_n, int64_t n_out_ub, hipEvent_t copy_begin,
+                  hipEvent_t copy_end, bool long_keys, const BatchFinish* fin);
 void launch_compact(hipStream_t s, const Work& w, const Hist& base, const MaxLevels& basem, const Hist& delta,
                     const Hist& dst, const uint8_t* htail, Scalars* sc, int64_t header_version, int64_t lvl3_n,
                     int64_t lvl2_n, int64_t delta_hint_n, int64_t grid_hint_n, hipEvent_t copy_begin,
@@ -334,9 +342,8 @@
 void carve_scans(Work& w, int64_t T, int64_t R, int64_t W, int64_t hist_cap, int64_t delta_cap);
 void launch_rangemax(hipStream_t s, const MaxLevels& m, Scalars* sc, const int64_t* n, int64_t lvl3_n,
                      int64_t lvl2_n, int64_t grid_hint_n);
-void launch_epilogue(hipStream_t s, const BatchDev& b, const Work& w, const MaxLevels& m, Scalars* sc,
-                     int compacted, int gc_ran, uint8_t* verdict_out, uint32_t* flag,
-                     uint32_t seq, int64_t grid_hint_n, int64_t* nd_out, int sort_nb, int sort_samples);
+void launch_epilogue(hipStream_t s, const BatchDev& b, const Work& w, const MaxLevels& m, Scalars* sc, int gc_ran,
+                     const BatchFinish& fin, int64_t grid_hint_n);
 int sort_cold_samples(int64_t E, int nb);
 
 enum ExportWord { kXwLo, kXwHi, kXwHeader, kXwN, kXwBytes, kXwScan , kXwWords = 8 };
diff --git a/foundationdb_amd/csrc/kernels.hip b/foundationdb_amd/csrc/kernels.hip
--- a/foundationdb_amd/csrc/kernels.hip
+++ b/foundationdb_amd/csrc/kernels.hip
@@ -7,6 +7,7 @@
 
 #include "engine.h"
 #include "lane_xor.h"
+#include "merge_map.h"
 
 namespace fdbcs {
 
@@ -2698,7 +2699,6 @@
     return b.keys[2 * g + end];
 }
 
-constexpr int kDeltaTile = 256;
 constexpr int kBaseTile = 4096;
 
 __device__ __forceinline__ void fill_tile_first(int32_t* tile_first, const int64_t* lo, int64_t j, int tile) {
@@ -2733,6 +2733,7 @@
     __shared__ uint32_t s_val[3][SP + 1];
     __shared__ uint32_t s_wsum[3][NSW];
     __shared__ uint32_t s_base[3];
+    __shared__ uint32_t s_pv[2];
     __shared__ int s_tile;
     const int64_t gt = (int64_t)blockIdx.x * blockDim.x + threadIdx.x;
     for (int64_t i = gt; i < lvl3_n * kL3Rep; i += (int64_t)gridDim.x * blockDim.x) lvl3[i * kL3Pad] = LLONG_MIN;
@@ -2746,7 +2747,7 @@
     const int64_t n = *io.n_in;
     const int q = threadIdx.x / (2 * LL), role = (threadIdx.x / LL) & 1;
     const int sg = tile * SP + (q < SP ? q : -1);
-    const bool live = sg >= 0 && sg < U && (q < SP || role == 0);
+    const bool live = sg >= 0 && sg < U;
     int64_t pos = 0;
     bool eq = false;
     DKey kb{}, ke{};
@@ -2771,6 +2772,9 @@
     if (threadIdx.x % (2 * LL) == 0) {
         if (q == SP) {
             s_lo[0] = live ? pos : 0;
+            const bool glue = live && dkey_cmp(seg_key(b, w, w.seg_b[sg + 1], 0), b.tail, ke, b.tail) == 0;
+            s_pv[0] = live ? (uint32_t)(hi - pos) : 0u;
+            s_pv[1] = live ? (!exact && !glue ? 2u : 1u) : 0u;
         } else if (live) {
             const int64_t lo = pos;
             const bool glue = sg + 1 < U && dkey_cmp(seg_key(b, w, w.seg_b[sg + 1], 0), b.tail, ke, b.tail) == 0;
@@ -2829,19 +2833,22 @@
             w.seg_rem[j] = ex[0];
             w.seg_ins[j] = ex[1];
             w.seg_tlen[j] = ex[2];
-            const int64_t t0 = j > 0 ? s_lo[k] / kDeltaTile + 1 : 0;
-            for (int64_t t = t0; t <= s_lo[k + 1] / kDeltaTile; t++) w.tile_first[t] = j;
+            const int64_t out = merge_out(s_lo[k + 1], ex[0], ex[1]);
+            const uint32_t prem = k > 0 ? s_val[0][k - 1] : s_pv[0], pins = k > 0 ? s_val[1][k - 1] : s_pv[1];
+            otile_fill(w.otile_first, j, out - (s_lo[k + 1] - (s_lo[k] + (int64_t)prem)) - (int64_t)pins, out);
         }
         if (tile == ntiles - 1 && j == U && k <= SP) {
             const uint32_t r = ex[0], in = ex[1], tl = ex[2];
             w.seg_rem[U] = r;
             w.seg_ins[U] = in;
             w.seg_tlen[U] = tl;
-            const int64_t t0 = U > 0 ? s_lo[k] / kDeltaTile + 1 : 0;
-            for (int64_t t = t0; t <= n / kDeltaTile + 1; t++) w.tile_first[t] = U;
+            const int64_t n_out = n - (int64_t)r + (int64_t)in;
+            const int64_t last_out =
+                U > 0 ? merge_out(s_lo[k], (int64_t)r - s_val[0][k - 1], (int64_t)in - s_val[1][k - 1]) : 0;
+            otile_fill_tail(w.otile_first, U, last_out, n_out);
             *io.before = n;
             *io.removed = r;
-            *io.n_out = n - (int64_t)r + (int64_t)in;
+            *io.n_out = n_out;
             sc->tail_next = sc->tail_used + 8 * (int64_t)tl;
         }
     }
@@ -2948,46 +2955,6 @@
     for (int64_t sg = (int64_t)blockIdx.x * blockDim.x + threadIdx.x; sg < U; sg += (int64_t)gridDim.x * blockDim.x)
         ins((int)sg, dst, g.lo[sg] - g.rem[sg] + g.ins[sg]);
 }
-
-struct BatchIns {
-    BatchDev b;
-    const uint32_t* pmeta;
-    const int32_t *seg_b, *seg_e;
-    const int64_t *tlen, *vend;
-    const uint8_t* endins;
-    uint8_t* htail;
-    const Scalars* sc;
-    int64_t now;
-    __device__ const DKey& key(int pos, int end) const {
-        return b.keys[2 * (int)item_range(pmeta[pos]) + end];
-    }
-    __device__ void operator()(int s, Hist dst, int64_t o) const {
-        int64_t tu = sc->tail_used / 8 + tlen[s];
-        const DKey kb = key(seg_b[s], 0);
-        uint32_t tb = 0;
-        if (kb.len > 16) {
-            tb = (uint32_t)tu;
-            copy_tail_words(htail + 8 * tu, b.tail + kb.tail, kb.len - 16);
-            tu += tail_units(kb.len);
-        }
-        dst.key[o] = make_ulonglong2(kb.hi, kb.lo);
-        dst.lt[o] = make_uint2(kb.len, tb);
-        dst.ver[o] = now;
-        if (endins[s]) {
-            const DKey ke = key(seg_e[s], 1);
-            uint32_t te = 0;
-            if (ke.len > 16) {
-                te = (uint32_t)tu;
-                copy_tail_words(htail + 8 * tu, b.tail + ke.tail, ke.len - 16);
-            }
-            dst.key[o + 1] = make_ulonglong2(ke.hi, ke.lo);
-            dst.lt[o + 1] = make_uint2(ke.len, te);
-            dst.ver[o + 1] = vend[s];
-        }
-    }
-};
-
-static Segs batch_segs(const Work& w) { return Segs{w.seg_lo, w.seg_hi, w.seg_rem, w.seg_ins, w.tile_first}; }
 
 static unsigned copy_tiles(int64_t grid_hint_n, int tile, int64_t max_inserts = 0) {
     int64_t tiles = (grid_hint_n + 1 + tile - 1) / tile;
@@ -3030,32 +2997,6 @@
     ep.zero_rank_n = sort_samples;
     ep.bsc = w.bsc;
     return ep;
-}
-
-void launch_merge(hipStream_t s, const BatchDev& b, const Work& w, const Hist& src, const MaxLevels& srcm,
-                  const Hist& dst, const MaxLevels& dstm, const int64_t* nd_src, uint8_t* htail, Scalars* sc,
-                  int64_t now, int64_t lvl3_n, int64_t lvl2_n, int64_t grid_hint_n, hipEvent_t copy_begin,
-                  hipEvent_t copy_end, bool long_keys) {
-    const TierIO io{nd_src, &sc->nd_next, &sc->d_before, &sc->d_rem};
-    const bool wide = seg_wide(b.W, long_keys);
-    fdb_launch(long_keys ? k_seg_prep<true, true> : (wide ? k_seg_prep<false, true> : k_seg_prep<false, false>),
-               dim3((unsigned)seg_tiles(b.W, long_keys, wide)), dim3(seg_threads(long_keys, wide)), 0, s, b, w, src, srcm, htail, sc, io, dstm.lvl[3], lvl3_n,
-               dstm.lvl[2], lvl2_n);
-    fdb_event(LaunchList::kTimingRecord, copy_begin, s);
-    BatchIns ins{};
-    ins.b = b;
-    ins.pmeta = w.pmeta;
-    ins.seg_b = w.seg_b;
-    ins.seg_e = w.seg_e;
-    ins.tlen = w.seg_tlen;
-    ins.vend = w.seg_vend;
-    ins.endins = w.seg_endins;
-    ins.htail = htail;
-    ins.sc = sc;
-    ins.now = now;
-    fdb_launch((k_merge_copy<BatchIns, kDeltaTile>), dim3(copy_tiles(grid_hint_n, kDeltaTile, b.W)), dim3(kBlock), 0,
-               s, batch_segs(w), src, dst, nd_src, &w.bsc->n_segments, ins);
-    fdb_event(LaunchList::kTimingRecord, copy_end, s);
 }
 
 
@@ -3456,9 +3397,7 @@
 static_assert(kScWords <= 32 && kBscWords <= 32, "one lane per word, Scalars in lanes 0-31, BatchScalars in 32-63");
 constexpr int sc_word(size_t off) { return (int)(off / 8); }
 
-template <bool BASE>
-__global__ __launch_bounds__(kEpiThreads) void k_epilogue(MaxLevels m, Scalars* sc, const int64_t* n_levels, Epilogue ep) {
-    if (threadIdx.x == 0) trace_min(ep.trace, kTrEpiBegin);
+__device__ __forceinline__ uint64_t epilogue_prefetch(const Epilogue& ep, const Scalars* sc) {
     const int lane = threadIdx.x & 63, wid = threadIdx.x >> 6;
     uint64_t pre = 0;
     if (ep.verdict_out && blockIdx.x == 0 && wid == 0) {
@@ -3467,97 +3406,11 @@
         else if (lane >= 32 && lane < 32 + kBscWords)
             pre = reinterpret_cast<const uint64_t*>(ep.bsc)[lane - 32];
     }
-    int64_t n0;
-    if (n_levels)
-        n0 = *n_levels;
-    else if (ep.compacted)
-        n0 = ep.gc_ran ? sc->n_gc : sc->n_next;
-    else
-        n0 = sc->nd_next;
-    const int64_t n1 = (n0 + kFan - 1) / kFan, nwv = (n1 + kEpiBlocks - 1) / kEpiBlocks;
-    for (int64_t wv = (int64_t)blockIdx.x * kEpiWaves + wid; wv < nwv; wv += (int64_t)gridDim.x * kEpiWaves) {
-        const int64_t b1_0 = wv * kEpiBlocks;
-        int64_t v[kEpiBlocks];
-#pragma unroll
-        for (int q = 0; q < kEpiBlocks; q++) {
-            const int64_t i = (b1_0 + q) * kFan + lane;
-            v[q] = i < n0 ? m.lvl[0][i] : LLONG_MIN;
-        }
-        const int64_t b1l = b1_0 + lane;
-        ulonglong2 sk = make_ulonglong2(0, 0);
-        if (lane < kEpiBlocks && b1l < n1) sk = m.keys[b1l * kFan];
-        constexpr int kE8 = kEpiBlocks * kFan / 8;
-        static_assert(kE8 <= 64, "one skey8 entry per lane");
-        const int64_t n8 = (n0 + 7) / 8, e8_0 = b1_0 * (kFan / 8);
-        ulonglong2 k8 = make_ulonglong2(0, 0);
-        ulonglong2 prev_k = make_ulonglong2(0, 0);
-        if (lane < kE8 && e8_0 + lane < n8) {
-            k8 = m.keys[(e8_0 + lane) * 8];
-            m.skey8[e8_0 + lane] = k8;
-        }
-        if (m.edir_epoch && lane == 0 && e8_0 > 0 && e8_0 < n8) prev_k = m.keys[(e8_0 - 1) * 8];
-        int64_t mine = LLONG_MIN;
-#pragma unroll
-        for (int q = 0; q < kEpiBlocks; q++) {
-            int64_t x = v[q];
-#pragma unroll
-            for (int o = 32; o > 0; o >>= 1) {
-                const int64_t y = __shfl_xor(x, o, 64);
-                x = y > x ? y : x;
-            }
-            if (lane == q) mine = x;
-        }
-        if (lane < kEpiBlocks && b1l < n1) {
-            m.lvl[1][b1l] = mine;
-            m.skey[0][b1l] = sk;
-            int64_t d = b1l, off = 0;
-            for (int L = 1; L < kIdxLevels && d % kArity == 0; L++) {
-                off += idx_level_cap(m.idx_cap, L - 1);
-                d /= kArity;
-                m.skey[0][off + d] = sk;
-            }
-        }
-        if (m.edir_epoch) {
-            const int64_t e = e8_0 + lane;
-            const bool live = lane < kE8 && e < n8;
-            const int64_t c_l = live ? (int64_t)dir_slot(m, k8.x, k8.y) : -1;
-            int64_t a = __shfl_up(c_l, 1, 64);
-            if (lane == 0) a = e8_0 > 0 && live ? (int64_t)dir_slot(m, prev_k.x, prev_k.y) : -1;
-            const uint64_t tag = (uint64_t)m.edir_epoch << 32;
-            const int64_t z = live ? (c_l < a + kDirRun ? c_l : a + kDirRun) : a;
-            const bool wide = live && z - a > 4;
-            if (live && !wide)
-                for (int64_t v = a + 1; v <= z; v++) m.edir[v] = tag | (uint64_t)e;
-            for (uint64_t wm = __ballot(wide); wm; wm &= wm - 1) {
-                const int q = __builtin_ctzll(wm);
-                const int64_t aq = __shfl(a, q, 64), zq = __shfl(z, q, 64);
-                for (int64_t v = aq + 1 + lane; v <= zq; v += 64) m.edir[v] = tag | (uint64_t)(e8_0 + q);
-            }
-            const uint64_t lm = __ballot(live && e == n8 - 1);
-            if (lm) {
-                const int q = __builtin_ctzll(lm);
-                const int64_t cq = __shfl(c_l, q, 64);
-                const int64_t top = (int64_t)m.dir_top + 1, z2 = cq + kDirRun < top ? cq + kDirRun : top;
-                for (int64_t v = cq + 1 + lane; v <= z2; v += 64) m.edir[v] = tag | (uint64_t)n8;
-            }
-        }
-        int64_t x = lane < kEpiBlocks ? mine : LLONG_MIN;
-#pragma unroll
-        for (int o = 1; o < kEpiBlocks; o <<= 1) {
-            const int64_t y = __shfl_xor(x, o, 64);
-            x = y > x ? y : x;
-        }
-#ifndef FDBCS_EPI_EXP
-#define FDBCS_EPI_EXP 0
-#endif
-        if (lane == 0 && b1_0 < n1) {
-            if (!(FDBCS_EPI_EXP & 1)) atomicMax((long long*)&m.lvl[2][b1_0 / kFan], (long long)x);
-            int64_t* l3 = &m.lvl[3][((b1_0 / ((int64_t)kFan * kFan)) * kL3Rep + (int64_t)(blockIdx.x % kL3Rep)) * kL3Pad];
-            if (!(FDBCS_EPI_EXP & 2) && x > __hip_atomic_load(l3, __ATOMIC_RELAXED, __HIP_MEMORY_SCOPE_AGENT))
-                atomicMax((long long*)l3, (long long)x);
-        }
-    }
-    if (!ep.verdict_out) return;
+    return pre;
+}
+
+__device__ __forceinline__ void epilogue_finish(const Epilogue& ep, Scalars* sc, uint64_t pre) {
+    const int lane = threadIdx.x & 63, wid = threadIdx.x >> 6;
     if (threadIdx.x == 0) trace_max(ep.trace, kTrEpiLevels);
     const int64_t tid = (int64_t)blockIdx.x * blockDim.x + threadIdx.x, stride = (int64_t)gridDim.x * blockDim.x;
     for (int64_t i = tid; i < ep.zero8_n; i += stride) ep.zero8[i] = 0;
@@ -3624,6 +3477,105 @@
     }
 }
 
+template <bool BASE>
+__global__ __launch_bounds__(kEpiThreads) void k_epilogue(MaxLevels m, Scalars* sc, const int64_t* n_levels, Epilogue ep) {
+    if (threadIdx.x == 0) trace_min(ep.trace, kTrEpiBegin);
+    const int lane = threadIdx.x & 63, wid = threadIdx.x >> 6;
+    const uint64_t pre = epilogue_prefetch(ep, sc);
+    int64_t n0;
+    if (n_levels)
+        n0 = *n_levels;
+    else if (ep.compacted)
+        n0 = ep.gc_ran ? sc->n_gc : sc->n_next;
+    else
+        n0 = sc->nd_next;
+    const int64_t n1 = (n0 + kFan - 1) / kFan, nwv = (n1 + kEpiBlocks - 1) / kEpiBlocks;
+    for (int64_t wv = (int64_t)blockIdx.x * kEpiWaves + wid; wv < nwv; wv += (int64_t)gridDim.x * kEpiWaves) {
+        const int64_t b1_0 = wv * kEpiBlocks;
+        int64_t v[kEpiBlocks];
+#pragma unroll
+        for (int q = 0; q < kEpiBlocks; q++) {
+            const int64_t i = (b1_0 + q) * kFan + lane;
+            v[q] = i < n0 ? m.lvl[0][i] : LLONG_MIN;
+        }
+        const int64_t b1l = b1_0 + lane;
+        ulonglong2 sk = make_ulonglong2(0, 0);
+        if (lane < kEpiBlocks && b1l < n1) sk = m.keys[b1l * kFan];
+        constexpr int kE8 = kEpiBlocks * kFan / 8;
+        static_assert(kE8 <= 64, "one skey8 entry per lane");
+        const int64_t n8 = (n0 + 7) / 8, e8_0 = b1_0 * (kFan / 8);
+        ulonglong2 k8 = make_ulonglong2(0, 0);
+        ulonglong2 prev_k = make_ulonglong2(0, 0);
+        if (lane < kE8 && e8_0 + lane < n8) {
+            k8 = m.keys[(e8_0 + lane) * 8];
+            m.skey8[e8_0 + lane] = k8;
+        }
+        if (m.edir_epoch && lane == 0 && e8_0 > 0 && e8_0 < n8) prev_k = m.keys[(e8_0 - 1) * 8];
+        int64_t mine = LLONG_MIN;
+#pragma unroll
+        for (int q = 0; q < kEpiBlocks; q++) {
+            int64_t x = v[q];
+#pragma unroll
+            for (int o = 32; o > 0; o >>= 1) {
+                const int64_t y = __shfl_xor(x, o, 64);
+                x = y > x ? y : x;
+            }
+            if (lane == q) mine = x;
+        }
+        if (lane < kEpiBlocks && b1l < n1) {
+            m.lvl[1][b1l] = mine;
+            m.skey[0][b1l] = sk;
+            int64_t d = b1l, off = 0;
+            for (int L = 1; L < kIdxLevels && d % kArity == 0; L++) {
+                off += idx_level_cap(m.idx_cap, L - 1);
+                d /= kArity;
+                m.skey[0][off + d] = sk;
+            }
+        }
+        if (m.edir_epoch) {
+            const int64_t e = e8_0 + lane;
+            const bool live = lane < kE8 && e < n8;
+            const int64_t c_l = live ? (int64_t)dir_slot(m, k8.x, k8.y) : -1;
+            int64_t a = __shfl_up(c_l, 1, 64);
+            if (lane == 0) a = e8_0 > 0 && live ? (int64_t)dir_slot(m, prev_k.x, prev_k.y) : -1;
+            const uint64_t tag = (uint64_t)m.edir_epoch << 32;
+            const int64_t z = live ? (c_l < a + kDirRun ? c_l : a + kDirRun) : a;
+            const bool wide = live && z - a > 4;
+            if (live && !wide)
+                for (int64_t v = a + 1; v <= z; v++) m.edir[v] = tag | (uint64_t)e;
+            for (uint64_t wm = __ballot(wide); wm; wm &= wm - 1) {
+                const int q = __builtin_ctzll(wm);
+                const int64_t aq = __shfl(a, q, 64), zq = __shfl(z, q, 64);
+                for (int64_t v = aq + 1 + lane; v <= zq; v += 64) m.edir[v] = tag | (uint64_t)(e8_0 + q);
+            }
+            const uint64_t lm = __ballot(live && e == n8 - 1);
+            if (lm) {
+                const int q = __builtin_ctzll(lm);
+                const int64_t cq = __shfl(c_l, q, 64);
+                const int64_t top = (int64_t)m.dir_top + 1, z2 = cq + kDirRun < top ? cq + kDirRun : top;
+                for (int64_t v = cq + 1 + lane; v <= z2; v += 64) m.edir[v] = tag | (uint64_t)n8;
+            }
+        }
+        int64_t x = lane < kEpiBlocks ? mine : LLONG_MIN;
+#pragma unroll
+        for (int o = 1; o < kEpiBlocks; o <<= 1) {
+            const int64_t y = __shfl_xor(x, o, 64);
+            x = y > x ? y : x;
+        }
+#ifndef FDBCS_EPI_EXP
+#define FDBCS_EPI_EXP 0
+#endif
+        if (lane == 0 && b1_0 < n1) {
+            if (!(FDBCS_EPI_EXP & 1)) atomicMax((long long*)&m.lvl[2][b1_0 / kFan], (long long)x);
+            int64_t* l3 = &m.lvl[3][((b1_0 / ((int64_t)kFan * kFan)) * kL3Rep + (int64_t)(blockIdx.x % kL3Rep)) * kL3Pad];
+            if (!(FDBCS_EPI_EXP & 2) && x > __hip_atomic_load(l3, __ATOMIC_RELAXED, __HIP_MEMORY_SCOPE_AGENT))
+                atomicMax((long long*)l3, (long long)x);
+        }
+    }
+    if (!ep.verdict_out) return;
+    epilogue_finish(ep, sc, pre);
+}
+
 __global__ __launch_bounds__(kBlock) void k_copy_bytes(uint8_t* __restrict__ dst, const uint8_t* __restrict__ src,
                                                        int64_t n) {
     for (int64_t i = (int64_t)blockIdx.x * blockDim.x + threadIdx.x; i < n; i += (int64_t)gridDim.x * blockDim.x)
@@ -3711,20 +3663,201 @@
     fdb_launch(k_epilogue<true>, dim3((unsigned)epilogue_grid(grid_hint_n, 0)), dim3(kEpiThreads), 0, s, m, sc, n, ep);
 }
 
-void launch_epilogue(hipStream_t s, const BatchDev& b, const Work& w, const MaxLevels& m, Scalars* sc,
-                     int compacted, int gc_ran, uint8_t* verdict_out, uint32_t* flag,
-                     uint32_t seq, int64_t grid_hint_n, int64_t* nd_out, int sort_nb, int sort_samples) {
-    Epilogue ep = make_epilogue(b, w, compacted, gc_ran, verdict_out, flag, seq, sort_nb, sort_samples);
-    ep.nd_out = nd_out;
-    if (compacted) launch_directory(s, m, gc_ran ? &sc->n_gc : &sc->n_next);
+static int64_t epilogue_extra(const BatchDev& b, const Epilogue& ep) {
     int64_t extra = std::max<int64_t>(b.R, b.T);
     for (int k = 0; k <= kNumScans; k++) extra = std::max(extra, ep.zero64_n[k]);
-    if (compacted)
-        fdb_launch(k_epilogue<true>, dim3((unsigned)epilogue_grid(grid_hint_n, extra)), dim3(kEpiThreads), 0, s, m, sc,
-                   (const int64_t*)nullptr, ep);
-    else
-        fdb_launch(k_epilogue<false>, dim3((unsigned)epilogue_grid(grid_hint_n, extra)), dim3(kEpiThreads), 0, s, m, sc,
-                   (const int64_t*)nullptr, ep);
+    return extra;
+}
+
+void launch_epilogue(hipStream_t s, const BatchDev& b, const Work& w, const MaxLevels& m, Scalars* sc, int gc_ran,
+                     const BatchFinish& fin, int64_t grid_hint_n) {
+    Epilogue ep = make_epilogue(b, w, 1, gc_ran, fin.verdict_out, fin.flag, fin.seq, fin.sort_nb, fin.sort_samples);
+    ep.nd_out = fin.nd_out;
+    launch_directory(s, m, gc_ran ? &sc->n_gc : &sc->n_next);
+    fdb_launch(k_epilogue<true>, dim3((unsigned)epilogue_grid(grid_hint_n, epilogue_extra(b, ep))), dim3(kEpiThreads),
+               0, s, m, sc, (const int64_t*)nullptr, ep);
+}
+
+struct MergeIns {
+    const DKey* segk;
+    const uint8_t* btail;
+    const int64_t *tlen, *vend;
+    uint8_t* htail;
+    const int64_t* U;
+    int64_t now;
+};
+
+struct OutSegs {
+    const int64_t *lo, *rem, *ins;
+    const int32_t* otile_first;
+};
+
+template <bool INDEX>
+__global__ __launch_bounds__(kBlock) void k_merge_gather(OutSegs g, Hist src, Hist dst, MaxLevels m, Scalars* sc,
+                                                         MergeIns ins, Epilogue ep) {
+    static_assert(kMergeTile == kBlock && kMergeTile == 4 * kFan && kMergeBack == 8,
+                  "one output position per thread, one level-1 block per wave, one group start back");
+    __shared__ int64_t s_out[kMergeSlots], s_shift[kMergeSlots];
+    __shared__ int32_t s_nins[kMergeSlots];
+    __shared__ int64_t s_wmax[kBlock / 64];
+    __shared__ int s_first, s_next;
+    const int lane = threadIdx.x & 63, wid = threadIdx.x >> 6;
+    uint64_t pre = 0;
+    if constexpr (INDEX) {
+        if (threadIdx.x == 0) trace_min(ep.trace, kTrEpiBegin);
+        pre = epilogue_prefetch(ep, sc);
+    }
+    const int64_t n_out = sc->nd_next;
+    auto fetch = [&](const MergeSrc& r, ulonglong2& kk, uint2& lt, int64_t& vv) __attribute__((always_inline)) {
+        if (r.seg < 0) {
+            kk = src.key[r.src];
+            lt = src.lt[r.src];
+            vv = src.ver[r.src];
+            return;
+        }
+        const int sg = r.seg;
+        const DKey k = ins.segk[2 * sg + r.which];
+        int64_t tu = (sc->tail_next - 8 * ins.tlen[*ins.U]) / 8 + ins.tlen[sg];
+        vv = ins.now;
+        if (r.which) {
+            tu += tail_units(ins.segk[2 * sg].len);
+            vv = ins.vend[sg];
+        }
+        uint32_t tt = 0;
+        if (k.len > 16) {
+            tt = (uint32_t)tu;
+            copy_tail_words(ins.htail + 8 * tu, ins.btail + k.tail, k.len - 16);
+        }
+        kk = make_ulonglong2(k.hi, k.lo);
+        lt = make_uint2(k.len, tt);
+    };
+    auto fetch_key = [&](const MergeSrc& r) __attribute__((always_inline)) -> ulonglong2 {
+        if (r.seg < 0) return src.key[r.src];
+        const DKey& k = ins.segk[2 * r.seg + r.which];
+        return make_ulonglong2(k.hi, k.lo);
+    };
+    for (int64_t t = blockIdx.x; t * kMergeTile < n_out; t += gridDim.x) {
+        if (threadIdx.x == 0) {
+            s_first = g.otile_first[t];
+            s_next = g.otile_first[t + 1];
+        }
+        __syncthreads();
+        const int64_t seg0 = (int64_t)s_first - kMergeBack;
+        const int cnt = merge_slot_count(s_first, s_next);
+        for (int k = threadIdx.x; k < cnt; k += blockDim.x) {
+            const MergeSlot sl = merge_slot(g.lo, g.rem, g.ins, seg0 + k);
+            s_out[k] = sl.out;
+            s_shift[k] = sl.shift;
+            s_nins[k] = sl.nins;
+        }
+        __syncthreads();
+        const int64_t o = t * kMergeTile + threadIdx.x;
+        const bool live = o < n_out;
+        ulonglong2 kk = make_ulonglong2(0, 0), prev_k = make_ulonglong2(0, 0);
+        uint2 lt = make_uint2(0, 0);
+        int64_t vv = LLONG_MIN;
+        if (live) fetch(merge_locate(s_out, s_shift, s_nins, cnt, seg0, o), kk, lt, vv);
+        if constexpr (INDEX) {
+            if (m.edir_epoch && lane == 1 && o - 1 < n_out && o >= 9)
+                prev_k = fetch_key(merge_locate(s_out, s_shift, s_nins, cnt, seg0, o - 9));
+        }
+        if (live) {
+            dst.key[o] = kk;
+            dst.lt[o] = lt;
+            dst.ver[o] = vv;
+        }
+        if constexpr (INDEX) {
+            const int64_t b1 = o >> 6;
+            const int64_t n8 = (n_out + 7) / 8, e = o >> 3;
+            const bool start = live && (lane & 7) == 0;
+            int64_t x = vv;
+#pragma unroll
+            for (int w = 32; w > 0; w >>= 1) {
+                const int64_t y = __shfl_xor(x, w, 64);
+                x = y > x ? y : x;
+            }
+            if (start) m.skey8[e] = kk;
+            if (lane == 0 && live) {
+                m.lvl[1][b1] = x;
+                m.skey[0][b1] = kk;
+                int64_t d = b1, off = 0;
+                for (int L = 1; L < kIdxLevels && d % kArity == 0; L++) {
+                    off += idx_level_cap(m.idx_cap, L - 1);
+                    d /= kArity;
+                    m.skey[0][off + d] = kk;
+                }
+            }
+            if (m.edir_epoch) {
+                const bool probe = lane == 1 && o - 1 < n_out && o >= 9;
+                const ulonglong2 qk = probe ? prev_k : kk;
+                const int64_t c_q = start || probe ? (int64_t)dir_slot(m, qk.x, qk.y) : -1;
+                const int64_t c_l = start ? c_q : -1;
+                int64_t a = __shfl_up(c_l, 8, 64);
+                const int64_t a0 = __shfl(c_q, 1, 64);
+                if (lane == 0) a = a0;
+                const uint64_t tag = (uint64_t)m.edir_epoch << 32;
+                const int64_t z = start ? (c_l < a + kDirRun ? c_l : a + kDirRun) : a;
+                const bool wide = start && z - a > 4;
+                if (start && !wide)
+                    for (int64_t v = a + 1; v <= z; v++) m.edir[v] = tag | (uint64_t)e;
+                for (uint64_t wm = __ballot(wide); wm; wm &= wm - 1) {
+                    const int q = __builtin_ctzll(wm);
+                    const int64_t aq = __shfl(a, q, 64), zq = __shfl(z, q, 64), eq = __shfl(e, q, 64);
+                    for (int64_t v = aq + 1 + lane; v <= zq; v += 64) m.edir[v] = tag | (uint64_t)eq;
+                }
+                const uint64_t lm = __ballot(start && e == n8 - 1);
+                if (lm) {
+                    const int q = __builtin_ctzll(lm);
+                    const int64_t cq = __shfl(c_l, q, 64);
+                    const int64_t top = (int64_t)m.dir_top + 1, z2 = cq + kDirRun < top ? cq + kDirRun : top;
+                    for (int64_t v = cq + 1 + lane; v <= z2; v += 64) m.edir[v] = tag | (uint64_t)n8;
+                }
+            }
+            if (lane == 0) s_wmax[wid] = x;
+        }
+        __syncthreads();
+        if constexpr (INDEX) {
+            if (threadIdx.x == 0) {
+                int64_t x = s_wmax[0];
+#pragma unroll
+                for (int q = 1; q < kBlock / 64; q++) x = s_wmax[q] > x ? s_wmax[q] : x;
+                const int64_t b1_0 = t * (kMergeTile / kFan);
+                atomicMax((long long*)&m.lvl[2][b1_0 / kFan], (long long)x);
+                int64_t* l3 = &m.lvl[3][((b1_0 / ((int64_t)kFan * kFan)) * kL3Rep + (int64_t)(blockIdx.x % kL3Rep)) * kL3Pad];
+                if (x > __hip_atomic_load(l3, __ATOMIC_RELAXED, __HIP_MEMORY_SCOPE_AGENT)) atomicMax((long long*)l3, (long long)x);
+            }
+        }
+    }
+    if constexpr (INDEX) epilogue_finish(ep, sc, pre);
+}
+
+static unsigned gather_grid(int64_t n_out_ub, int64_t extra) {
+    int64_t tiles = std::max<int64_t>((n_out_ub + kMergeTile - 1) / kMergeTile, (extra + kBlock - 1) / kBlock);
+    return (unsigned)std::min<int64_t>(std::max<int64_t>(tiles, 1), 8192);
+}
+
+void launch_merge(hipStream_t s, const BatchDev& b, const Work& w, const Hist& src, const MaxLevels& srcm,
+                  const Hist& dst, const MaxLevels& dstm, const int64_t* nd_src, uint8_t* htail, Scalars* sc,
+                  int64_t now, int64_t lvl3_n, int64_t lvl2_n, int64_t n_out_ub, hipEvent_t copy_begin,
+                  hipEvent_t copy_end, bool long_keys, const BatchFinish* fin) {
+    const TierIO io{nd_src, &sc->nd_next, &sc->d_before, &sc->d_rem};
+    const bool wide = seg_wide(b.W, long_keys);
+    fdb_launch(long_keys ? k_seg_prep<true, true> : (wide ? k_seg_prep<false, true> : k_seg_prep<false, false>),
+               dim3((unsigned)seg_tiles(b.W, long_keys, wide)), dim3(seg_threads(long_keys, wide)), 0, s, b, w, src, srcm, htail, sc, io, dstm.lvl[3], lvl3_n,
+               dstm.lvl[2], lvl2_n);
+    fdb_event(LaunchList::kTimingRecord, copy_begin, s);
+    const OutSegs g{w.seg_lo, w.seg_rem, w.seg_ins, w.otile_first};
+    const MergeIns ins{w.segk, b.tail, w.seg_tlen, w.seg_vend, htail, &w.bsc->n_segments, now};
+    if (fin) {
+        Epilogue ep = make_epilogue(b, w, 0, 0, fin->verdict_out, fin->flag, fin->seq, fin->sort_nb, fin->sort_samples);
+        ep.nd_out = fin->nd_out;
+        fdb_launch(k_merge_gather<true>, dim3(gather_grid(n_out_ub, epilogue_extra(b, ep))), dim3(kBlock), 0, s, g, src,
+                   dst, dstm, sc, ins, ep);
+    } else {
+        fdb_launch(k_merge_gather<false>, dim3(gather_grid(n_out_ub, 0)), dim3(kBlock), 0, s, g, src, dst, dstm, sc,
+                   ins, Epilogue{});
+    }
+    fdb_event(LaunchList::kTimingRecord, copy_end, s);
 }
 
 
diff --git a/foundationdb_amd/csrc/merge_map.h b/foundationdb_amd/csrc/merge_map.h
--- /dev/null
+++ b/foundationdb_amd/csrc/merge_map.h
@@ -0,0 +1,76 @@
+#pragma once
+#include <stdint.h>
+
+#if defined(__HIPCC__)
+#define FDBCS_MM_HD __host__ __device__
+#else
+#define FDBCS_MM_HD
+#endif
+
+namespace fdbcs {
+
+constexpr int kMergeTile = 256;
+constexpr int kMergeBack = 8;
+constexpr int kMergeSlots = kMergeTile + kMergeBack;
+
+FDBCS_MM_HD inline int64_t merge_out(int64_t lo, int64_t rem, int64_t ins) { return lo - rem + ins; }
+
+struct MergeSlot {
+    int64_t out, shift;
+    int32_t nins;
+};
+FDBCS_MM_HD inline MergeSlot merge_slot(const int64_t* lo, const int64_t* rem, const int64_t* ins, int64_t j) {
+    MergeSlot s;
+    if (j < 0) {
+        s.out = INT64_MIN;
+        s.shift = 0;
+        s.nins = 0;
+    } else {
+        s.out = merge_out(lo[j], rem[j], ins[j]);
+        s.shift = rem[j + 1] - ins[j + 1];
+        s.nins = (int32_t)(ins[j + 1] - ins[j]);
+    }
+    return s;
+}
+
+FDBCS_MM_HD inline int merge_slot_count(int32_t first, int32_t next) { return next - first + kMergeBack; }
+
+struct MergeSrc {
+    int64_t src;
+    int32_t seg, which;
+};
+
+FDBCS_MM_HD inline MergeSrc merge_locate(const int64_t* s_out, const int64_t* s_shift, const int32_t* s_nins, int cnt,
+                                         int64_t seg0, int64_t o) {
+    int sl = 0;
+#if defined(__HIP_DEVICE_COMPILE__)
+#pragma unroll
+#endif
+    for (int step = 256; step > 0; step >>= 1) {
+        const int mid = sl + step;
+        if (mid < cnt && s_out[mid] <= o) sl = mid;
+    }
+    static_assert(kMergeSlots < 512, "the lifting's first step covers every slot");
+    MergeSrc r;
+    if (s_nins[sl] > 0 && o - s_out[sl] < s_nins[sl]) {
+        r.src = -1;
+        r.seg = (int32_t)(seg0 + sl);
+        r.which = (int32_t)(o - s_out[sl]);
+    } else {
+        r.src = o + s_shift[sl];
+        r.seg = -1;
+        r.which = 0;
+    }
+    return r;
+}
+
+FDBCS_MM_HD inline void otile_fill(int32_t* otile_first, int64_t j, int64_t prev_out, int64_t out) {
+    const int64_t t0 = j > 0 ? prev_out / kMergeTile + 1 : 0;
+    for (int64_t t = t0; t <= out / kMergeTile; t++) otile_first[t] = (int32_t)j;
+}
+FDBCS_MM_HD inline void otile_fill_tail(int32_t* otile_first, int64_t U, int64_t last_out, int64_t n_out) {
+    const int64_t t0 = U > 0 ? last_out / kMergeTile + 1 : 0;
+    for (int64_t t = t0; t <= n_out / kMergeTile + 1; t++) otile_first[t] = (int32_t)U;
+}
+
+}
```

After: 53.91 million. -1.3%, worse.
